# ynalcakan/RGBX_Semantic_Segmentation

Hardware: AMD Instinct MI355X
Metric: train images/sec CMX-B2 480x640 bs=2/GPU at 1/2/4/8 MI355X; % MFMA roofline (higher is better)
Workload: dtype bf16

## Files before the change

### rgbx_semantic_segmentation_amd/_lib.py

```python
from __future__ import annotations

import ctypes
import os
import re

import torch

_HERE = os.path.dirname(os.path.abspath(__file__))
_VARIANT = os.environ.get("CMX_LIB_VARIANT", "")
LIB_PATH = os.path.join(_HERE, f"libcmx_hip_{_VARIANT}.so" if _VARIANT else "libcmx_hip.so")
HEADER_PATHS = [os.path.join(_HERE, "..", "include", "cmx_hip.h"), os.path.join(_HERE, "cmx_hip.h")]
OHEM_HEADER_PATHS = [os.path.join(_HERE, "..", "include", "cmx_ohem.h"), os.path.join(_HERE, "cmx_ohem.h")]
EASPP_HEADER_PATHS = [os.path.join(_HERE, "..", "include", "cmx_easpp.h"), os.path.join(_HERE, "cmx_easpp.h")]
FCN_HEADER_PATHS = [os.path.join(_HERE, "..", "include", "cmx_fcn.h"), os.path.join(_HERE, "cmx_fcn.h")]
DEEPLAB_HEADER_PATHS = [os.path.join(_HERE, "..", "include", "cmx_deeplab.h"), os.path.join(_HERE, "cmx_deeplab.h")]


class CMXError(RuntimeError):
    pass


CMX_OK, CMX_ERR_SHAPE, CMX_ERR_DTYPE, CMX_ERR_LAUNCH, CMX_ERR_ARG = 0, -1, -2, -3, -4


def _ctype(decl: str):
    decl = decl.strip()
    if "*" in decl:
        if decl.startswith("const char") and decl.count("*") == 1 and not decl.split("*")[1].strip():
            return ctypes.c_char_p
        return ctypes.c_void_p
    base = decl.rsplit(" ", 1)[0] if " " in decl else decl
    base = base.replace("const", "").strip()
    return {"int": ctypes.c_int32, "int64_t": ctypes.c_int64, "uint64_t": ctypes.c_uint64, "float": ctypes.c_float,
            "size_t": ctypes.c_size_t, "double": ctypes.c_double, "hipStream_t": ctypes.c_void_p, "void": None}[base]


POINTER, STREAM, SCALAR = "pointer", "stream", "scalar"


def _kind(decl: str) -> str:
    if "*" in decl:
        return SCALAR if decl.strip().startswith("const char") else POINTER
    return STREAM if "hipStream_t" in decl.split() else SCALAR


class Signature(tuple):
    kinds: tuple = ()


def _header(path: str | None) -> str:
    return open(path or next(p for p in HEADER_PATHS if os.path.exists(p))).read()


def parse_header(path: str | None = None):
    text = re.sub(r"/\*.*?\*/", "", _header(path), flags=re.S)
    out = {}
    for m in re.finditer(r"^\s*([A-Za-z_][\w\s\*]*?)\b(cmx_\w+)\s*\(([^)]*)\)\s*;", text, re.M):
        ret, name, args = m.group(1), m.group(2), m.group(3).strip()
        rt = ctypes.c_char_p if ret.strip() == "const char*" else _ctype(ret.strip() + " r")
        decls = [] if args in ("", "void") else args.split(",")
        out[name] = Signature((rt, [_ctype(a) for a in decls]))
        out[name].kinds = tuple(_kind(a) for a in decls)
    return out


def header_abi_version(path: str | None = None) -> int:
    m = re.search(r"^#define\s+CMX_ABI_VERSION\s+(\d+)", _header(path), re.M)
    if m is None:
        raise CMXError(f"{path or 'cmx_hip.h'} defines no CMX_ABI_VERSION")
    return int(m.group(1))


def _load():
    if not os.path.exists(LIB_PATH):
        raise CMXError(f"libcmx_hip.so not found at {LIB_PATH}; run __graft_entry__.build() "
                       "(or `make -C rgbx_semantic_segmentation_amd/csrc`).  There is no CPU fallback.")
    lib = ctypes.CDLL(LIB_PATH)
    lib.cmx_abi_version.restype = ctypes.c_int32
    lib.cmx_abi_version.argtypes = []
    want, have = header_abi_version(), int(lib.cmx_abi_version())
    if have != want:
        raise CMXError(f"{LIB_PATH} was built for C-ABI revision {have}, the header declares {want}: "
                       "rebuild it (`make -C rgbx_semantic_segmentation_amd/csrc`)")
    sigs = parse_header()
    ohem = parse_header(next(p for p in OHEM_HEADER_PATHS if os.path.exists(p)))
    easpp = parse_header(next(p for p in EASPP_HEADER_PATHS if os.path.exists(p)))
    fcn = parse_header(next(p for p in FCN_HEADER_PATHS if os.path.exists(p)))
    deeplab = parse_header(next(p for p in DEEPLAB_HEADER_PATHS if os.path.exists(p)))
    for table in (sigs, ohem, easpp, fcn, deeplab):
        for name, (rt, argt) in table.items():
            fn = getattr(lib, name)
            fn.argtypes = argt
            fn.restype = rt
            assert STREAM not in table[name].kinds[:-1], f"{name}: hipStream_t must be the last parameter"
    return lib, sigs, ohem, easpp, fcn, deeplab


LIB, SIGNATURES, OHEM_SIGNATURES, EASPP_SIGNATURES, FCN_SIGNATURES, DEEPLAB_SIGNATURES = _load()


def last_error() -> str:
    return LIB.cmx_last_error().decode()


def stream() -> int:
    return torch.cuda.current_stream().cuda_stream


def ptr(t) -> int:
    return 0 if t is None else t.data_ptr()


def _pointer_arg(a):
    return a.data_ptr() if isinstance(a, torch.Tensor) else a


def _scalar_arg(a):
    if isinstance(a, torch.Tensor):
        raise TypeError("a tensor was passed where the header declares a scalar")
    return int(a) if a is True or a is False else a


_BOUND = {name: (getattr(LIB, name), tuple(_pointer_arg if k == POINTER else _scalar_arg for k in sig.kinds),
                 sig.kinds[-1:] == (STREAM,))
          for name, sig in {**SIGNATURES, **OHEM_SIGNATURES, **EASPP_SIGNATURES, **FCN_SIGNATURES,
                            **DEEPLAB_SIGNATURES}.items()}


def marshal(name: str, args: tuple) -> tuple:
    _, convs, takes_stream = _BOUND[name]
    if len(args) != len(convs):
        if not (takes_stream and len(args) == len(convs) - 1):
            raise TypeError(f"{name} takes {len(convs)} arguments, {len(args)} given")
        args = (*args, stream())
    return tuple([c(a) for c, a in zip(convs, args)])


observer = None


def try_call(name: str, *args) -> int:
    fn = _BOUND[name][0]
    args = marshal(name, args)
    st = int(fn(*args))
    if st == 0 and observer is not None:
        observer(name, fn, args)
    return st


def call(name: str, *args) -> None:
    refusable(name, (), *args)


REFUSED = object()


def refusable(name: str, refusals: tuple, *args):
    st = try_call(name, *args)
    if st in refusals:
        return REFUSED
    if st != 0:
        raise CMXError(f"{name} failed ({st}): {last_error()}")


def query(name: str, *args) -> int:
    return int(_BOUND[name][0](*marshal(name, args)))


DTYPE_CODES = {torch.float32: 0, torch.bfloat16: 1, torch.float16: 2}


def dtype_code(t: torch.Tensor) -> int:
    if t.dtype not in DTYPE_CODES:
        raise CMXError(f"unsupported dtype {t.dtype}")
    return DTYPE_CODES[t.dtype]
```

### rgbx_semantic_segmentation_amd/csrc/dwconv.hip

```cpp
#include "cmx_common.h"

namespace {
constexpr int RXF = 4;
constexpr int RXB = 2;
constexpr int RY = 8;
constexpr int DW_BWD_THREADS = 65536;

typedef cmx_f2 Px[2];

template <typename T>
__device__ __forceinline__ void ld4(const T* p, Px& v) {
  if constexpr (sizeof(T) == 4) {
    const float4 a = *reinterpret_cast<const float4*>(p);
    v[0] = (cmx_f2){a.x, a.y};
    v[1] = (cmx_f2){a.z, a.w};
  } else {
    const uint2 a = *reinterpret_cast<const uint2*>(p);
    v[0] = unpack2<T>(a.x);
    v[1] = unpack2<T>(a.y);
  }
}

template <typename T>
__device__ __forceinline__ void st4(T* p, const Px& v) {
  if constexpr (sizeof(T) == 4) {
    *reinterpret_cast<float4*>(p) = make_float4(v[0].x, v[0].y, v[1].x, v[1].y);
  } else {
    *reinterpret_cast<uint2*>(p) = make_uint2(pack2<T>(v[0].x, v[0].y), pack2<T>(v[1].x, v[1].y));
  }
}

template <typename T>
__device__ __forceinline__ cmx_f2 stored(cmx_f2 v) {
  if constexpr (sizeof(T) == 4) {
    return v;
  } else {
    return unpack2<T>(pack2<T>(v.x, v.y));
  }
}

__device__ __forceinline__ void load_w36(const float* wg, cmx_f2 (&w2)[2][9]) {
  const float4* p = reinterpret_cast<const float4*>(wg);
  float w[36];
#pragma unroll
  for (int i = 0; i < 9; ++i) {
    const float4 a = p[i];
    w[4 * i] = a.x; w[4 * i + 1] = a.y; w[4 * i + 2] = a.z; w[4 * i + 3] = a.w;
  }
#pragma unroll
  for (int k = 0; k < 9; ++k) {
    w2[0][k] = (cmx_f2){w[k], w[9 + k]};
    w2[1][k] = (cmx_f2){w[18 + k], w[27 + k]};
  }
}

__device__ __forceinline__ void load_bias(const float* b, Px& bias) {
  if (b) {
    const float4 bb = *reinterpret_cast<const float4*>(b);
    bias[0] = (cmx_f2){bb.x, bb.y};
    bias[1] = (cmx_f2){bb.z, bb.w};
  } else {
    bias[0] = bias[1] = pk_splat(0.f);
  }
}

template <typename T, int R>
__device__ __forceinline__ void load_row(const T* ib, int y, int x0, int H, int W, int C, Px (&r)[R + 2]) {
  const bool yok = y >= 0 && y < H;
#pragma unroll
  for (int j = 0; j < R + 2; ++j) {
    const int x = x0 - 1 + j;
    if (yok && x >= 0 && x < W) {
      ld4<T>(ib + (y * W + x) * C, r[j]);
    } else {
      r[j][0] = pk_splat(0.f);
      r[j][1] = pk_splat(0.f);
    }
  }
}

struct Strip {
  int img, x0, y0;
};

template <int R>
__device__ __forceinline__ Strip strip_of(int s, int NXS, int NYS) {
  Strip st;
  st.x0 = (s % NXS) * R;
  const int r = s / NXS;
  st.y0 = (r % NYS) * RY;
  st.img = r / NYS;
  return st;
}

template <typename T, bool FLIP, int ACT>
__global__ __launch_bounds__(256) void dw_fwd_kernel(const T* __restrict__ h, const float* __restrict__ w,
                                                     const float* __restrict__ b, T* __restrict__ out, int ipg, int H,
                                                     int W, int C, int NXS, int NYS) {
  const int CQ = C >> 2;
  const int t = blockIdx.x * blockDim.x + threadIdx.x;
  if (t >= CQ * NXS * NYS * ipg) return;
  const int g = blockIdx.y;
  const int c0 = (t % CQ) * 4;
  const Strip st = strip_of<RXF>(t / CQ, NXS, NYS);
  cmx_f2 wr[2][9];
  load_w36(w + ((long)g * C + c0) * 9, wr);
  Px bias;
  load_bias(b ? b + g * C + c0 : nullptr, bias);
  const long off = ((long)g * ipg + st.img) * H * W * C + c0;
  const T* ib = h + off;
  T* ob = out + off;
  Px rin[3][RXF + 2];
  load_row<T, RXF>(ib, st.y0 - 1, st.x0, H, W, C, rin[0]);
  load_row<T, RXF>(ib, st.y0, st.x0, H, W, C, rin[1]);
#pragma unroll
  for (int rr = 0; rr < RY; ++rr) {
    const int y = st.y0 + rr;
    load_row<T, RXF>(ib, y + 1, st.x0, H, W, C, rin[(rr + 2) % 3]);
#pragma unroll
    for (int xi = 0; xi < RXF; ++xi) {
      Px acc = {bias[0], bias[1]};
#pragma unroll
      for (int i = 0; i < 3; ++i)
#pragma unroll
        for (int j = 0; j < 3; ++j) {
          const int tap = FLIP ? 8 - (i * 3 + j) : i * 3 + j;
#pragma unroll
          for (int u = 0; u < 2; ++u) acc[u] = pk_fma(wr[u][tap], rin[(rr + i) % 3][xi + j][u], acc[u]);
        }
      acc[0] = act2_fwd<ACT>(acc[0]);
      acc[1] = act2_fwd<ACT>(acc[1]);
      if (y < H && st.x0 + xi < W) st4<T>(ob + (y * W + st.x0 + xi) * C, acc);
    }
  }
}

template <typename T, int ACT>
__global__ __launch_bounds__(256) void dw_bwd_dz_kernel(const T* __restrict__ da, const T* __restrict__ h,
                                                        const float* __restrict__ w, const float* __restrict__ b,
                                                        T* __restrict__ dz, float* __restrict__ ws, int ipg, int H,
                                                        int W, int C, int NXS, int NYS, int P) {
  const int CQ = C >> 2;
  const int t = blockIdx.x * blockDim.x + threadIdx.x;
  if (t >= CQ * P) return;
  const int g = blockIdx.y;
  const int q = t % CQ, slot = t / CQ;
  const int c0 = q * 4;
  cmx_f2 wr[2][9], aw[2][9];
  Px bias, ab;
  load_w36(w + ((long)g * C + c0) * 9, wr);
  load_bias(b ? b + g * C + c0 : nullptr, bias);
#pragma unroll
  for (int u = 0; u < 2; ++u) {
    ab[u] = pk_splat(0.f);
#pragma unroll
    for (int k = 0; k < 9; ++k) aw[u][k] = pk_splat(0.f);
  }
  const int nstrips = NXS * NYS * ipg;
  for (int s = slot; s < nstrips; s += P) {
    const Strip st = strip_of<RXB>(s, NXS, NYS);
    const long off = ((long)g * ipg + st.img) * H * W * C + c0;
    const T* ib = h + off;
    const T* dab = da + off;
    T* dzb = dz + off;
    Px rin[3][RXB + 2];
    load_row<T, RXB>(ib, st.y0 - 1, st.x0, H, W, C, rin[0]);
    load_row<T, RXB>(ib, st.y0, st.x0, H, W, C, rin[1]);
#pragma unroll
    for (int rr = 0; rr < RY; ++rr) {
      const int y = st.y0 + rr;
      load_row<T, RXB>(ib, y + 1, st.x0, H, W, C, rin[(rr + 2) % 3]);
#pragma unroll
      for (int xi = 0; xi < RXB; ++xi) {
        const bool in = y < H && st.x0 + xi < W;
        Px d = {pk_splat(0.f), pk_splat(0.f)};
        if (in) {
          Px z = {bias[0], bias[1]};
#pragma unroll
          for (int k = 0; k < 9; ++k)
#pragma unroll
            for (int u = 0; u < 2; ++u) z[u] = pk_fma(wr[u][k], rin[(rr + k / 3) % 3][xi + k % 3][u], z[u]);
          const int pofs = (y * W + st.x0 + xi) * C;
          ld4<T>(dab + pofs, d);
#pragma unroll
          for (int u = 0; u < 2; ++u) d[u] = d[u] * act2_grad<ACT>(z[u]);
          st4<T>(dzb + pofs, d);
#pragma unroll
          for (int u = 0; u < 2; ++u) d[u] = stored<T>(d[u]);
        }
#pragma unroll
        for (int u = 0; u < 2; ++u) {
          ab[u] += d[u];
#pragma unroll
          for (int k = 0; k < 9; ++k) aw[u][k] = pk_fma(d[u], rin[(rr + k / 3) % 3][xi + k % 3][u], aw[u][k]);
        }
      }
    }
  }
  float* o = ws + ((long)g * P + slot) * C * 10 + (long)c0 * 10;
#pragma unroll
  for (int u = 0; u < 2; ++u) {
#pragma unroll
    for (int k = 0; k < 9; ++k) {
      o[(2 * u) * 10 + k] = aw[u][k].x;
      o[(2 * u + 1) * 10 + k] = aw[u][k].y;
    }
    o[(2 * u) * 10 + 9] = ab[u].x;
    o[(2 * u + 1) * 10 + 9] = ab[u].y;
  }
}

__global__ void dw_scatter_kernel(const float* __restrict__ tmp, float* __restrict__ dw, float* __restrict__ db, int G,
                                  int C, int accumulate) {
  const long total = (long)G * C * 10;
  for (int i = blockIdx.x * blockDim.x + threadIdx.x; i < (int)total; i += gridDim.x * blockDim.x) {
    const int k = i % 10;
    const int gc = i / 10;
    const float s = tmp[i];
    float* o = k < 9 ? &dw[gc * 9 + k] : (db ? &db[gc] : nullptr);
    if (o) *o = accumulate ? *o + s : s;
  }
}

constexpr int TY2 = 8, TX2 = 16;
constexpr int EY = TY2 + 2, EX = TX2 + 2;
constexpr int HY = TY2 + 4, HX = TX2 + 4;
constexpr int TYB = 16, TXB = 16, EYB = TYB + 2, EXB = TXB + 2;

template <typename T> struct V8;
template <> struct V8<bf16> { uint4 a; };
template <> struct V8<f16> { uint4 a; };
template <> struct V8<float> { float4 a, b; };

template <typename T>
__device__ __forceinline__ V8<T> v8_load(const T* p) {
  V8<T> v;
  if constexpr (sizeof(T) == 2) v.a = *reinterpret_cast<const uint4*>(p);
  else { v.a = reinterpret_cast<const float4*>(p)[0]; v.b = reinterpret_cast<const float4*>(p)[1]; }
  return v;
}
template <typename T>
__device__ __forceinline__ void v8_store(T* p, const V8<T>& v) {
  if constexpr (sizeof(T) == 2) *reinterpret_cast<uint4*>(p) = v.a;
  else { reinterpret_cast<float4*>(p)[0] = v.a; reinterpret_cast<float4*>(p)[1] = v.b; }
}
template <typename T>
__device__ __forceinline__ V8<T> v8_zero() {
  V8<T> v;
  if constexpr (sizeof(T) == 2) v.a = make_uint4(0, 0, 0, 0);
  else { v.a = make_float4(0.f, 0.f, 0.f, 0.f); v.b = v.a; }
  return v;
}
template <typename T>
__device__ __forceinline__ void v8_unpack(const V8<T>& v, cmx_f2 (&o)[4]) {
  if constexpr (sizeof(T) == 2) {
    const uint32_t w[4] = {v.a.x, v.a.y, v.a.z, v.a.w};
#pragma unroll
    for (int i = 0; i < 4; ++i) o[i] = unpack2<T>(w[i]);
  } else {
    o[0] = (cmx_f2){v.a.x, v.a.y}; o[1] = (cmx_f2){v.a.z, v.a.w};
    o[2] = (cmx_f2){v.b.x, v.b.y}; o[3] = (cmx_f2){v.b.z, v.b.w};
  }
}
template <typename T>
__device__ __forceinline__ V8<T> v8_pack(const cmx_f2 (&o)[4]) {
  V8<T> v;
  if constexpr (sizeof(T) == 2) {
    v.a = make_uint4(pack2<T>(o[0].x, o[0].y), pack2<T>(o[1].x, o[1].y), pack2<T>(o[2].x, o[2].y),
                     pack2<T>(o[3].x, o[3].y));
  } else {
    v.a = make_float4(o[0].x, o[0].y, o[1].x, o[1].y);
    v.b = make_float4(o[2].x, o[2].y, o[3].x, o[3].y);
  }
  return v;
}

__device__ __forceinline__ void load_w72(const float* wg, cmx_f2 (&w2)[4][9]) {
  cmx_f2 (&a)[2][9] = *reinterpret_cast<cmx_f2 (*)[2][9]>(&w2[0]);
  cmx_f2 (&b)[2][9] = *reinterpret_cast<cmx_f2 (*)[2][9]>(&w2[2]);
  load_w36(wg, a);
  load_w36(wg + 36, b);
}

struct Tile2 {
  int g, img, ty0, tx0, cb0, sp;
};
template <int TY_ = TY2, int TX_ = TX2>
__device__ __forceinline__ Tile2 tile2_of(int CB, int ipg, int tiles_x, int tiles_y, int ncb) {
  Tile2 t;
  int b = blockIdx.x;
  const int cb = b % ncb; b /= ncb;
  t.sp = b;
  const int tx = b % tiles_x; b /= tiles_x;
  const int ty = b % tiles_y; b /= tiles_y;
  t.img = b;
  t.g = blockIdx.y;
  t.ty0 = ty * TY_; t.tx0 = tx * TX_; t.cb0 = cb * CB;
  return t;
}

template <typename T, int CB, int RY_, int RX_>
__device__ __forceinline__ void stage_region(const T* __restrict__ base, T* img, int y0, int x0, int H, int W, int C) {
  constexpr int NCG = CB / 8, NPX = RY_ * RX_;
  constexpr int ITER = (NCG * NPX + 255) / 256;
  V8<T> v[ITER];
#pragma unroll
  for (int k = 0; k < ITER; ++k) {
    const int it = threadIdx.x + k * 256;
    const int cg = it % NCG, px = it / NCG;
    const int y = y0 + px / RX_, x = x0 + px % RX_;
    v[k] = v8_zero<T>();
    if (it < NCG * NPX && y >= 0 && y < H && x >= 0 && x < W) v[k] = v8_load<T>(base + ((long)y * W + x) * C + cg * 8);
  }
#pragma unroll
  for (int k = 0; k < ITER; ++k) {
    const int it = threadIdx.x + k * 256;
    if (it < NCG * NPX) v8_store<T>(img + ((it % NCG) * NPX + it / NCG) * 8, v[k]);
  }
}

template <typename T> struct V4;
template <> struct V4<bf16> { uint2 a; };
template <> struct V4<f16> { uint2 a; };
template <> struct V4<float> { float4 a; };
template <typename T>
__device__ __forceinline__ V4<T> v4_load(const T* p) {
  V4<T> v;
  if constexpr (sizeof(T) == 2) v.a = *reinterpret_cast<const uint2*>(p);
  else v.a = *reinterpret_cast<const float4*>(p);
  return v;
}
template <typename T>
__device__ __forceinline__ void v4_unpack(const V4<T>& v, cmx_f2 (&o)[2]) {
  if constexpr (sizeof(T) == 2) {
    o[0] = unpack2<T>(v.a.x);
    o[1] = unpack2<T>(v.a.y);
  } else {
    o[0] = (cmx_f2){v.a.x, v.a.y}; o[1] = (cmx_f2){v.a.z, v.a.w};
  }
}
template <typename T>
__device__ __forceinline__ void v4_store(T* p, const cmx_f2 (&o)[2]) {
  if constexpr (sizeof(T) == 2) *reinterpret_cast<uint2*>(p) = make_uint2(pack2<T>(o[0].x, o[0].y), pack2<T>(o[1].x, o[1].y));
  else *reinterpret_cast<float4*>(p) = make_float4(o[0].x, o[0].y, o[1].x, o[1].y);
}
template <typename T, int CB, int RY_, int RX_>
__device__ __forceinline__ void stage_region_pm(const T* __restrict__ base, T* img, int y0, int x0, int H, int W, int C) {
  constexpr int NCG = CB / 8, NPX = RY_ * RX_;
  constexpr int ITER = (NCG * NPX + 255) / 256;
  V8<T> v[ITER];
#pragma unroll
  for (int k = 0; k < ITER; ++k) {
    const int it = threadIdx.x + k * 256;
    const int cg = it % NCG, px = it / NCG;
    const int y = y0 + px / RX_, x = x0 + px % RX_;
    v[k] = v8_zero<T>();
    if (it < NCG * NPX && y >= 0 && y < H && x >= 0 && x < W) v[k] = v8_load<T>(base + ((long)y * W + x) * C + cg * 8);
  }
#pragma unroll
  for (int k = 0; k < ITER; ++k) {
    const int it = threadIdx.x + k * 256;
    if (it < NCG * NPX) v8_store<T>(img + it * 8, v[k]);
  }
}

template <typename T, int CB, int ACT, bool FLIP>
__global__ __launch_bounds__(256) void dw2_fwd_kernel(const T* __restrict__ h, const float* __restrict__ w,
                                                      const float* __restrict__ b, T* __restrict__ out, int ipg, int H,
                                                      int W, int C, int tiles_x, int tiles_y, int ncb,
                                                      T* __restrict__ gprime) {
  constexpr int NCQ = CB / 4, PPI = 256 / NCQ;
  __shared__ __attribute__((aligned(16))) T hs[EY * EX * CB];
  const Tile2 t = tile2_of(CB, ipg, tiles_x, tiles_y, ncb);
  const long ibase = ((long)t.g * ipg + t.img) * H * W * C + t.cb0;
  stage_region_pm<T, CB, EY, EX>(h + ibase, hs, t.ty0 - 1, t.tx0 - 1, H, W, C);
  const int cq = threadIdx.x % NCQ, pl = threadIdx.x / NCQ;
  const int c0 = t.cb0 + cq * 4;
  __syncthreads();
  cmx_f2 wr[2][9], bias[2];
  load_w36(w + ((long)t.g * C + c0) * 9, wr);
  if (b) {
    const float4 b0 = *reinterpret_cast<const float4*>(b + (long)t.g * C + c0);
    bias[0] = (cmx_f2){b0.x, b0.y}; bias[1] = (cmx_f2){b0.z, b0.w};
  } else {
    bias[0] = bias[1] = pk_splat(0.f);
  }
  const T* hc = hs + cq * 4;
  if constexpr (PPI == TX2) {
    const int x = t.tx0 + pl;
    const int nr = H - t.ty0;
    if (x >= W) return;
    const T* hp = hc + pl * CB;
    cmx_f2 win[3][3][2];
#pragma unroll
    for (int j = 0; j < 3; ++j) {
      v4_unpack<T>(v4_load<T>(hp + j * CB), win[0][j]);
      v4_unpack<T>(v4_load<T>(hp + (EX + j) * CB), win[1][j]);
    }
    long o = ibase + ((long)t.ty0 * W + x) * C + cq * 4;
    const long ostep = (long)W * C;
#pragma unroll
    for (int r = 0; r < TY2; ++r) {
      if (r < nr) {
#pragma unroll
        for (int j = 0; j < 3; ++j) {
          v4_unpack<T>(v4_load<T>(hp + ((r + 2) * EX + j) * CB), win[(r + 2) % 3][j]);
        }
        cmx_f2 acc[2] = {bias[0], bias[1]};
#pragma unroll
        for (int i = 0; i < 3; ++i)
#pragma unroll
          for (int j = 0; j < 3; ++j) {
            const int tap = FLIP ? 8 - (i * 3 + j) : i * 3 + j;
#pragma unroll
            for (int u = 0; u < 2; ++u) acc[u] = pk_fma(wr[u][tap], win[(r + i) % 3][j][u], acc[u]);
          }
        if (gprime) {
          cmx_f2 gd[2];
#pragma unroll
          for (int u = 0; u < 2; ++u) gd[u] = act2_grad<ACT>(acc[u]);
          v4_store<T>(gprime + o, gd);
        }
#pragma unroll
        for (int u = 0; u < 2; ++u) acc[u] = act2_fwd<ACT>(acc[u]);
        v4_store<T>(out + o, acc);
        o += ostep;
      }
    }
  } else {
    for (int it = pl; it < TY2 * TX2; it += PPI) {
      const int r = it / TX2, c = it % TX2;
      const int y = t.ty0 + r, x = t.tx0 + c;
      if (y >= H || x >= W) continue;
      cmx_f2 acc[2] = {bias[0], bias[1]};
#pragma unroll
      for (int i = 0; i < 3; ++i)
#pragma unroll
        for (int j = 0; j < 3; ++j) {
          cmx_f2 v[2];
          v4_unpack<T>(v4_load<T>(hc + ((r + i) * EX + c + j) * CB), v);
          const int tap = FLIP ? 8 - (i * 3 + j) : i * 3 + j;
#pragma unroll
          for (int u = 0; u < 2; ++u) acc[u] = pk_fma(wr[u][tap], v[u], acc[u]);
        }
      const long o = ibase + ((long)y * W + x) * C + cq * 4;
      if (gprime) {
        cmx_f2 gd[2];
#pragma unroll
        for (int u = 0; u < 2; ++u) gd[u] = act2_grad<ACT>(acc[u]);
        v4_store<T>(gprime + o, gd);
      }
#pragma unroll
      for (int u = 0; u < 2; ++u) acc[u] = act2_fwd<ACT>(acc[u]);
      v4_store<T>(out + o, acc);
    }
  }
}

template <int N>
__device__ __forceinline__ void rs_step(const float (&v)[N], float (&o)[N / 2], int off, bool up) {
#pragma unroll
  for (int k = 0; k < N / 2; ++k) {
    const float send = up ? v[k] : v[k + N / 2];
    const float keep = up ? v[k + N / 2] : v[k];
    o[k] = keep + xor_lane(send, off);
  }
}

template <typename T, int CB>
__device__ __forceinline__ void stage_dz(const T* __restrict__ da, const T* __restrict__ gp, T* dzs, int ty0, int tx0,
                                         int H, int W, int C) {
  constexpr int NCG = CB / 8, NE = EYB * EXB;
  constexpr int ITE = (NCG * NE + 255) / 256;
  V8<T> a[ITE], g[ITE];
#pragma unroll
  for (int k = 0; k < ITE; ++k) {
    const int it = threadIdx.x + k * 256;
    const int cg = it % NCG, px = it / NCG;
    const int y = ty0 - 1 + px / EXB, x = tx0 - 1 + px % EXB;
    a[k] = v8_zero<T>();
    g[k] = v8_zero<T>();
    if (it < NCG * NE && y >= 0 && y < H && x >= 0 && x < W) {
      const long o = ((long)y * W + x) * C + cg * 8;
      a[k] = v8_load<T>(da + o);
      g[k] = v8_load<T>(gp + o);
    }
  }
#pragma unroll
  for (int k = 0; k < ITE; ++k) {
    const int it = threadIdx.x + k * 256;
    if (it < NCG * NE) {
      cmx_f2 d[4], gd[4];
      v8_unpack<T>(a[k], d);
      v8_unpack<T>(g[k], gd);
#pragma unroll
      for (int u = 0; u < 4; ++u) d[u] = d[u] * gd[u];
      v8_store<T>(dzs + it * 8, v8_pack<T>(d));
    }
  }
}

template <typename T, int CB>
__global__ __launch_bounds__(256, 3) void dw2_bwdg_kernel(const T* __restrict__ da, const T* __restrict__ h,
                                                       const T* __restrict__ gprime, const float* __restrict__ w,
                                                       T* __restrict__ dh, float* __restrict__ part, int ipg, int H,
                                                       int W, int C, int tiles_x, int tiles_y, int ncb, int nsp) {
  constexpr int NCQ = CB / 4, PPI = 256 / NCQ;
  constexpr int NE = EYB * EXB, NIN = TYB * TXB;
  constexpr int LPQ = 64 / NCQ;
  constexpr int NV = LPQ == 4 ? 10 : 5;
  constexpr int NIT = NIN / PPI;
  __shared__ __attribute__((aligned(16))) T dzs[NE * CB];
  static_assert(sizeof(dzs) >= 4 * 64 * NV * sizeof(float), "cross-wave reduce buffer");
  static_assert(NIN % PPI == 0, "pixel rounds");
  const Tile2 t = tile2_of<TYB, TXB>(CB, ipg, tiles_x, tiles_y, ncb);
  const long ibase = ((long)t.g * ipg + t.img) * H * W * C + t.cb0;
  stage_dz<T, CB>(da + ibase, gprime + ibase, dzs, t.ty0, t.tx0, H, W, C);
  const int cq = threadIdx.x % NCQ, pl = threadIdx.x / NCQ;
  const int c0 = t.cb0 + cq * 4;
  V4<T> hreg[NIT];
#pragma unroll
  for (int k = 0; k < NIT; ++k) {
    const int it = pl + k * PPI;
    const int y = t.ty0 + it / TXB, x = t.tx0 + it % TXB;
    hreg[k].a = {};
    if (y < H && x < W) hreg[k] = v4_load<T>(h + ibase + ((long)y * W + x) * C + cq * 4);
  }
  __syncthreads();
  cmx_f2 wr[2][9];
  load_w36(w + ((long)t.g * C + c0) * 9, wr);
  const T* dzc = dzs + cq * 4;
  cmx_f2 acc[2][10];
#pragma unroll
  for (int u = 0; u < 2; ++u)
#pragma unroll
    for (int k = 0; k < 10; ++k) acc[u][k] = pk_splat(0.f);
  if constexpr (PPI == TXB) {
    const int x = t.tx0 + pl;
    const int nr = H - t.ty0;
    if (x < W) {
      const T* dzp = dzc + pl * CB;
      cmx_f2 win[3][3][2];
#pragma unroll
      for (int j = 0; j < 3; ++j) {
        v4_unpack<T>(v4_load<T>(dzp + j * CB), win[0][j]);
        v4_unpack<T>(v4_load<T>(dzp + (EXB + j) * CB), win[1][j]);
      }
      long o = ibase + ((long)t.ty0 * W + x) * C + cq * 4;
      const long ostep = (long)W * C;
#pragma unroll
      for (int k = 0; k < NIT; ++k) {
        if (k < nr) {
#pragma unroll
          for (int j = 0; j < 3; ++j) v4_unpack<T>(v4_load<T>(dzp + ((k + 2) * EXB + j) * CB), win[(k + 2) % 3][j]);
          cmx_f2 hv[2];
          v4_unpack<T>(hreg[k], hv);
          cmx_f2 g[2] = {pk_splat(0.f), pk_splat(0.f)};
#pragma unroll
          for (int i = 0; i < 3; ++i)
#pragma unroll
            for (int j = 0; j < 3; ++j) {
              const cmx_f2 (&dv)[2] = win[(k + 2 - i) % 3][2 - j];
#pragma unroll
              for (int u = 0; u < 2; ++u) {
                g[u] = pk_fma(wr[u][i * 3 + j], dv[u], g[u]);
                acc[u][i * 3 + j] = pk_fma(hv[u], dv[u], acc[u][i * 3 + j]);
              }
              if (i == 1 && j == 1) {
#pragma unroll
                for (int u = 0; u < 2; ++u) acc[u][9] += dv[u];
              }
            }
          if (dh) v4_store<T>(dh + o, g);
          o += ostep;
        }
      }
    }
  } else {
#pragma unroll
    for (int k = 0; k < NIT; ++k) {
      const int it = pl + k * PPI;
      const int r = it / TXB, c = it % TXB;
      const int y = t.ty0 + r, x = t.tx0 + c;
      if (y >= H || x >= W) continue;
      cmx_f2 hv[2];
      v4_unpack<T>(hreg[k], hv);
      cmx_f2 g[2] = {pk_splat(0.f), pk_splat(0.f)};
#pragma unroll
      for (int i = 0; i < 3; ++i)
#pragma unroll
        for (int j = 0; j < 3; ++j) {
          cmx_f2 dv[2];
          v4_unpack<T>(v4_load<T>(dzc + ((r + 2 - i) * EXB + c + 2 - j) * CB), dv);
#pragma unroll
          for (int u = 0; u < 2; ++u) {
            g[u] = pk_fma(wr[u][i * 3 + j], dv[u], g[u]);
            acc[u][i * 3 + j] = pk_fma(hv[u], dv[u], acc[u][i * 3 + j]);
          }
          if (i == 1 && j == 1) {
#pragma unroll
            for (int u = 0; u < 2; ++u) acc[u][9] += dv[u];
          }
        }
      if (dh) v4_store<T>(dh + ibase + ((long)y * W + x) * C + cq * 4, g);
    }
  }
  const int lane = threadIdx.x & 63, wv = threadIdx.x >> 6;
  float flat[40], r20[20], r10[10];
#pragma unroll
  for (int u = 0; u < 2; ++u)
#pragma unroll
    for (int k = 0; k < 10; ++k) {
      flat[(2 * u) * 10 + k] = acc[u][k].x;
      flat[(2 * u + 1) * 10 + k] = acc[u][k].y;
    }
  int seg = 0;
  rs_step<40>(flat, r20, NCQ, (lane & NCQ) != 0); seg = seg * 2 + ((lane & NCQ) != 0);
  rs_step<20>(r20, r10, 2 * NCQ, (lane & (2 * NCQ)) != 0); seg = seg * 2 + ((lane & (2 * NCQ)) != 0);
  float rv[NV];
  if constexpr (NV == 5) {
    rs_step<10>(r10, rv, 4 * NCQ, (lane & (4 * NCQ)) != 0); seg = seg * 2 + ((lane & (4 * NCQ)) != 0);
  } else {
#pragma unroll
    for (int k = 0; k < 10; ++k) rv[k] = r10[k];
  }
  __syncthreads();
  float* red = reinterpret_cast<float*>(dzs);
#pragma unroll
  for (int k = 0; k < NV; ++k) red[(wv * 64 + lane) * NV + k] = rv[k];
  __syncthreads();
  float* o = part + ((long)t.g * nsp + t.sp) * C * 10 + (long)t.cb0 * 10;
  for (int e = threadIdx.x; e < 64 * NV; e += 256) {
    const float v = red[e] + red[64 * NV + e] + red[128 * NV + e] + red[192 * NV + e];
    const int l = e / NV, k = e % NV;
    const int q = l % NCQ, sg = (l / NCQ);
    int sgi = 0;
#pragma unroll
    for (int bit = 0; bit < (NV == 5 ? 3 : 2); ++bit) sgi = sgi * 2 + ((sg >> bit) & 1);
    o[q * 40 + sgi * NV + k] = v;
  }
}


template <typename T, int CB, int ACT>
__global__ __launch_bounds__(256, 2) void dw2_bwd_kernel(const T* __restrict__ da, const T* __restrict__ h,
                                                      const float* __restrict__ w, const float* __restrict__ b,
                                                      T* __restrict__ dh, float* __restrict__ part, int ipg, int H,
                                                      int W, int C, int tiles_x, int tiles_y, int ncb, int nsp) {
  constexpr int NCG = CB / 8, TPC = 256 / NCG;
  __shared__ __attribute__((aligned(16))) T hs[NCG * HY * HX * 8];
  __shared__ __attribute__((aligned(16))) T das[NCG * EY * EX * 8];
  __shared__ __attribute__((aligned(16))) T dzs[NCG * EY * EX * 8];
  const Tile2 t = tile2_of(CB, ipg, tiles_x, tiles_y, ncb);
  const long ibase = ((long)t.g * ipg + t.img) * H * W * C + t.cb0;
  stage_region<T, CB, HY, HX>(h + ibase, hs, t.ty0 - 2, t.tx0 - 2, H, W, C);
  stage_region<T, CB, EY, EX>(da + ibase, das, t.ty0 - 1, t.tx0 - 1, H, W, C);
  const int cg = threadIdx.x / TPC, pl = threadIdx.x % TPC;
  const int c0 = t.cb0 + cg * 8;
  cmx_f2 wr[4][9], bias[4];
  load_w72(w + ((long)t.g * C + c0) * 9, wr);
  if (b) {
    const float4 b0 = *reinterpret_cast<const float4*>(b + (long)t.g * C + c0);
    const float4 b1 = *reinterpret_cast<const float4*>(b + (long)t.g * C + c0 + 4);
    bias[0] = (cmx_f2){b0.x, b0.y}; bias[1] = (cmx_f2){b0.z, b0.w};
    bias[2] = (cmx_f2){b1.x, b1.y}; bias[3] = (cmx_f2){b1.z, b1.w};
  } else {
#pragma unroll
    for (int u = 0; u < 4; ++u) bias[u] = pk_splat(0.f);
  }
  __syncthreads();
  const T* hc = hs + cg * HY * HX * 8;
  const T* dac = das + cg * EY * EX * 8;
  T* dzc = dzs + cg * EY * EX * 8;
  for (int it = pl; it < EY * EX; it += TPC) {
    const int r = it / EX, c = it % EX;
    const int y = t.ty0 - 1 + r, x = t.tx0 - 1 + c;
    V8<T> dzv = v8_zero<T>();
    if (y >= 0 && y < H && x >= 0 && x < W) {
      cmx_f2 z[4] = {bias[0], bias[1], bias[2], bias[3]};
#pragma unroll
      for (int i = 0; i < 3; ++i)
#pragma unroll
        for (int j = 0; j < 3; ++j) {
          cmx_f2 v[4];
          v8_unpack<T>(v8_load<T>(hc + ((r + i) * HX + c + j) * 8), v);
#pragma unroll
          for (int u = 0; u < 4; ++u) z[u] = pk_fma(wr[u][i * 3 + j], v[u], z[u]);
        }
      cmx_f2 d[4];
      v8_unpack<T>(v8_load<T>(dac + it * 8), d);
#pragma unroll
      for (int u = 0; u < 4; ++u) d[u] = d[u] * act2_grad<ACT>(z[u]);
      dzv = v8_pack<T>(d);
    }
    v8_store<T>(dzc + it * 8, dzv);
  }
  __syncthreads();
  if (dh) {
    for (int it = pl; it < TY2 * TX2; it += TPC) {
      const int r = it / TX2, c = it % TX2;
      const int y = t.ty0 + r, x = t.tx0 + c;
      if (y >= H || x >= W) continue;
      cmx_f2 g[4] = {pk_splat(0.f), pk_splat(0.f), pk_splat(0.f), pk_splat(0.f)};
#pragma unroll
      for (int i = 0; i < 3; ++i)
#pragma unroll
        for (int j = 0; j < 3; ++j) {
          cmx_f2 dv[4];
          v8_unpack<T>(v8_load<T>(dzc + ((r + 2 - i) * EX + c + 2 - j) * 8), dv);
#pragma unroll
          for (int u = 0; u < 4; ++u) g[u] = pk_fma(wr[u][i * 3 + j], dv[u], g[u]);
        }
      v8_store<T>(dh + ibase + ((long)y * W + x) * C + cg * 8, v8_pack<T>(g));
    }
  }
  cmx_f2 acc[4][10];
#pragma unroll
  for (int u = 0; u < 4; ++u)
#pragma unroll
    for (int k = 0; k < 10; ++k) acc[u][k] = pk_splat(0.f);
  for (int it = pl; it < TY2 * TX2; it += TPC) {
    const int r = it / TX2, c = it % TX2;
    if (t.ty0 + r >= H || t.tx0 + c >= W) continue;
    cmx_f2 dz0[4];
    v8_unpack<T>(v8_load<T>(dzc + ((r + 1) * EX + c + 1) * 8), dz0);
#pragma unroll
    for (int i = 0; i < 3; ++i)
#pragma unroll
      for (int j = 0; j < 3; ++j) {
        cmx_f2 hv[4];
        v8_unpack<T>(v8_load<T>(hc + ((r + 1 + i) * HX + c + 1 + j) * 8), hv);
#pragma unroll
        for (int u = 0; u < 4; ++u) acc[u][i * 3 + j] = pk_fma(dz0[u], hv[u], acc[u][i * 3 + j]);
      }
#pragma unroll
    for (int u = 0; u < 4; ++u) acc[u][9] += dz0[u];
  }
  const int lane = threadIdx.x & 63;
  float flat[80], r40[40], r20[20], r10[10], r5[5];
#pragma unroll
  for (int u = 0; u < 4; ++u)
#pragma unroll
    for (int k = 0; k < 10; ++k) {
      flat[(2 * u) * 10 + k] = acc[u][k].x;
      flat[(2 * u + 1) * 10 + k] = acc[u][k].y;
    }
  int seg = 0, s_off = TPC >> 1;
  rs_step<80>(flat, r40, s_off, (lane & s_off) != 0); seg = seg * 2 + ((lane & s_off) != 0); s_off >>= 1;
  rs_step<40>(r40, r20, s_off, (lane & s_off) != 0); seg = seg * 2 + ((lane & s_off) != 0); s_off >>= 1;
  rs_step<20>(r20, r10, s_off, (lane & s_off) != 0); seg = seg * 2 + ((lane & s_off) != 0); s_off >>= 1;
  rs_step<10>(r10, r5, s_off, (lane & s_off) != 0); seg = seg * 2 + ((lane & s_off) != 0); s_off >>= 1;
  for (; s_off > 0; s_off >>= 1) {
#pragma unroll
    for (int k = 0; k < 5; ++k) r5[k] += xor_lane(r5[k], s_off);
  }
  if ((lane & (TPC / 16 - 1)) == 0) {
    float* o = part + ((long)t.g * nsp + t.sp) * C * 10 + (long)c0 * 10 + seg * 5;
#pragma unroll
    for (int k = 0; k < 5; ++k) o[k] = r5[k];
  }
}

int bwd_slots(int CQ, int nstrips) {
  int pmax = DW_BWD_THREADS / CQ;
  if (pmax < 1) pmax = 1;
  if (pmax >= nstrips) return nstrips;
  const int per = (nstrips + pmax - 1) / pmax;
  return (nstrips + per - 1) / per;
}
}

static int tile_cb(int C, int dtype) { return (C % 64 == 0 && (dtype == 1 || dtype == 2)) ? 64 : C % 32 == 0 ? 32 : 0; }

extern "C" {

int cmx_dwconv3x3_fwd(const void* h, const float* w, const float* b, void* out, int NI, int imgs_per_group, int H,
                      int W, int C, int act, int dtype, hipStream_t s) {
  return cmx_dwconv3x3_fwd_save(h, w, b, out, nullptr, NI, imgs_per_group, H, W, C, act, dtype, s);
}

int cmx_dwconv3x3_fwd_save(const void* h, const float* w, const float* b, void* out, void* gprime, int NI,
                           int imgs_per_group, int H, int W, int C, int act, int dtype, hipStream_t s) {
  CMX_REQUIRE(C % 4 == 0 && NI % imgs_per_group == 0, CMX_ERR_SHAPE, "dwconv_fwd: C=%d", C);
  CMX_REQUIRE(!gprime || tile_cb(C, dtype), CMX_ERR_SHAPE, "dwconv_fwd_save: C=%d has no LDS-tiled path", C);
  CMX_REQUIRE((long)NI * H * W * C < (1L << 31), CMX_ERR_SHAPE, "dwconv_fwd: tensor too large for 32-bit indexing");
  const int G = NI / imgs_per_group;
  const int CB = tile_cb(C, dtype);
  if (CB) {
    const int tx = cdiv(W, TX2), ty = cdiv(H, TY2), ncb = C / CB;
    const dim3 grid((unsigned)imgs_per_group * ty * tx * ncb, G);
    CMX_DISPATCH(dtype, T, {
      CMX_ACT_DISPATCH(act, A, {
        if (CB == 32) {
          hipLaunchKernelGGL((dw2_fwd_kernel<T, 32, A, false>), grid, dim3(256), 0, s, (const T*)h, w, b, (T*)out,
                             imgs_per_group, H, W, C, tx, ty, ncb, (T*)gprime);
        } else if constexpr (sizeof(T) == 2) {
          hipLaunchKernelGGL((dw2_fwd_kernel<T, 64, A, false>), grid, dim3(256), 0, s, (const T*)h, w, b, (T*)out,
                             imgs_per_group, H, W, C, tx, ty, ncb, (T*)gprime);
        }
      });
    });
    return cmx_check_launch("dwconv_fwd");
  }
  const int NXS = cdiv(W, RXF), NYS = cdiv(H, RY);
  const long threads = (long)(C / 4) * NXS * NYS * imgs_per_group;
  CMX_DISPATCH(dtype, T, {
    CMX_ACT_DISPATCH(act, A, {
      hipLaunchKernelGGL((dw_fwd_kernel<T, false, A>), dim3(cdiv(threads, 256), G), dim3(256), 0, s, (const T*)h, w,
                         b, (T*)out, imgs_per_group, H, W, C, NXS, NYS);
    });
  });
  return cmx_check_launch("dwconv_fwd");
}

int cmx_dwconv3x3_bwd_saved(const void* da, const void* h, const void* gprime, const float* w, void* dh, float* dw,
                            float* db, float* workspace, int NI, int imgs_per_group, int H, int W, int C, int accumulate,
                            int dtype, hipStream_t s) {
  const int CB = tile_cb(C, dtype);
  CMX_REQUIRE(CB && NI % imgs_per_group == 0 && gprime, CMX_ERR_SHAPE, "dwconv_bwd_saved: C=%d", C);
  CMX_REQUIRE((long)NI * H * W * C < (1L << 31), CMX_ERR_SHAPE, "dwconv_bwd_saved: tensor too large");
  const int G = NI / imgs_per_group;
  const int tx = cdiv(W, TXB), ty = cdiv(H, TYB), ncb = C / CB;
  const int P = imgs_per_group * ty * tx;
  const dim3 grid((unsigned)P * ncb, G);
  CMX_DISPATCH(dtype, T, {
    if (CB == 32) {
      hipLaunchKernelGGL((dw2_bwdg_kernel<T, 32>), grid, dim3(256), 0, s, (const T*)da, (const T*)h,
                         (const T*)gprime, w, (T*)dh, workspace, imgs_per_group, H, W, C, tx, ty, ncb, P);
    } else if constexpr (sizeof(T) == 2) {
      hipLaunchKernelGGL((dw2_bwdg_kernel<T, 64>), grid, dim3(256), 0, s, (const T*)da, (const T*)h,
                         (const T*)gprime, w, (T*)dh, workspace, imgs_per_group, H, W, C, tx, ty, ncb, P);
    }
  });
  if (!dw && !db) return cmx_check_launch("dwconv_bwd_saved");
  float* tmp = workspace + (size_t)G * P * C * 10;
  int st = cmx_reduce_partials(workspace, tmp, G, P, C * 10, 0, 1.f, s);
  if (st) return st;
  const long tot = (long)G * C * 10;
  hipLaunchKernelGGL(dw_scatter_kernel, dim3(cdiv(tot, 256) < 4096 ? cdiv(tot, 256) : 4096), dim3(256), 0, s, tmp, dw,
                     db, G, C, accumulate);
  return cmx_check_launch("dwconv_bwd_saved");
}

int cmx_dwconv3x3_bwd_saved_tiles(int imgs_per_group, int H, int W) {
  return imgs_per_group * cdiv(H, TYB) * cdiv(W, TXB);
}

size_t cmx_dwconv3x3_bwd_workspace(int NI, int imgs_per_group, int H, int W, int C) {
  const int G = NI / imgs_per_group;
  int P;
  if (tile_cb(C, 0)) {
    const int p8 = imgs_per_group * cdiv(H, TY2) * cdiv(W, TX2);
    const int p16 = cmx_dwconv3x3_bwd_saved_tiles(imgs_per_group, H, W);
    P = p8 > p16 ? p8 : p16;
  } else {
    P = bwd_slots(C / 4, cdiv(W, RXB) * cdiv(H, RY) * imgs_per_group);
  }
  return ((size_t)G * P * C * 10 + (size_t)G * C * 10) * sizeof(float);
}

int cmx_dwconv3x3_bwd(const void* da, const void* h, const float* w, const float* b, void* dz, void* dh, float* dw,
                      float* db, float* workspace, int NI, int imgs_per_group, int H, int W, int C, int act,
                      int accumulate, int dtype, hipStream_t s) {
  CMX_REQUIRE(C % 4 == 0 && NI % imgs_per_group == 0, CMX_ERR_SHAPE, "dwconv_bwd: C=%d", C);
  CMX_REQUIRE((long)NI * H * W * C < (1L << 31), CMX_ERR_SHAPE, "dwconv_bwd: tensor too large for 32-bit indexing");
  const int G = NI / imgs_per_group;
  const int CB = tile_cb(C, dtype);
  int P;
  if (CB) {
    const int tx = cdiv(W, TX2), ty = cdiv(H, TY2), ncb = C / CB;
    P = imgs_per_group * ty * tx;
    const dim3 grid((unsigned)P * ncb, G);
    CMX_DISPATCH(dtype, T, {
      CMX_ACT_DISPATCH(act, A, {
        if (CB == 32) {
          hipLaunchKernelGGL((dw2_bwd_kernel<T, 32, A>), grid, dim3(256), 0, s, (const T*)da, (const T*)h, w, b,
                             (T*)dh, workspace, imgs_per_group, H, W, C, tx, ty, ncb, P);
        } else if constexpr (sizeof(T) == 2) {
          hipLaunchKernelGGL((dw2_bwd_kernel<T, 64, A>), grid, dim3(256), 0, s, (const T*)da, (const T*)h, w, b,
                             (T*)dh, workspace, imgs_per_group, H, W, C, tx, ty, ncb, P);
        }
      });
    });
  } else {
    CMX_REQUIRE(dz, CMX_ERR_ARG, "dwconv_bwd: C=%d takes the strip path, which needs a dz buffer", C);
    const int CQ = C / 4;
    const int NXB = cdiv(W, RXB), NXS = cdiv(W, RXF), NYS = cdiv(H, RY);
    P = bwd_slots(CQ, NXB * NYS * imgs_per_group);
    CMX_DISPATCH(dtype, T, {
      CMX_ACT_DISPATCH(act, A, {
        hipLaunchKernelGGL((dw_bwd_dz_kernel<T, A>), dim3(cdiv((long)CQ * P, 256), G), dim3(256), 0, s, (const T*)da,
                           (const T*)h, w, b, (T*)dz, workspace, imgs_per_group, H, W, C, NXB, NYS, P);
      });
      if (dh) {
        const long threads = (long)CQ * NXS * NYS * imgs_per_group;
        hipLaunchKernelGGL((dw_fwd_kernel<T, true, 0>), dim3(cdiv(threads, 256), G), dim3(256), 0, s, (const T*)dz, w,
                           (const float*)nullptr, (T*)dh, imgs_per_group, H, W, C, NXS, NYS);
      }
    });
  }
  if (!dw && !db) return cmx_check_launch("dwconv_bwd");
  float* tmp = workspace + (size_t)G * P * C * 10;
  int st = cmx_reduce_partials(workspace, tmp, G, P, C * 10, 0, 1.f, s);
  if (st) return st;
  const long tot = (long)G * C * 10;
  hipLaunchKernelGGL(dw_scatter_kernel, dim3(cdiv(tot, 256) < 4096 ? cdiv(tot, 256) : 4096), dim3(256), 0, s, tmp, dw,
                     db, G, C, accumulate);
  return cmx_check_launch("dwconv_bwd");
}

}
```

### rgbx_semantic_segmentation_amd/floor.py

```python
from __future__ import annotations

import collections

from .models.encoders.dual_segformer import MIT_SPECS, NUM_HEADS, SR_RATIOS

PEAK_TFLOPS = 2516.6
PEAK_TBS = 8.0
A = 2
F32 = 4


def _grid(H, W, k, s, p):
    return (H + 2 * p - k) // s + 1, (W + 2 * p - k) // s + 1


def step_work(backbone="mit_b2", H=480, W=640, B=2, K=40, E=512, n_params=None):
    fam = collections.defaultdict(lambda: [0.0, 0.0])

    def add(f, flops=0.0, byts=0.0):
        fam[f][0] += flops
        fam[f][1] += byts

    def gemm(M, N, Kd, G=1, res=False, wgrad=True, dgrad=True, bias_grad=True):
        add("gemm", 2 * G * M * N * Kd, G * A * (M * Kd + N * Kd + M * N + (M * N if res else 0)))
        if dgrad:
            add("gemm", 2 * G * M * N * Kd, G * A * (M * N + N * Kd + M * Kd))
        if wgrad:
            add("wgrad", 2 * G * M * N * Kd, G * (A * (M * N + M * Kd) + F32 * N * (Kd + (1 if bias_grad else 0))))

    def ln(rows, C, G=1, two=False, tap=False):
        add("layernorm", 0, G * A * rows * C * 2 + G * F32 * 2 * rows)
        add("layernorm", 0, G * A * rows * C * (3 + (1 if two else 0) + (1 if tap else 0)) + G * F32 * 2 * rows)

    def dw(M_pix, C, G=1):
        add("dwconv", 2 * 9 * G * M_pix * C * 3, G * A * M_pix * C * 3)
        add("dwconv", 0, G * A * M_pix * C * 4)

    def bn(M, C, res=False):
        add("batchnorm", 0, A * M * C * (1 + 2 + (1 if res else 0)))
        add("batchnorm", 0, A * M * C * (2 + 3 + (2 if res else 0) + (1 if res else 0)))

    dims, depths = MIT_SPECS[backbone]["embed_dims"], MIT_SPECS[backbone]["depths"]
    G = 2
    h, w, cin = H, W, 3
    grids = []
    for s in range(4):
        k, st = (7, 4) if s == 0 else (3, 2)
        h, w = _grid(h, w, k, st, k // 2)
        N, C = h * w, dims[s]
        M = B * N
        grids.append((h, w, C))
        if s == 0:
            Kp = (cin * k * k + 7) // 8 * 8
            img = F32 * B * cin * H * W
            add("pe1", 2 * G * M * C * cin * k * k, G * (img + A * C * Kp + A * M * C))
            add("pe1", 2 * G * M * C * cin * k * k, G * (img + A * M * C + F32 * C * (Kp + 1)))
        else:
            gemm(M, C, cin * k * k, G)
            add("im2col", 0, G * A * M * cin * k * k * 2)
        ln(M, C, G)
        R = SR_RATIOS[s]
        hk, wk = _grid(h, w, R, R, 0) if R > 1 else (h, w)
        Nk = hk * wk
        Mk = B * Nk
        for _ in range(depths[s]):
            ln(M, C, G, two=R > 1, tap=True)
            gemm(M, C, C, G)
            if R > 1:
                gemm(Mk, C, R * R * C, G)
                ln(Mk, C, G)
            gemm(Mk, 2 * C, C, G)
            d = C // NUM_HEADS[s]
            fwd_f = 4 * G * B * N * Nk * C
            add("sra", fwd_f, G * A * (M * C + Mk * 2 * C + M * C) + G * F32 * B * NUM_HEADS[s] * N)
            add("sra", 2.5 * fwd_f, G * A * (3 * M * C + Mk * 2 * C + M * C + Mk * 2 * C) + G * F32 * B * NUM_HEADS[s] * N * 2)
            gemm(M, C, C, G, res=True)
            ln(M, C, G, tap=True)
            gemm(M, 4 * C, C, G)
            dw(M, 4 * C, G)
            gemm(M, C, 4 * C, G, res=True)
        ln(M, C, G, tap=True)
        add("frm", 0, G * A * M * C)
        add("frm", 2 * 2 * B * (16 * C * C + 8 * C * C), F32 * 3 * (16 * C * C + 8 * C * C))
        gemm(M, C, 2 * C, 1)
        add("frm", 0, A * M * C * (G + 1 + G))
        add("frm", 0, A * M * C * (G + G + 1 + G + 1) + A * M * C * G * 2)
        d = C // NUM_HEADS[s]
        gemm(M, 2 * C, C, G)
        gemm(M, 2 * C, C, G, bias_grad=False)
        add("ffm", 2 * G * B * NUM_HEADS[s] * N * d * d * 2 * 3,
            G * A * (M * 2 * C + M * C * 2) * 3)
        gemm(M, C, 2 * C, G, res=True)
        gemm(M, C, 2 * C, 1, bias_grad=False)
        gemm(M, C, 2 * C, 1)
        dw(M, C, 1)
        gemm(M, C, C, 1)
        bn(M, C)
        bn(M, C, res=True)
        if s == 3 and backbone.endswith("_w_ef_aspp"):
            for n_out in (256, 64, 64, 64):
                gemm(M, n_out, C, 1, bias_grad=False)
                bn(M, n_out)
            for _ in range(3 * 3):
                mac2, wsz = 2 * M * 9 * 64 * 64, 9 * 64 * 64
                add("easpp", 3 * mac2, A * (2 * M * 64 + wsz) * 2 + A * 2 * M * 64 + F32 * wsz)
                bn(M, 64)
            for _ in range(3):
                gemm(M, 256, 64, 1, bias_grad=False)
                bn(M, 256)
            add("easpp", 3 * 2 * B * 256 * C, A * M * C * 2 + F32 * 3 * 256 * C)
            add("easpp", 0, A * M * (4 * 256 + 1280) * 2)
            gemm(M, C, 1280, 1, bias_grad=False)
            bn(M, C)
            add("easpp", 0, F32 * M * C * 3)
        cin = C
    h1, w1, _ = grids[0]
    N1 = B * h1 * w1
    for (hh, ww, C) in grids:
        gemm(B * hh * ww, E, C, 1)
    for (hh, ww, C) in grids[1:]:
        gemm(B * hh * ww, E, E, 1, bias_grad=False)
        add("bilinear", 0, A * (B * hh * ww * E + N1 * E) * 2)
    gemm(N1, E, E, 1)
    bn(N1, E)
    gemm(N1, K, E, 1)
    add("ce", 0, A * N1 * K * 3 + 8 * B * H * W * 2)
    if n_params:
        add("adamw", 0, n_params * 30)
    return fam


def floor_table(**kw):
    rows, tot = [], 0.0
    for f, (fl, by) in sorted(step_work(**kw).items(), key=lambda kv: -max(kv[1][0] / PEAK_TFLOPS / 1e6,
                                                                            kv[1][1] / PEAK_TBS / 1e6)):
        tf, tb = fl / (PEAK_TFLOPS * 1e6), by / (PEAK_TBS * 1e6)
        rows.append((f, fl, by, max(tf, tb), "mfma" if tf > tb else "hbm"))
        tot += max(tf, tb)
    return rows, tot


if __name__ == "__main__":
    rows, tot = floor_table(n_params=66.58e6)
    for f, fl, by, us, bd in rows:
        print(f"{f:10s} {fl / 1e9:9.1f} GFLOP {by / 1e9:8.3f} GB  floor {us:8.1f} us ({bd})")
    print(f"step floor {tot:.0f} us")
```

### rgbx_semantic_segmentation_amd/functions.py

```python
from __future__ import annotations

import os

import torch
from torch.autograd import Function

from . import deferred
from . import kernels as K


def _c(t):
    return t if t.is_contiguous() else t.contiguous()


def _dgrad(dz, W_slice, out):
    K.gemm(dz, W_slice.transpose(1, 2), out)
    return out


def _wgrad_into(dz, x, Wg_slice, bg=None):
    if deferred.wgrad(dz, x, Wg_slice, bg):
        return
    K.gemm(dz.transpose(1, 2), x.transpose(1, 2), Wg_slice, out_mode=1, dbias=bg, splitk=0)


def _fwd_gemm(x, W, b, y, act="none", res=None, rscale=None, rps=1, x2=None):
    K.gemm(x, W, y, bias=b, residual=res, rscale=rscale, rows_per_sample=rps, act=act, A2=x2)
    return y


class GLinear(Function):

    @staticmethod
    def forward(ctx, W, Wg, b, bg, anchor, act, res, rscale, rps, x1, x2, tap=None, ln=None, dgrad_tap=None):
        G, N, Ktot = W.shape
        M = x1.shape[1]
        assert x1.shape[-1] + (x2.shape[-1] if x2 is not None else 0) == Ktot, (x1.shape, W.shape)
        y = torch.empty(G, M, N, dtype=x1.dtype, device=x1.device)
        pre = None
        if ln is not None:
            gamma, beta, eps, sink = ln
            pre = K.gemm_ln(x1, W, y, gamma, beta, eps, bias=b, residual=res, rscale=rscale, rows_per_sample=rps,
                            act=act, A2=x2)
            sink.pre = pre
        if pre is None:
            _fwd_gemm(x1, W, b, y, act=act, res=res, rscale=rscale, rps=rps, x2=x2)
        ctx.save_for_backward(W, x1, x2, y if act == "relu" else None)
        ctx.meta = (Wg, bg, act, res is not None, rscale, rps, tap, dgrad_tap)
        return y

    @staticmethod
    def backward(ctx, dy):
        W, x1, x2, y = ctx.saved_tensors
        Wg, bg, act, has_res, rscale, rps, tap, dgrad_tap = ctx.meta
        dy = _c(dy)
        G, M, N = dy.shape
        dres = dy if has_res else None
        dz = dy
        if rscale is not None:
            dz = tap.take(dy) if tap is not None else None
            if dz is None:
                dz = K.scale_samples(dy, rscale, rps * N)
        if act == "relu":
            dz = K.act_bwd(dz, y, "relu")
        k1 = x1.shape[-1]
        dx1 = dx2 = None
        if dgrad_tap is not None and ctx.needs_input_grad[9] and dz.is_contiguous():
            dgrad_tap.put((dz, W[:, :, :k1]))
        elif ctx.needs_input_grad[9]:
            dx1 = _dgrad(dz, W[:, :, :k1], torch.empty_like(x1))
        if x2 is not None and ctx.needs_input_grad[10]:
            dx2 = _dgrad(dz, W[:, :, k1:], torch.empty_like(x2))
        _wgrad_into(dz, x1, Wg[:, :, :k1], bg)
        if x2 is not None:
            _wgrad_into(dz, x2, Wg[:, :, k1:])
        return (None, None, None, None, None, None, dres, None, None, dx1, dx2, None, None, None)


class LNTail:
    __slots__ = ("mod", "pre")

    def __init__(self, mod):
        self.mod, self.pre = mod, None


def glinear(store, wp, bp, x1, x2=None, act="none", res=None, rscale=None, rps=1, tap=None, ln_tail=None,
            dgrad_tap=None):
    W = store.w(wp)
    Wg = store.g(wp)
    G = W.shape[0]
    W = W.view(G, W.shape[1], -1)
    Wg = Wg.view(G, Wg.shape[1], -1)
    b = bg = None
    if bp is not None:
        b = store.w(bp, compute=False).view(G, -1)
        bg = store.g(bp).view(G, -1)
    ln = None
    N = W.shape[1]
    if ln_tail is not None and LN_ROW and N <= 128 and N % 8 == 0:
        m = ln_tail.mod
        ln = (store.w(m.weight, compute=False).view(G, -1), store.w(m.bias, compute=False).view(G, -1), m.eps, ln_tail)
    return GLinear.apply(W, Wg, b, bg, wp, act, res, rscale, rps, x1, x2, tap, ln, dgrad_tap)


LN_ROW = os.environ.get("CMX_LN_ROW", "1") != "0"

MULTI_GEMM = os.environ.get("CMX_MULTI_GEMM", "1") != "0"


def _gemm_group(jobs):
    rest = jobs
    if MULTI_GEMM and len(jobs) > 1:
        plans = [K.gemm(**j, plan=True) for j in jobs]
        ok = [p for p in plans if p is not None]
        if len(ok) > 1:
            for i in range(0, len(ok), 4):
                if len(ok[i:i + 4]) > 1:
                    K.gemm_multi(ok[i:i + 4])
                else:
                    K.gemm(**jobs[plans.index(ok[i])])
            rest = [j for j, p in zip(jobs, plans) if p is None]
    for j in rest:
        K.gemm(**j)


class GLinearMulti(Function):

    @staticmethod
    def forward(ctx, spec, *ts):
        n = len(spec)
        xs = ts[n:]
        ys, jobs = [], []
        for (W, Wg, b, bg), x in zip(spec, xs):
            y = torch.empty(W.shape[0], x.shape[1], W.shape[1], dtype=x.dtype, device=x.device)
            jobs.append(dict(A=x, B=W, C=y, bias=b))
            ys.append(y)
        _gemm_group(jobs)
        ctx.spec = spec
        ctx.save_for_backward(*xs)
        return tuple(ys)

    @staticmethod
    def backward(ctx, *dys):
        xs = ctx.saved_tensors
        spec = ctx.spec
        n = len(spec)
        dxs, jobs = [None] * n, []
        for i, ((W, Wg, b, bg), x, dy) in enumerate(zip(spec, xs, dys)):
            if dy is None:
                continue
            dy = _c(dy)
            if ctx.needs_input_grad[1 + n + i]:
                dxs[i] = torch.empty_like(x)
                jobs.append(dict(A=dy, B=W.transpose(1, 2), C=dxs[i]))
            _wgrad_into(dy, x, Wg, bg)
        _gemm_group(jobs)
        return (None,) * (1 + n) + tuple(dxs)


def glinear_multi(store, specs):
    spec, anchors, xs = [], [], []
    for wp, bp, x in specs:
        W = store.w(wp)
        G = W.shape[0]
        W = W.view(G, W.shape[1], -1)
        Wg = store.g(wp).view(G, W.shape[1], -1)
        b = bg = None
        if bp is not None:
            b = store.w(bp, compute=False).view(G, -1)
            bg = store.g(bp).view(G, -1)
        spec.append((W, Wg, b, bg))
        anchors.append(wp)
        xs.append(x)
    return GLinearMulti.apply(tuple(spec), *anchors, *xs)


class GradTap:
    __slots__ = ("t",)

    def __init__(self):
        self.t = None

    def put(self, t):
        self.t = t

    def take(self, like):
        t, self.t = self.t, None
        return t if (t is not None and t.shape == like.shape) else None


class LayerNormResF(Function):

    @staticmethod
    def forward(ctx, x, gamma, beta, gg, bg, eps, G, scale, rps, tap, anchor, pre=None, dtap=None):
        if pre is not None:
            y, mean, rstd = pre
        else:
            y, mean, rstd = K.layernorm_fwd(x, gamma, beta, eps, G=G)
        ctx.save_for_backward(x, gamma, mean, rstd)
        ctx.meta = (gg, bg, G, scale, rps, tap, dtap)
        ctx.set_materialize_grads(False)
        return y, y.view_as(y), x

    @staticmethod
    def backward(ctx, dy, dy2, dres):
        x, gamma, mean, rstd = ctx.saved_tensors
        gg, bg, G, scale, rps, tap, dtap = ctx.meta
        C = x.shape[-1]
        R = x.numel() // C // G
        handed = dtap.take() if dtap is not None else None
        if handed is not None:
            other = dy if dy is not None else dy2
            other = _c(other) if other is not None else None
            dres_c = _c(dres) if dres is not None else None
            dxs = torch.empty_like(x) if (tap is not None and scale is not None) else None
            sc = scale if dxs is not None else None
            if len(handed) == 3:
                dyc, Wc, pg = handed
                Gc, NIg, H, Wd_, Cc = pg[:5]
                xv = x.view(Gc * NIg, H, Wd_, Cc)
                out = K.conv_patch_dgrad_ln_bwd(dyc, Wc, pg, xv, gamma, mean, rstd,
                                                dres=dres_c.view_as(xv) if dres_c is not None else None,
                                                dy2=other.view_as(xv) if other is not None else None, sscale=sc,
                                                rows_per_sample=rps, dxs=dxs.view_as(xv) if dxs is not None else None)
                if out is not None:
                    out = (out[0].view_as(x), out[1])
                else:
                    dy = torch.empty(Gc * NIg, H, Wd_, Cc, dtype=dyc.dtype, device=dyc.device)
                    K.conv_patch_dgrad(dyc, Wc, dy, pg)
                    dy, dy2 = dy.view_as(x), other
            else:
                dz, Wd = handed
                out = K.gemm_ln_bwd(dz, Wd, x, gamma, mean, rstd, dres=dres_c, dy2=other, sscale=sc,
                                    rows_per_sample=rps, dxs=dxs)
                if out is None:
                    dy = _dgrad(dz, Wd, torch.empty_like(x))
                    dy2 = other
            if out is not None:
                dx, part = out
                nb = part.shape[1]
                deferred.reduce(part, gg, bg, G, nb, nb * 2 * C, 2 * C, 1, 2 * C, C, gg.stride(0), 0, bg.stride(0), 0)
                if dxs is not None:
                    tap.put(dxs)
                return dx, None, None, None, None, None, None, None, None, None, None, None, None
        elif dy is None:
            dy, dy2 = dy2, None
        dy = _c(dy) if dy is not None else torch.zeros_like(x)
        dy2 = _c(dy2) if dy2 is not None else None
        dres = _c(dres) if dres is not None else None
        dxs = torch.empty_like(x) if (tap is not None and scale is not None) else None
        defer = deferred.ENABLED
        dx, part = K.layernorm_bwd_res(dy, x, gamma, mean, rstd, G, None if defer else gg, None if defer else bg,
                                       dy2=dy2, dres=dres, sscale=scale, rows_per_sample=rps, dxs=dxs)
        if defer:
            nb = part.shape[1]
            deferred.reduce(part, gg, bg, G, nb, nb * 2 * C, 2 * C, 1, 2 * C, C, gg.stride(0), 0, bg.stride(0), 0)
        if dxs is not None:
            tap.put(dxs)
        return dx, None, None, None, None, None, None, None, None, None, None, None, None


LN_BWD_FUSE = os.environ.get("CMX_LN_BWD_FUSE", "1") != "0"


def ln_bwd_fusable(x, patch=None) -> bool:
    C = x.shape[-1]
    ok = (LN_BWD_FUSE and deferred.ENABLED and x.dtype in (torch.bfloat16, torch.float16) and C <= 128
          and C % 8 == 0 and x.is_contiguous())
    if ok and patch is not None:
        H, W, R = patch
        ok = C in (64, 128) and H % R == 0 and W % R == 0
    return ok


def layernorm_res(store, mod, x, G, scale=None, rps=1, tap=None, tail=None, dtap=None):
    gamma = store.w(mod.weight, compute=False).view(G, -1)
    beta = store.w(mod.bias, compute=False).view(G, -1)
    gg = store.g(mod.weight).view(G, -1)
    bg = store.g(mod.bias).view(G, -1)
    pre = None
    if tail is not None:
        assert tail.mod is mod
        pre, tail.pre = tail.pre, None
    return LayerNormResF.apply(x, gamma, beta, gg, bg, mod.eps, G, scale, rps, tap, mod.weight, pre, dtap)


class LayerNormF(Function):
    @staticmethod
    def forward(ctx, x, gamma, beta, gg, bg, eps, G, anchor):
        y, mean, rstd = K.layernorm_fwd(x, gamma, beta, eps, G=G)
        ctx.save_for_backward(x, gamma, mean, rstd)
        ctx.gg, ctx.bg, ctx.G = gg, bg, G
        return y

    @staticmethod
    def backward(ctx, dy):
        x, gamma, mean, rstd = ctx.saved_tensors
        if deferred.ENABLED:
            dx = _layernorm_bwd_deferred(_c(dy), x, gamma, mean, rstd, ctx.G, ctx.gg, ctx.bg)
        else:
            dx = K.layernorm_bwd(_c(dy), x, gamma, mean, rstd, ctx.G, ctx.gg, ctx.bg)
        return dx, None, None, None, None, None, None, None


def _layernorm_bwd_deferred(dy, x, gamma, mean, rstd, G, gg, bg):
    C = x.shape[-1]
    dx, part = K.layernorm_bwd(dy, x, gamma, mean, rstd, G, None, None)
    nb = part.shape[1]
    deferred.reduce(part, gg, bg, G, nb, nb * 2 * C, 2 * C, 1, 2 * C, C, gg.stride(0), 0, bg.stride(0), 0)
    return dx


def layernorm(store, mod, x, G):
    gamma = store.w(mod.weight, compute=False).view(G, -1)
    beta = store.w(mod.bias, compute=False).view(G, -1)
    gg = store.g(mod.weight).view(G, -1)
    bg = store.g(mod.bias).view(G, -1)
    return LayerNormF.apply(x, gamma, beta, gg, bg, mod.eps, G, mod.weight)


class SplitF(Function):

    @staticmethod
    def forward(ctx, t, k, dim):
        ctx.k, ctx.dim, ctx.n = k, dim, t.shape[dim]
        ctx.set_materialize_grads(False)
        return t.narrow(dim, 0, k), t.narrow(dim, k, t.shape[dim] - k)

    @staticmethod
    def backward(ctx, g1, g2):
        if g1 is None and g2 is None:
            return None, None, None
        ref = g1 if g1 is not None else g2
        shp = list(ref.shape)
        if g1 is None:
            shp[ctx.dim] = ctx.k
            g1 = torch.zeros(shp, dtype=ref.dtype, device=ref.device)
        if g2 is None:
            shp[ctx.dim] = ctx.n - ctx.k
            g2 = torch.zeros(shp, dtype=ref.dtype, device=ref.device)
        return torch.cat([g1, g2], ctx.dim), None, None


def split(t, k, dim=-1):
    return SplitF.apply(t, k, dim % t.dim())


class ResidualF(Function):

    @staticmethod
    def forward(ctx, x, y, scale, nps):
        ctx.scale, ctx.nps = scale, nps
        return K.residual_add(x, y, scale, n_per_sample=nps)

    @staticmethod
    def backward(ctx, dout):
        dout = _c(dout)
        dy = dout if ctx.scale is None else K.scale_samples(dout, ctx.scale, ctx.nps)
        return dout, dy, None, None


class ReluF(Function):
    @staticmethod
    def forward(ctx, x):
        y = K.act_fwd(x, "relu")
        ctx.save_for_backward(y)
        return y

    @staticmethod
    def backward(ctx, dy):
        (y,) = ctx.saved_tensors
        return K.act_bwd(_c(dy), y, "relu")


class SRAttentionF(Function):

    @staticmethod
    def forward(ctx, q, kv, Bt, N, Nk, heads, D):
        C = heads * D
        o, lse = K.sra_attn_fwd(q, kv, kv[..., C:], Bt, N, Nk, heads, D, D ** -0.5, C, 2 * C)
        o = o.view(q.shape)
        ctx.save_for_backward(q, kv, o, lse)
        ctx.dims = (Bt, N, Nk, heads, D)
        return o

    @staticmethod
    def backward(ctx, do):
        q, kv, o, lse = ctx.saved_tensors
        Bt, N, Nk, heads, D = ctx.dims
        C = heads * D
        dq, dkv = K.sra_attn_bwd(q, kv, kv[..., C:], o, _c(do), lse, Bt, N, Nk, heads, D, D ** -0.5, C, 2 * C)
        return dq.view(q.shape), dkv.view(kv.shape), None, None, None, None, None


class ActF(Function):

    @staticmethod
    def forward(ctx, z, act):
        ctx.act = act
        ctx.save_for_backward(z)
        return K.act_fwd(z, act)

    @staticmethod
    def backward(ctx, dy):
        (z,) = ctx.saved_tensors
        return K.act_bwd(_c(dy), z, ctx.act), None


class CrossFlashAttnF(Function):

    @staticmethod
    def forward(ctx, q, kv, B, N, heads, D):
        G, M, C = q.shape
        assert G == 2 and M == B * N and kv.shape == (2, M, 2 * C) and q.is_contiguous() and kv.is_contiguous()
        dt = K.dtype_code(q)
        o = torch.empty_like(q)
        lse = torch.empty(2, B, heads, N, dtype=torch.float32, device=q.device)
        for g in range(2):
            src = kv[1 - g]
            K.call("cmx_sra_attn_fwd", q[g], src, src[:, C:], o[g], lse[g], B, N, N, heads, D, C, 2 * C, C, D ** -0.5,
                   dt)
        ctx.save_for_backward(q, kv, o, lse)
        ctx.dims = (B, N, heads, D)
        return o

    @staticmethod
    def backward(ctx, do):
        q, kv, o, lse = ctx.saved_tensors
        B, N, heads, D = ctx.dims
        C = heads * D
        do = _c(do)
        dt = K.dtype_code(q)
        dq = torch.empty_like(q)
        dkv = torch.empty_like(kv)
        ws = K._ws(K.query("cmx_sra_attn_bwd_workspace", B, N, N, heads, D), q.device)
        for g in range(2):
            src, dsrc = kv[1 - g], dkv[1 - g]
            K.call("cmx_sra_attn_bwd", q[g], src, src[:, C:], o[g], do[g], lse[g], dq[g], dsrc, dsrc[:, C:], ws, B, N,
                   N, heads, D, C, 2 * C, C, C, C, 2 * C, D ** -0.5, dt)
        return dq, dkv, None, None, None, None


def _rowln(x, g, b, eps):
    R, C = x.shape
    y = torch.empty_like(x)
    mean = torch.empty(R, dtype=torch.float32, device=x.device)
    rstd = torch.empty_like(mean)
    K.call("cmx_rowln_fwd", x, g, b, y, mean, rstd, R, C, float(eps))
    return y, mean, rstd


def _rowln_bwd(dy, x, g, mean, rstd, gg, gb):
    R, C = x.shape
    dx = torch.empty_like(x)
    K.call("cmx_rowln_bwd", dy, x, g, mean, rstd, dx, gg, gb, R, C)
    return dx


class IFRMF(Function):

    @staticmethod
    def forward(ctx, x, sw, prm, anchor):
        (W1, b1, g1, e1, W3, b3, g4, e4, Wg, bgt, lc, ls, eps1, eps4) = prm["w"]
        G, B, N, C = x.shape
        dt = K.dtype_code(x)
        pooled, argmax = K.frm_pool_fwd(x, pool_tickets(anchor, x, B, C))
        h1 = K.small_linear_fwd(pooled, W1, b1, 4 * C)
        n1, m1, r1 = _rowln(h1, g1, e1, eps1)
        a1 = K.act_fwd(n1, "gelu")
        h2 = K.small_linear_fwd(a1, W3, b3, 2 * C)
        y, m2, r2 = _rowln(h2, g4, e4, eps4)
        gt = K.small_linear_fwd(y, Wg, bgt, 2 * C, "sigmoid")
        cw = torch.empty(B, 2 * C, dtype=torch.float32, device=x.device)
        K.call("cmx_mul2", y, gt, cw, B * 2 * C)
        out = torch.empty_like(x)
        K.call("cmx_ifrm_combine_fwd", x, cw, sw, lc, ls, out, B, N, C, dt)
        ctx.save_for_backward(x, sw, pooled, argmax, h1, m1, r1, n1, a1, h2, m2, r2, y, gt, cw)
        ctx.prm = prm
        return out

    @staticmethod
    def backward(ctx, dout):
        x, sw, pooled, argmax, h1, m1, r1, n1, a1, h2, m2, r2, y, gt, cw = ctx.saved_tensors
        (W1, b1, g1, e1, W3, b3, g4, e4, Wg, bgt, lc, ls, eps1, eps4) = ctx.prm["w"]
        (gW1, gb1, gg1, ge1, gW3, gb3, gg4, ge4, gWg, gbg, glc, gls) = ctx.prm["g"]
        G, B, N, C = x.shape
        dt = K.dtype_code(x)
        f32 = dict(dtype=torch.float32, device=x.device)
        dout = _c(dout)
        dx = torch.empty_like(x)
        dsw = torch.empty_like(sw)
        nb = K.query("cmx_ifrm_combine_nblk", B, N)
        part = torch.empty(nb, 2 * C, **f32)
        lpart = torch.empty(2, nb, **f32)
        K.call("cmx_ifrm_combine_bwd", dout, x, cw, sw, lc, ls, dx, dsw, part, lpart, B, N, C, dt)
        K.partials_sum(lpart[0], glc, 1, nb, 1)
        K.partials_sum(lpart[1], gls, 1, nb, 1)
        dcw = K.partials_sum(part, torch.empty(B, 2 * C, **f32), B, nb // B, 2 * C)
        dy = torch.empty_like(y)
        dgt = torch.empty_like(gt)
        K.call("cmx_mul2_bwd", dcw, y, gt, dy, dgt, B * 2 * C)
        dyp = K.small_linear_bwd(dgt, 1, 0, 2 * C, gt, y, Wg, gWg, gbg, 2 * C, "sigmoid")
        K.partials_sum(dyp, dy, 1, dyp.shape[0], B * 2 * C, accumulate=True)
        dh2 = _rowln_bwd(dy, h2, g4, m2, r2, gg4, ge4)
        dap = K.small_linear_bwd(dh2, 1, 0, 2 * C, h2, a1, W3, gW3, gb3, 2 * C)
        da1 = K.partials_sum(dap, torch.empty(B, 4 * C, **f32), 1, dap.shape[0], B * 4 * C)
        dn1 = K.act_bwd(da1, n1, "gelu")
        dh1 = _rowln_bwd(dn1, h1, g1, m1, r1, gg1, ge1)
        dpp = K.small_linear_bwd(dh1, 1, 0, 4 * C, h1, pooled, W1, gW1, gb1, 4 * C)
        K.frm_pool_bwd(dpp, argmax, dx)
        return dx, dsw, None, None


class DWConvF(Function):

    @staticmethod
    def forward(ctx, h, w, b, wg, bg, NI, ipg, H, W, act, anchor):
        C = h.shape[-1]
        out = torch.empty_like(h)
        tiled = C % (64 if h.dtype in (torch.bfloat16, torch.float16) else 32) == 0
        gprime = torch.empty_like(h) if tiled else None
        K.call("cmx_dwconv3x3_fwd_save", h, w, b, out, gprime, NI, ipg, H, W, C, K.ACT[act], K.dtype_code(h))
        ctx.save_for_backward(h, w, b, gprime)
        ctx.meta = (wg, bg, NI, ipg, H, W, act)
        return out

    @staticmethod
    def backward(ctx, da):
        h, w, b, gprime = ctx.saved_tensors
        wg, bg, NI, ipg, H, W, act = ctx.meta
        C = h.shape[-1]
        da = _c(da)
        G, dt = NI // ipg, K.dtype_code(h)
        dh = torch.empty_like(h) if ctx.needs_input_grad[0] else None
        nbytes = K.query("cmx_dwconv3x3_bwd_workspace", NI, ipg, H, W, C)
        ws = K._ws(nbytes, h.device)
        defer = deferred.ENABLED
        dw, db = (None, None) if defer else (wg, bg)
        if gprime is not None:
            K.call("cmx_dwconv3x3_bwd_saved", da, h, gprime, w, dh, dw, db, ws, NI, ipg, H, W, C, 0, dt)
        else:
            dz = torch.empty_like(h) if C % 32 else None
            K.call("cmx_dwconv3x3_bwd", da, h, w, b, dz, dh, dw, db, ws, NI, ipg, H, W, C, K.ACT[act], 0, dt)
        if defer:
            P = (K.query("cmx_dwconv3x3_bwd_saved_tiles", ipg, H, W) if gprime is not None
                 else nbytes // (40 * G * C) - 1)
            deferred.reduce(ws, wg, bg, G, P, P * C * 10, C * 10, C, 10, 9, wg.stride(0), 9, bg.stride(0), 1)
        return dh, None, None, None, None, None, None, None, None, None, None


def dwconv(store, conv, h, NI, ipg, H, W, act):
    G = NI // ipg
    w = store.w(conv.weight, compute=False).view(G, -1, 9)
    b = store.w(conv.bias, compute=False).view(G, -1)
    wg = store.g(conv.weight).view(G, -1, 9)
    bg = store.g(conv.bias).view(G, -1)
    return DWConvF.apply(h, w, b, wg, bg, NI, ipg, H, W, act, conv.weight)


class DgradTap:
    __slots__ = ("t",)

    def __init__(self):
        self.t = None

    def put(self, t):
        self.t = t

    def take(self):
        t, self.t = self.t, None
        return t


IMPLICIT_CONV = os.environ.get("CMX_IMPLICIT_CONV", "1") != "0"
PE1_DIRECT = os.environ.get("CMX_PE1_DIRECT", "1") != "0"


class ConvF(Function):

    @staticmethod
    def forward(ctx, x, W, Wg, b, bg, geom, anchor, x2=None, dtap=None):
        G, NI, H, Wd, C, KH, KW, st, pad, Ho, Wo, nchw = geom
        ctx.x2 = x2
        ctx.dtap = dtap
        ctx.pe1 = None
        Kp = W.shape[-1]
        if IMPLICIT_CONV and not nchw and x.dtype in (torch.bfloat16, torch.float16) and C % 64 == 0 \
                and x.is_contiguous():
            N = W.shape[1]
            NIg = NI // G
            y = torch.empty(G, NIg * Ho * Wo, N, dtype=x.dtype, device=x.device)
            M = NIg * Ho * Wo
            dt = K.dtype_code(x)
            sk = K.query("cmx_gemm_splitk", G, M, N, Kp, 0, dt)
            ws = K._ws(K.query("cmx_gemm_workspace", G, M, N, sk), x.device) if sk > 1 else None
            K.call("cmx_conv_implicit_fwd", x, W, y, b, ws, G, NIg, H, Wd, C, KH, KW, st, pad, Ho, Wo, N,
                   NIg * H * Wd * C, W.stride(0), y.stride(0), b.stride(0) if b is not None else 0, sk, dt)
            ctx.save_for_backward(x, W)
            ctx.meta = (Wg, bg, geom)
            ctx.xshape = x.shape
            ctx.implicit = True
            return y
        ctx.implicit = False
        if nchw and PE1_DIRECT and W.dtype in (torch.bfloat16, torch.float16) and deferred.ENABLED \
                and b is not None and (C, KH, KW, st, pad) == (3, 7, 7, 4, 3) and W.shape[1] <= 64 \
                and W.shape[1] % 8 == 0 and x.dtype == torch.float32 and x.is_contiguous() \
                and (x2 is None or x2.is_contiguous()):
            Bg = NI // G
            img1 = (x2 if x2 is not None else x[Bg:]) if G == 2 else None
            y = K.pe1_conv_fwd(x, img1, W, b, (G, Bg, C, H, Wd, KH, KW, st, pad, Ho, Wo))
            ctx.pe1 = (x, img1)
            ctx.save_for_backward(None, W)
            ctx.meta = (Wg, bg, geom)
            return y
        cols = torch.empty(G, NI // G * Ho * Wo, Kp, dtype=W.dtype, device=W.device)
        if nchw:
            if x2 is not None:
                K.call("cmx_im2col_nchw2_f32", x, x2, NI - x2.shape[0], cols, NI, C, H, Wd, KH, KW, st, pad, Ho, Wo, Kp,
                       K.dtype_code(cols))
            else:
                K.call("cmx_im2col_nchw_f32", x, cols, NI, C, H, Wd, KH, KW, st, pad, Ho, Wo, Kp, K.dtype_code(cols))
        else:
            K.im2col_nhwc(x, cols, NI, H, Wd, C, KH, KW, st, pad, Ho, Wo)
        y = _fwd_gemm(cols, W, b, torch.empty(G, cols.shape[1], W.shape[1], dtype=cols.dtype, device=cols.device))
        ctx.save_for_backward(cols, W)
        ctx.meta = (Wg, bg, geom)
        ctx.xshape = x.shape
        return y

    @staticmethod
    def backward(ctx, dy):
        cols, W = ctx.saved_tensors
        Wg, bg, geom = ctx.meta
        G, NI, H, Wd, C, KH, KW, st, pad, Ho, Wo, nchw = geom
        dy = _c(dy)
        if ctx.pe1 is not None:
            _pe1_wgrad(dy, ctx.pe1, Wg, bg, (G, NI // G, C, H, Wd, KH, KW, st, pad, Ho, Wo), W.shape[1], W.shape[-1])
            return None, None, None, None, None, None, None, None, None
        if ctx.implicit:
            x = cols
            if not deferred.conv_wgrad(dy, x, Wg, bg, (G, NI // G, H, Wd, C, KH, KW, st, pad, Ho, Wo)):
                cols = torch.empty(G, NI // G * Ho * Wo, W.shape[-1], dtype=x.dtype, device=x.device)
                _wgrad_into(dy, K.im2col_nhwc(x, cols, NI, H, Wd, C, KH, KW, st, pad, Ho, Wo), Wg, bg)
        else:
            _wgrad_into(dy, cols, Wg, bg)
        dx = None
        if ctx.needs_input_grad[0] and ctx.dtap is not None and KH == KW == st and pad == 0 and H == Ho * st \
                and Wd == Wo * st:
            ctx.dtap.put((dy, W, (G, NI // G, H, Wd, C, st, Ho, Wo)))
        elif ctx.needs_input_grad[0] and not nchw and KH == KW == st and pad == 0 and H // st == Ho and Wd // st == Wo:
            exact = H % st == 0 and Wd % st == 0
            dx = (torch.empty if exact else torch.zeros)(NI, H, Wd, C, dtype=dy.dtype, device=dy.device)
            dx = K.conv_patch_dgrad(dy, W, dx, (G, NI // G, H, Wd, C, st, Ho, Wo)).view(ctx.xshape)
        elif ctx.needs_input_grad[0] and not nchw:
            dcols = _dgrad(dy, W, torch.empty(G, NI // G * Ho * Wo, W.shape[-1], dtype=dy.dtype, device=dy.device))
            dx = torch.empty(NI, H, Wd, C, dtype=dy.dtype, device=dy.device)
            K.call("cmx_col2im_nhwc", dcols, dx, NI, H, Wd, C, KH, KW, st, pad, Ho, Wo, W.shape[-1], K.dtype_code(dx))
            dx = dx.view(ctx.xshape)
        return dx, None, None, None, None, None, None, None, None


def _pe1_wgrad(dy, imgs, Wg, bg, geom, N, Kp):
    ws = K.pe1_conv_wgrad(dy, *imgs, geom, N, Kp)
    G, nblk = ws.shape[:2]
    deferred.reduce(ws, Wg, bg, G, nblk, nblk * N * (Kp + 1), N * (Kp + 1), N, Kp + 1, Kp, Wg.stride(0),
                    Wg.stride(1), bg.stride(0), 1)


class PatchEmbed1F(Function):

    @staticmethod
    def forward(ctx, x, x2, W, Wg, b, bg, gamma, beta, gg, gb, eps, geom, anchor):
        G, NI, H, Wd, C, KH, KW, st, pad, Ho, Wo = geom
        Bg = NI // G
        img1 = (x2 if x2 is not None else x[Bg:]) if G == 2 else None
        y, out, mean, rstd = K.pe1_conv_fwd(x, img1, W, b, (G, Bg, C, H, Wd, KH, KW, st, pad, Ho, Wo),
                                            ln=(gamma, beta, eps))
        ctx.save_for_backward(y, gamma, mean, rstd)
        ctx.imgs = (x, img1)
        ctx.meta = (W.shape, Wg, bg, gg, gb, geom)
        return out

    @staticmethod
    def backward(ctx, dout):
        y, gamma, mean, rstd = ctx.saved_tensors
        wshape, Wg, bg, gg, gb, geom = ctx.meta
        G, NI, H, Wd, C, KH, KW, st, pad, Ho, Wo = geom
        dy = _layernorm_bwd_deferred(_c(dout), y, gamma, mean, rstd, G, gg, gb)
        _pe1_wgrad(dy, ctx.imgs, Wg, bg, (G, NI // G, C, H, Wd, KH, KW, st, pad, Ho, Wo), wshape[1], wshape[-1])
        return (None,) * 13


def patch_embed1(store, pe, x, G, NI, H, W, x2=None):
    mod = pe.proj
    KH, KW = mod.kernel_size
    C = x.shape[1]
    st, pad = pe.stride, pe.pad
    Ho, Wo = (H + 2 * pad - KH) // st + 1, (W + 2 * pad - KW) // st + 1
    Wt = store.w(mod.weight)
    N = Wt.shape[1]
    if (PE1_DIRECT and deferred.ENABLED and Wt.dtype in (torch.bfloat16, torch.float16) and mod.bias is not None
            and (C, KH, KW, st, pad) == (3, 7, 7, 4, 3) and N in (32, 64) and x.dtype == torch.float32
            and x.is_contiguous() and (x2 is None or x2.is_contiguous())):
        Wt = Wt.view(G, N, -1)
        Wg = store.g(mod.weight).view(G, N, -1)
        b = store.w(mod.bias, compute=False).view(G, -1)
        bg = store.g(mod.bias).view(G, -1)
        nm = pe.norm
        gamma = store.w(nm.weight, compute=False).view(G, -1)
        beta = store.w(nm.bias, compute=False).view(G, -1)
        gg = store.g(nm.weight).view(G, -1)
        gb = store.g(nm.bias).view(G, -1)
        geom = (G, NI, H, W, C, KH, KW, st, pad, Ho, Wo)
        out = PatchEmbed1F.apply(x, x2, Wt, Wg, b, bg, gamma, beta, gg, gb, nm.eps, geom, mod.weight)
        return out, Ho, Wo
    y, Ho, Wo = conv(store, mod, x, G, NI, H, W, C, st, pad, nchw=True, x2=x2)
    return layernorm(store, pe.norm, y, G), Ho, Wo


def conv(store, mod, x, G, NI, H, W, C, stride, pad, nchw=False, x2=None, dtap=None):
    KH, KW = mod.kernel_size
    Ho = (H + 2 * pad - KH) // stride + 1
    Wo = (W + 2 * pad - KW) // stride + 1
    Wt = store.w(mod.weight)
    Wgt = store.g(mod.weight)
    Wt = Wt.view(G, Wt.shape[1], -1)
    Wgt = Wgt.view(G, Wgt.shape[1], -1)
    b = store.w(mod.bias, compute=False).view(G, -1) if mod.bias is not None else None
    bg = store.g(mod.bias).view(G, -1) if mod.bias is not None else None
    geom = (G, NI, H, W, C, KH, KW, stride, pad, Ho, Wo, nchw)
    return ConvF.apply(x, Wt, Wgt, b, bg, geom, mod.weight, x2, dtap), Ho, Wo


def _heads(t, GB, N, heads, D, off=0):
    G, M, W = t.shape
    rs = t.stride(1)
    assert t.stride(2) == 1 and t.stride(0) == M * rs and M == (GB // G) * N, (t.shape, t.stride(), GB, N)
    return t.as_strided((GB, heads, N, D), (N * rs, D, rs, 1), t.storage_offset() + off)


def _cross_attn_fwd(u, kv, B, N, heads, D):
    G, M, C = u.shape
    GB = G * B
    kh, vh = _heads(kv, GB, N, heads, D), _heads(kv, GB, N, heads, D, C)
    KV = torch.empty(GB, heads, D, D, dtype=torch.float32, device=u.device)
    K.gemm_h2(kh.transpose(2, 3), vh.transpose(2, 3), KV, out_mode=1)
    P = torch.empty(GB, heads, D, D, dtype=torch.float32, device=u.device)
    ctxT = torch.empty(GB, heads, D, D, dtype=u.dtype, device=u.device)
    K.call("cmx_ffm_ctx_fwd", KV, P, ctxT, G, B, heads, D, D ** -0.5, K.dtype_code(u))
    out = torch.empty(G, M, C, dtype=u.dtype, device=u.device)
    K.gemm_h2(_heads(u, GB, N, heads, D), ctxT, _heads(out, GB, N, heads, D))
    return out, P, ctxT


def _cross_attn_bwd(dout, u, kv, P, ctxT, B, N, heads, D, du):
    G, M, C = u.shape
    GB = G * B
    dout = _c(dout)
    doh = _heads(dout, GB, N, heads, D)
    K.gemm_h2(doh, ctxT.transpose(2, 3), _heads(du, GB, N, heads, D))
    dctx = torch.empty(GB, heads, D, D, dtype=torch.float32, device=u.device)
    K.gemm_h2(_heads(u, GB, N, heads, D).transpose(2, 3), doh.transpose(2, 3), dctx, out_mode=1)
    dA = torch.empty(GB, heads, D, D, dtype=u.dtype, device=u.device)
    K.call("cmx_ffm_ctx_bwd", P, dctx, dA, G, B, heads, D, D ** -0.5, K.dtype_code(u))
    dkv = torch.empty(G, M, 2 * C, dtype=kv.dtype, device=kv.device)
    kh, vh = _heads(kv, GB, N, heads, D), _heads(kv, GB, N, heads, D, C)
    K.gemm_h2(vh, dA, _heads(dkv, GB, N, heads, D))
    K.gemm_h2(kh, dA.transpose(2, 3), _heads(dkv, GB, N, heads, D, C))
    return dkv


class CrossAttentionF(Function):

    @staticmethod
    def forward(ctx, u, kv, B, N, heads, D):
        out, P, ctxT = _cross_attn_fwd(u, kv, B, N, heads, D)
        ctx.save_for_backward(u, kv, P, ctxT)
        ctx.meta = (B, N, heads, D)
        return out

    @staticmethod
    def backward(ctx, dout):
        u, kv, P, ctxT = ctx.saved_tensors
        B, N, heads, D = ctx.meta
        du = torch.empty_like(u)
        dkv = _cross_attn_bwd(dout, u, kv, P, ctxT, B, N, heads, D, du)
        return du, dkv, None, None, None, None


def _stacked_w(store, p):
    W = store.w(p)
    return W.view(W.shape[0], W.shape[1], -1)


def _stacked_g(store, p):
    Wg = store.g(p)
    return Wg.view(Wg.shape[0], Wg.shape[1], -1)


class CrossPathF(Function):

    @staticmethod
    def forward(ctx, x, Wcp, Wgcp, bcp, bgcp, Wkv, Wgkv, Wend, Wgend, bend, bgend, B, N, heads, anchor):
        G, M, C = x.shape
        D = C // heads
        a = torch.empty(G, M, 2 * C, dtype=x.dtype, device=x.device)
        _fwd_gemm(x, Wcp, bcp, a, act="relu")
        y, u = a[..., :C], a[..., C:]
        kv = torch.empty(G, M, 2 * C, dtype=x.dtype, device=x.device)
        _fwd_gemm(u, Wkv, None, kv)
        v, P, ctxT = _cross_attn_fwd(u, kv, B, N, heads, D)
        e = torch.empty(G, M, C, dtype=x.dtype, device=x.device)
        _fwd_gemm(y, Wend, bend, e, res=x, x2=v)
        ctx.save_for_backward(x, a, kv, v, P, ctxT, Wcp, Wkv, Wend)
        ctx.meta = (Wgcp, bgcp, Wgkv, Wgend, bgend, B, N, heads, D)
        return e

    @staticmethod
    def backward(ctx, de):
        x, a, kv, v, P, ctxT, Wcp, Wkv, Wend = ctx.saved_tensors
        Wgcp, bgcp, Wgkv, Wgend, bgend, B, N, heads, D = ctx.meta
        G, M, C = x.shape
        de = _c(de)
        y, u = a[..., :C], a[..., C:]
        da = torch.empty(G, M, 2 * C, dtype=x.dtype, device=x.device)
        dy, du = da[..., :C], da[..., C:]
        dv = torch.empty_like(v)
        _gemm_group([dict(A=de, B=Wend[:, :, :C].transpose(1, 2), C=dy, mask=y),
                     dict(A=de, B=Wend[:, :, C:].transpose(1, 2), C=dv)])
        _wgrad_into(de, y, Wgend[:, :, :C], bgend)
        _wgrad_into(de, v, Wgend[:, :, C:])
        dkv = _cross_attn_bwd(dv, u, kv, P, ctxT, B, N, heads, D, du)
        K.gemm(dkv, Wkv.transpose(1, 2), du, residual=du, mask=u)
        _wgrad_into(dkv, u, Wgkv)
        dz = da
        dx = torch.empty_like(x)
        K.gemm(dz, Wcp.transpose(1, 2), dx, residual=de)
        _wgrad_into(dz, x, Wgcp, bgcp)
        return (dx,) + (None,) * 14


def cross_path(store, cp, x, B, N, heads):
    w = lambda p: _stacked_w(store, p)
    g = lambda p: _stacked_g(store, p)
    G = x.shape[0]
    pj, kvm, ep = cp.channel_proj1, cp.cross_attn.kv1, cp.end_proj1
    return CrossPathF.apply(x, w(pj.weight), g(pj.weight), store.w(pj.bias, compute=False).view(G, -1),
                            store.g(pj.bias).view(G, -1), w(kvm.weight), g(kvm.weight), w(ep.weight), g(ep.weight),
                            store.w(ep.bias, compute=False).view(G, -1), store.g(ep.bias).view(G, -1), B, N, heads,
                            pj.weight)


class PairEmbedF(Function):

    @staticmethod
    def forward(ctx, o, Wres, Wgres, Wce, Wgce, bce, bgce, anchor):
        _, M, C = o.shape
        res = torch.empty(1, M, C, dtype=o.dtype, device=o.device)
        t = torch.empty(1, M, Wce.shape[1], dtype=o.dtype, device=o.device)
        _gemm_group([dict(A=o[0:1], B=Wres, C=res, A2=o[1:2]),
                     dict(A=o[0:1], B=Wce, C=t, bias=bce, A2=o[1:2])])
        ctx.save_for_backward(o, Wres, Wce)
        ctx.meta = (Wgres, Wgce, bgce)
        return res, t

    @staticmethod
    def backward(ctx, dres, dt):
        o, Wres, Wce = ctx.saved_tensors
        Wgres, Wgce, bgce = ctx.meta
        _, M, C = o.shape
        dres, dt = _c(dres), _c(dt)
        do = torch.empty_like(o)

        def halves(W):
            return W[0].view(W.shape[1], 2, C).permute(1, 0, 2)
        K.gemm(dres.expand(2, M, dres.shape[2]), halves(Wres).transpose(1, 2), do)
        K.gemm(dt.expand(2, M, dt.shape[2]), halves(Wce).transpose(1, 2), do, residual=do)
        _wgrad_into(dres, o[0:1], Wgres[:, :, :C])
        _wgrad_into(dres, o[1:2], Wgres[:, :, C:])
        _wgrad_into(dt, o[0:1], Wgce[:, :, :C], bgce)
        _wgrad_into(dt, o[1:2], Wgce[:, :, C:])
        return (do,) + (None,) * 7


def pair_embed(store, ce, o):
    w = lambda p: _stacked_w(store, p)
    g = lambda p: _stacked_g(store, p)
    c0 = ce.channel_embed[0]
    return PairEmbedF.apply(o, w(ce.residual.weight), g(ce.residual.weight), w(c0.weight), g(c0.weight),
                            store.w(c0.bias, compute=False).view(1, -1), store.g(c0.bias).view(1, -1),
                            ce.residual.weight)


_POOL_TK: dict = {}


def pool_tickets(owner, x, B, C):
    return K.tickets(_POOL_TK, "cmx_frm_pool_tickets", owner, x, B, C)


FRM_PROBE = None


class FRMF(Function):

    @staticmethod
    def forward(ctx, x, prm, anchor):
        (W1, b1, W2, b2, W0, b0, w2s, b2s) = prm["w"]
        G, B, N, C = x.shape
        dt = K.dtype_code(x)
        pooled, argmax = K.frm_pool_fwd(x, pool_tickets(anchor, x, B, C))
        y1 = K.small_linear_fwd(pooled, W1, b1, 4 * C, "relu")
        cw = K.small_linear_fwd(y1, W2, b2, 2 * C, "sigmoid")
        if FRM_PROBE is not None:
            FRM_PROBE[id(anchor)] = y1.detach().clone()
        h = torch.empty(1, B * N, C, dtype=x.dtype, device=x.device)
        K.gemm(x[0].view(1, B * N, C), W0[None], h, bias=b0[None], A2=x[1].view(1, B * N, C))
        h = h[0]
        sw = torch.empty(B * N, 2, dtype=torch.float32, device=x.device)
        out = torch.empty_like(x)
        K.call("cmx_frm_combine_fwd", x, cw, h, w2s, b2s, sw, out, B, N, C, dt)
        ctx.save_for_backward(x, pooled, argmax, y1, cw, h, sw)
        ctx.prm = prm
        ctx.set_materialize_grads(False)
        return out, out.view_as(out)

    @staticmethod
    def backward(ctx, dout, dout2):
        x, pooled, argmax, y1, cw, h, sw = ctx.saved_tensors
        (W1, b1, W2, b2, W0, b0, w2s, b2s) = ctx.prm["w"]
        (gW1, gb1, gW2, gb2, gW0, gb0, gw2s, gb2s) = ctx.prm["g"]
        G, B, N, C = x.shape
        dt = K.dtype_code(x)
        if dout is None:
            dout, dout2 = dout2, None
        if dout is None:
            return None, None, None
        dout = _c(dout)
        dout2 = _c(dout2) if dout2 is not None else None
        dx = torch.empty_like(x)
        dh = torch.empty_like(h)
        nb = K.query("cmx_frm_combine_bwd_nblk", N, C, dt)
        ws = K._ws(K.query("cmx_frm_combine_bwd_workspace", B, N, C, dt), x.device)
        K.call("cmx_frm_combine_bwd", dout, dout2, x, cw, sw, h, w2s, dx, dh, ws, B, N, C, dt)
        psp = ws[B * nb * 2 * C:B * nb * 2 * C + B * nb * (2 * C + 2)]
        if deferred.ENABLED:
            deferred.reduce(psp, gw2s, gb2s, 1, B * nb, 0, 2 * C + 2, 1, 2 * C + 2, 2 * C, 0, 0, 0, 0)
        else:
            tmp = torch.empty(2 * C + 2, dtype=torch.float32, device=x.device)
            K.partials_sum(psp, tmp, 1, B * nb, 2 * C + 2)
            gw2s.view(-1).copy_(tmp[:2 * C])
            gb2s.view(-1).copy_(tmp[2 * C:])
        Wd = W0.view(C, 2, C).permute(1, 0, 2)
        dx2 = dx.view(2, B * N, C)
        K.gemm(dh[None].expand(2, B * N, C), Wd.transpose(1, 2), dx2, residual=dx2)
        _wgrad_into(dh[None], x[0].view(1, B * N, C), gW0[None, :, :C], gb0.view(1, C))
        _wgrad_into(dh[None], x[1].view(1, B * N, C), gW0[None, :, C:])
        ns = K.query("cmx_small_linear_nslice")
        if B * -(-2 * C // ns) * nb <= 8192:
            dcw, nsl, ss, sm = ws, nb, 2 * C, nb * 2 * C
        else:
            dcw, nsl, ss, sm = torch.empty(B, 2 * C, dtype=torch.float32, device=x.device), 1, 0, 2 * C
            K.partials_sum(ws, dcw, B, nb, 2 * C)
        dy1p = K.small_linear_bwd(dcw, nsl, ss, sm, cw, y1, W2, gW2, gb2, 2 * C, "sigmoid")
        dpp = K.small_linear_bwd(dy1p, ns, B * 4 * C, 4 * C, y1, pooled, W1, gW1, gb1, 4 * C, "relu")
        K.frm_pool_bwd(dpp, argmax, dx)
        return dx, None, None


def frm(store, mod, x):
    cwm, swm = mod.channel_weights.mlp, mod.spatial_weights.mlp
    C = x.shape[-1]
    f32 = lambda p: store.w(p, stacked=False, compute=False)
    cmp = lambda p: store.w(p, stacked=False)
    g = lambda p: store.g(p, stacked=False)
    prm = {
        "w": (f32(cwm[0].weight), f32(cwm[0].bias), f32(cwm[2].weight), f32(cwm[2].bias),
              cmp(swm[0].weight).view(C, 2 * C), f32(swm[0].bias), f32(swm[2].weight).view(2, C), f32(swm[2].bias)),
        "g": (g(cwm[0].weight), g(cwm[0].bias), g(cwm[2].weight), g(cwm[2].bias),
              g(swm[0].weight).view(C, 2 * C), g(swm[0].bias), g(swm[2].weight).view(2, C), g(swm[2].bias)),
    }
    return FRMF.apply(x, prm, cwm[0].weight)


def sync_bn_sums(sums: torch.Tensor, count: float, group) -> float:
    if group is None:
        return count
    import torch.distributed as dist
    dist.all_reduce(sums, group=group)
    return count * dist.get_world_size(group)


BN_SMALL_M = int(os.environ.get("CMX_BN_SMALL_M", "600"))


class BatchNormF(Function):
    @staticmethod
    def forward(ctx, x, res, prm, training, act, dscale, rps, group, anchor):
        gamma, beta, gg, bg, rm, rv, eps, momentum = prm
        M, C = x.shape
        dt = K.dtype_code(x)
        mean = torch.empty(C, dtype=torch.float32, device=x.device)
        invstd = torch.empty(C, dtype=torch.float32, device=x.device)
        count = float(M)
        ctx.small = training and group is None and M <= BN_SMALL_M and C % 16 == 0
        y = torch.empty_like(x)
        if ctx.small:
            sums = torch.empty(2, C, dtype=torch.float64, device=x.device)
            K.call("cmx_bn_small_fwd", x, res, gamma, beta, dscale, y, sums, mean, invstd, rm, rv, M, C, rps,
                   K.ACT[act], eps, momentum, dt)
        elif training:
            sums, ws = K.bn_scratch(M, C, x.device)
            if group is None:
                K.call("cmx_bn_stats_finalize", x, sums, ws, M, C, eps, momentum, rm, rv, mean, invstd, dt)
            else:
                K.call("cmx_bn_stats", x, sums, ws, M, C, dt)
                count = sync_bn_sums(sums, count, group)
                K.call("cmx_bn_finalize", sums, count, eps, momentum, rm, rv, mean, invstd, C, 1)
        else:
            K.call("cmx_bn_finalize", None, 1.0, eps, momentum, rm, rv, mean, invstd, C, 0)
        if not ctx.small:
            K.call("cmx_bn_apply", x, mean, invstd, gamma, beta, res, dscale, y, M, C, rps, K.ACT[act], dt)
        ctx.save_for_backward(x, res if res is not None else x, mean, invstd)
        ctx.meta = (prm, training, act, dscale, rps, group, count, res is not None)
        return y

    @staticmethod
    def backward(ctx, dy):
        x, res, mean, invstd = ctx.saved_tensors
        prm, training, act, dscale, rps, group, count, has_res = ctx.meta
        gamma, beta, gg, bg, rm, rv, eps, momentum = prm
        res = res if has_res else None
        M, C = x.shape
        dt = K.dtype_code(x)
        dy = _c(dy)
        dx = torch.empty_like(x)
        dres = torch.empty_like(x) if has_res else None
        if ctx.small:
            K.call("cmx_bn_small_bwd", dy, x, mean, invstd, gamma, beta, res, dscale, gg, bg, dx, dres, M, C, rps,
                   K.ACT[act], 0, dt)
            return dx, dres, None, None, None, None, None, None, None
        sums, ws = K.bn_scratch(M, C, x.device)
        K.call("cmx_bn_bwd_reduce", dy, x, mean, invstd, gamma, beta, res, dscale, sums, gg, bg, ws, M, C, rps,
               K.ACT[act], 0, dt)
        if training:
            sync_bn_sums(sums, count, group)
        K.call("cmx_bn_bwd_apply", dy, x, mean, invstd, gamma, beta, res, dscale, sums, count, dx, dres, M, C, rps,
               K.ACT[act], training, dt)
        return dx, dres, None, None, None, None, None, None, None


def batchnorm(store, bn, x, training, res=None, act="none", dscale=None, rps=1, group=None):
    prm = (store.w(bn.weight, stacked=False, compute=False), store.w(bn.bias, stacked=False, compute=False),
           store.g(bn.weight, stacked=False), store.g(bn.bias, stacked=False), bn.running_mean, bn.running_var,
           float(bn.eps), float(bn.momentum))
    if training and not getattr(bn, "_nbt_shared", False):
        bn.num_batches_tracked.add_(1)
    return BatchNormF.apply(x, res, prm, training, act, dscale, rps, group, bn.weight)


_SE_TK: dict = {}


def se_tickets(owner, x, B, C):
    return K.tickets(_SE_TK, "cmx_se_pool_tickets", owner, x, B, C, least=1)


class SEGateF(Function):

    @staticmethod
    def forward(ctx, y, prm, dscale, anchor):
        (W1, b1, W2, b2) = prm["w"]
        B, N, C = y.shape
        H = W1.shape[0]
        dt = K.dtype_code(y)
        pooled = torch.empty(B, C, dtype=torch.float32, device=y.device)
        ws = K._ws(K.query("cmx_se_pool_workspace", B, N, C), y.device)
        K.call("cmx_se_pool_fwd", y, pooled, ws, se_tickets(anchor, y, B, C), B, N, C, dt)
        z1 = K.small_linear_fwd(pooled, W1, b1, H)
        h1 = K.act_fwd(z1, "gelu")
        a = K.small_linear_fwd(h1, W2, b2, C, "sigmoid")
        out = torch.empty_like(y)
        K.call("cmx_se_scale_fwd", y, a, dscale, out, B, N, C, dt)
        ctx.save_for_backward(y, a, z1, pooled)
        ctx.meta = (prm, dscale)
        return out

    @staticmethod
    def backward(ctx, dout):
        y, a, z1, pooled = ctx.saved_tensors
        prm, dscale = ctx.meta
        (W1, b1, W2, b2) = prm["w"]
        (gW1, gb1, gW2, gb2) = prm["g"]
        B, N, C = y.shape
        H = W1.shape[0]
        dt = K.dtype_code(y)
        f32 = dict(dtype=torch.float32, device=y.device)
        dout = _c(dout)
        nda = K.query("cmx_se_bwd_nslice", B, N, C)
        dap = torch.empty(nda, B, C, **f32)
        K.call("cmx_se_bwd_reduce", dout, y, dscale, dap, B, N, C, dt)
        h1 = K.act_fwd(z1, "gelu")
        dh1p = K.small_linear_bwd(dap, nda, B * C, C, a, h1, W2, gW2, gb2, C, "sigmoid")
        dh1 = K.partials_sum(dh1p, torch.empty(B, H, **f32), 1, dh1p.shape[0], B * H)
        dz1 = K.act_bwd(dh1, z1, "gelu")
        dpp = K.small_linear_bwd(dz1, 1, 0, H, z1, pooled, W1, gW1, gb1, H)
        dy = torch.empty_like(y)
        K.call("cmx_se_bwd_apply", dout, a, dscale, dpp, dpp.shape[0], B * C, dy, B, N, C, dt)
        return dy, None, None, None


def se_gate(store, att, y, dscale=None):
    f32 = lambda p: store.w(p, stacked=False, compute=False)
    g = lambda p: store.g(p, stacked=False)
    c1, c2 = att[1], att[3]
    prm = {"w": (f32(c1.weight), f32(c1.bias), f32(c2.weight), f32(c2.bias)),
           "g": (g(c1.weight), g(c1.bias), g(c2.weight), g(c2.bias))}
    return SEGateF.apply(y, prm, dscale, c1.weight)


class DilatedConv3F(Function):

    @staticmethod
    def forward(ctx, geom, Ws, Wgs, a0, a1, a2, x0, x1, x2):
        B, h, w, rates = geom
        xs = (x0, x1, x2)
        ys = tuple(torch.empty_like(x) for x in xs)
        K.easpp_conv("cmx_easpp_conv_fwd", xs, Ws, ys, B, h, w, rates)
        ctx.save_for_backward(*xs)
        ctx.meta = (geom, Ws, Wgs)
        return ys

    @staticmethod
    def backward(ctx, *dys):
        xs = ctx.saved_tensors
        (B, h, w, rates), Ws, Wgs = ctx.meta
        dys = tuple(_c(d) for d in dys)
        dxs = tuple(torch.empty_like(x) for x in xs)
        K.easpp_conv("cmx_easpp_conv_dgrad", dys, Ws, dxs, B, h, w, rates)
        K.easpp_conv_wgrad(dys, xs, Wgs, B, h, w, rates)
        return (None,) * 6 + dxs


def dilated_conv3(store, convs, xs, B, h, w):
    Ws = tuple(store.w(c.weight, stacked=False) for c in convs)
    Wgs = tuple(store.g(c.weight, stacked=False) for c in convs)
    geom = (B, h, w, tuple(int(c.dilation[0]) for c in convs))
    return DilatedConv3F.apply(geom, Ws, Wgs, *(c.weight for c in convs), *xs)


class PooledConvF(Function):

    @staticmethod
    def forward(ctx, x, W, Wg, B, N, anchor):
        x = _c(x)
        C = x.shape[-1]
        pooled = torch.empty(B, C, dtype=torch.float32, device=x.device)
        ws = K._ws(K.query("cmx_se_pool_workspace", B, N, C), x.device)
        K.call("cmx_se_pool_fwd", x, pooled, ws, se_tickets(anchor, x, B, C), B, N, C, K.dtype_code(x))
        z = K.small_linear_fwd(pooled, W, None, W.shape[0])
        ctx.save_for_backward(pooled, z, W)
        ctx.meta = (Wg, B, N, x.dtype)
        return z

    @staticmethod
    def backward(ctx, dz):
        pooled, z, W = ctx.saved_tensors
        Wg, B, N, dtype = ctx.meta
        C, Cout = pooled.shape[1], W.shape[0]
        dpp = K.small_linear_bwd(_c(dz), 1, 0, Cout, z, pooled, W, Wg, None, Cout)
        dx = torch.empty(B * N, C, dtype=dtype, device=dz.device)
        K.call("cmx_easpp_pool_bwd", dpp, dpp.shape[0], B * C, dx, B, N, C, K.dtype_code(dx))
        return dx, None, None, None, None, None


def pooled_conv(store, conv, x, B, N):
    return PooledConvF.apply(x, store.w(conv.weight, stacked=False, compute=False),
                             store.g(conv.weight, stacked=False), B, N, conv.weight)


class EasppConcatF(Function):

    @staticmethod
    def forward(ctx, y0, y1, y2, y3, pool, B, N):
        y0, y1, y2, y3, pool = (_c(t) for t in (y0, y1, y2, y3, pool))
        Cm = y0.shape[-1]
        cat = torch.empty(B * N, 5 * Cm, dtype=y0.dtype, device=y0.device)
        K.call("cmx_easpp_concat_fwd", y0, y1, y2, y3, pool, cat, B, N, Cm, K.dtype_code(y0))
        ctx.meta = (B, N, Cm)
        return cat

    @staticmethod
    def backward(ctx, dcat):
        B, N, Cm = ctx.meta
        dcat = _c(dcat)
        ds = tuple(torch.empty(B * N, Cm, dtype=dcat.dtype, device=dcat.device) for _ in range(4))
        dpool = torch.empty(B, Cm, dtype=torch.float32, device=dcat.device)
        K.call("cmx_easpp_concat_bwd", dcat, *ds, dpool, B, N, Cm, K.dtype_code(dcat))
        return (*ds, dpool, None, None)


def easpp_dropout_scale(state, n, p, device):
    scale = torch.empty(n, dtype=torch.float32, device=device)
    K.call("cmx_easpp_dropout_mask", scale, n, float(p), state[0], state[1])
    return scale


class AsppConv3F(Function):

    @staticmethod
    def forward(ctx, geom, Ws, Wgs, a0, a1, a2, x):
        B, h, w, rates = geom
        if x.stride(-1) != 1:
            x = x.contiguous()
        ctx.save_for_backward(x)
        ctx.meta = (geom, Ws, Wgs)
        return K.aspp_conv_fwd(x, Ws, B, h, w, rates)

    @staticmethod
    def backward(ctx, *dys):
        x, = ctx.saved_tensors
        (B, h, w, rates), Ws, Wgs = ctx.meta
        dys = tuple(_c(d) for d in dys)
        dx = K.aspp_conv_dgrad(dys, Ws, B, h, w, rates) if ctx.needs_input_grad[6] else None
        K.aspp_conv_wgrad(dys, x, Wgs, B, h, w, rates)
        return (None,) * 6 + (dx,)


def aspp_conv3(store, convs, x, B, h, w):
    Ws = tuple(store.w(c.weight, stacked=False) for c in convs)
    Wgs = tuple(store.g(c.weight, stacked=False) for c in convs)
    geom = (B, h, w, tuple(int(c.dilation[0]) for c in convs))
    return AsppConv3F.apply(geom, Ws, Wgs, *(c.weight for c in convs), x)


class UpcatAcF(Function):

    @staticmethod
    def forward(ctx, lo, skip, dims):
        B, h, w, H, W = dims
        lo, skip = _c(lo), _c(skip)
        ctx.meta = (dims, lo.shape[-1], skip.shape[-1])
        return K.upcat_ac_fwd(lo, skip, B, h, w, H, W)

    @staticmethod
    def backward(ctx, dcat):
        (B, h, w, H, W), C, Cs = ctx.meta
        dlo, dskip = K.upcat_ac_bwd(_c(dcat), B, h, w, H, W, C, Cs)
        return dlo, dskip, None


def _adjoint_to(dZ, B, H1, W1, h, w, E):
    tmp = torch.empty(B * H1, w, E, dtype=torch.float32, device=dZ.device)
    K.bilinear_adjoint_1d(dZ, tmp, B * H1, W1, w, E, W1 * E, E)
    g = torch.empty(B, h * w, E, dtype=dZ.dtype, device=dZ.device)
    return K.bilinear_adjoint_1d(tmp, g, B, H1, h, w * E, H1 * w * E, w * E)


class DecoderFuseF(Function):

    SLOTS = (0, 1, 2, 3)

    @staticmethod
    def forward(ctx, e4, e3, e2, e1, Wf, Wfg, bf, bfg, sizes, anchor):
        return _decoder_fuse_fwd(ctx, DecoderFuseF.SLOTS, e4, e3, e2, e1, Wf, Wfg, bf, bfg, sizes)

    @staticmethod
    def backward(ctx, dZ):
        return _decoder_fuse_bwd(ctx, dZ)


class DecoderFuseC1F(DecoderFuseF):
    SLOTS = (3, 2, 1, 0)

    @staticmethod
    def forward(ctx, e4, e3, e2, e1, Wf, Wfg, bf, bfg, sizes, anchor):
        return _decoder_fuse_fwd(ctx, DecoderFuseC1F.SLOTS, e4, e3, e2, e1, Wf, Wfg, bf, bfg, sizes)


def _decoder_fuse_fwd(ctx, slots, e4, e3, e2, e1, Wf, Wfg, bf, bfg, sizes):
    B, N1, E = e1.shape
    (H1, W1), hw = sizes[0], sizes[1:]
    W = Wf[0]
    zs, jobs = [], []
    for j, (e, (h, w)) in enumerate(zip((e4, e3, e2), (hw[2], hw[1], hw[0]))):
        slot = slots[j]
        z = torch.empty(1, B * h * w, E, dtype=e.dtype, device=e.device)
        jobs.append(dict(A=e.reshape(1, B * h * w, E), B=W[None, :, slot * E:(slot + 1) * E], C=z))
        zs.append(z)
    _gemm_group(jobs)
    Z = K.decoder_fuse_fwd(_c(e1), W[:, slots[3] * E:(slots[3] + 1) * E], bf, zs, H1, W1, hw)
    ctx.save_for_backward(e4, e3, e2, e1, Wf)
    ctx.meta = (Wfg, bfg, sizes, slots)
    return Z


def _decoder_fuse_bwd(ctx, dZ):
    e4, e3, e2, e1, Wf = ctx.saved_tensors
    Wfg, bfg, sizes, slots = ctx.meta
    B, N1, E = e1.shape
    (H1, W1), hw = sizes[0], sizes[1:]
    dZ = _c(dZ).view(1, B * N1, E)
    grads, jobs = [], []
    for j, (e, (h, w)) in enumerate(zip((e4, e3, e2), (hw[2], hw[1], hw[0]))):
        dz = _adjoint_to(dZ, B, H1, W1, h, w, E).view(1, B * h * w, E)
        sl = slice(slots[j] * E, (slots[j] + 1) * E)
        g = torch.empty_like(dz)
        jobs.append(dict(A=dz, B=Wf[:, :, sl].transpose(1, 2), C=g))
        grads.append(g.view(e.shape))
        _wgrad_into(dz, e.reshape(1, B * h * w, E), Wfg[:, :, sl])
    e1f = e1.reshape(1, B * N1, E)
    de1 = torch.empty_like(e1f)
    s1 = slice(slots[3] * E, (slots[3] + 1) * E)
    jobs.append(dict(A=dZ, B=Wf[:, :, s1].transpose(1, 2), C=de1))
    _wgrad_into(dZ, e1f, Wfg[:, :, s1], bfg)
    _gemm_group(jobs)
    return grads[0], grads[1], grads[2], de1.view(e1.shape), None, None, None, None, None, None


DECODER_FOLD = os.environ.get("CMX_DECODER_FOLD", "1") != "0"
DECODER_UP3 = os.environ.get("CMX_DECODER_UP3", "0") == "1"
DECODER_ADJ3 = os.environ.get("CMX_DECODER_ADJ3", "1") != "0"


def _up3_ok(E, ws):
    return DECODER_UP3 and E % 64 == 0 and sum(ws) <= 160


def _adj3_ok(E, W1, ws, dtype):
    cs, esz = (64, 4) if dtype == torch.float32 else (128, 2)
    if not DECODER_ADJ3 or E % cs:
        return False
    taps = sum(w * ((2 * W1 + w - 1) // w + 3) for w in ws)
    return (2 * taps + 3) // 4 * 16 + W1 * cs * esz <= 65536


class DecoderFoldF(Function):

    SLOTS = (0, 1, 2, 3)

    @staticmethod
    def forward(ctx, x4, x3, x2, x1, Wf, Wc, bf, bc, grads, sizes, anchor):
        return _decoder_fold_fwd(ctx, DecoderFoldF.SLOTS, x4, x3, x2, x1, Wf, Wc, bf, bc, grads, sizes)

    @staticmethod
    def backward(ctx, dZ):
        return _decoder_fold_bwd(ctx, dZ)


class DecoderFoldC1F(DecoderFoldF):
    SLOTS = (3, 2, 1, 0)

    @staticmethod
    def forward(ctx, x4, x3, x2, x1, Wf, Wc, bf, bc, grads, sizes, anchor):
        return _decoder_fold_fwd(ctx, DecoderFoldC1F.SLOTS, x4, x3, x2, x1, Wf, Wc, bf, bc, grads, sizes)


def _decoder_fold_fwd(ctx, slots, x4, x3, x2, x1, Wf, Wc, bf, bc, grads, sizes):
    B, N1, C1 = x1.shape
    E = Wf.shape[0]
    (H1, W1), hw = sizes[0], sizes[1:]
    xs = (x4, x3, x2, x1)
    Cs = [w.shape[1] for w in Wc]
    Ms = [torch.empty(1, E, C, dtype=Wf.dtype, device=Wf.device) for C in Cs]
    _gemm_group([dict(A=Wf[None, :, s * E:(s + 1) * E], B=Wc[s][None].transpose(1, 2), C=Ms[s], splitk=1)
                 for s in range(4)])
    b = torch.empty(E, dtype=torch.float32, device=Wf.device)
    K.call("cmx_decoder_fold_bias", Wf, Wf.stride(0), bf, *bc, b, E, K.dtype_code(Wf))
    zs, jobs = [], []
    for j, (h, w) in enumerate((hw[2], hw[1], hw[0])):
        s = slots[j]
        z = torch.empty(1, B * h * w, E, dtype=x1.dtype, device=x1.device)
        jobs.append(dict(A=_c(xs[j]).reshape(1, B * h * w, Cs[s]), B=Ms[s], C=z))
        zs.append(z)
    _gemm_group(jobs)
    if _up3_ok(E, [w for (_, w) in hw]):
        Z = torch.empty(B * N1, E, dtype=x1.dtype, device=x1.device)
        U = torch.empty(1, B * N1, E, dtype=x1.dtype, device=x1.device)
        K.call("cmx_bilinear_up3_add", zs[0], zs[1], zs[2], B, *hw[2], *hw[1], *hw[0], b, U, H1, W1, E,
               K.dtype_code(x1))
        K.gemm(_c(x1).view(1, B * N1, C1), Ms[slots[3]], Z.view(1, B * N1, E), residual=U)
    else:
        Z = K.decoder_fuse_fwd(_c(x1), Ms[slots[3]][0], b, zs, H1, W1, hw)
    ctx.save_for_backward(*xs, Wf, *Wc, *Ms)
    ctx.meta = (bc, grads, sizes, _adj3_ok(E, W1, [w for (_, w) in hw], x1.dtype), slots)
    return Z


def _decoder_fold_bwd(ctx, dZ):
    t = ctx.saved_tensors
    xs, Wf, Wc, Ms = t[:4], t[4], t[5:9], t[9:13]
    bc, grads, sizes, adj3, slots = ctx.meta
    B, N1, C1 = xs[3].shape
    E = Wf.shape[0]
    (H1, W1), hw = sizes[0], sizes[1:]
    Cs = [w.shape[1] for w in Wc]
    dZ = _c(dZ).view(1, B * N1, E)
    offs = [0]
    for C in Cs:
        offs.append(offs[-1] + E * C)
    dM = torch.empty(offs[-1], dtype=torch.float32, device=dZ.device)
    gb = torch.empty(1, E, dtype=torch.float32, device=dZ.device)
    if adj3:
        dYs = [torch.empty(1, B * h * w, E, dtype=dZ.dtype, device=dZ.device) for (h, w) in (hw[2], hw[1], hw[0])]
        ts = [torch.empty(B * H1 * w * E, dtype=torch.float32, device=dZ.device) for (h, w) in (hw[2], hw[1], hw[0])]
        K.call("cmx_bilinear_adjoint3", dZ, *ts, *dYs, B, H1, W1, *hw[2], *hw[1], *hw[0], E, K.dtype_code(dZ))
    dxs, jobs = [], []
    for j in range(4):
        s = slots[j]
        if j == 3:
            dY = dZ
        elif adj3:
            dY = dYs[j]
        else:
            dY = _adjoint_to(dZ, B, H1, W1, *hw[2 - j], E).view(1, -1, E)
        x = xs[j].reshape(1, -1, Cs[s])
        dx = torch.empty_like(x)
        jobs.append(dict(A=dY, B=Ms[s].transpose(1, 2), C=dx))
        dxs.append(dx.view(xs[j].shape))
        _wgrad_into(dY, x, dM[offs[s]:offs[s + 1]].view(1, E, Cs[s]), gb if j == 3 else None)
    _gemm_group(jobs)
    deferred.after(lambda: _decoder_fold_chain(dM, gb, offs, Wf, Wc, bc, grads, Cs, E))
    return (*dxs, None, None, None, None, None, None, None)


def _decoder_fold_chain(dM, gb, offs, Wf, Wc, bc, grads, Cs, E):
    Wfg, bfg, Wcg, bcg = grads
    h16 = Wf.dtype != torch.float32
    dMh = torch.empty(dM.shape, dtype=Wf.dtype, device=dM.device) if h16 else None
    WfT = torch.empty(4 * E, E, dtype=Wf.dtype, device=Wf.device)
    K.call("cmx_decoder_fold_bwd_prep", dM, dMh, dM.numel(), gb, Wf, Wf.stride(0), WfT, Wfg, Wfg.stride(-2), *bc, *bcg,
           bfg, E, K.dtype_code(Wf))
    src = dMh if h16 else dM
    D = [src[offs[s]:offs[s + 1]].view(1, E, Cs[s]) for s in range(4)]
    _gemm_group([dict(A=D[s], B=Wc[s][None], C=Wfg[:, :, s * E:(s + 1) * E], out_mode=2, splitk=1) for s in range(4)])
    _gemm_group([dict(A=WfT[None, s * E:(s + 1) * E], B=D[s].transpose(1, 2), C=Wcg[s], out_mode=1, splitk=1)
                 for s in range(4)])


def _scale_adjoint(ctx, adj, dloss, out):
    dl = torch.empty(ctx.lshape, dtype=ctx.ldtype, device=adj.device)
    K.call("cmx_upsample_ce_bwd_scale", adj, dloss, out, dl, dl.numel(), K.dtype_code(dl))
    return dl


class UpsampleCEF(Function):

    @staticmethod
    def forward(ctx, logits, label, dims, ignore):
        B, h, w, H, W, Kc = dims
        fused = H == 4 * h and W == 4 * w and Kc <= 40
        logits = _c(logits)
        grad = None if fused else torch.empty(B, H, W, Kc, dtype=logits.dtype, device=logits.device)
        out = torch.empty(3, dtype=torch.float32, device=logits.device)
        ws = K._ws(K.query("cmx_upsample_ce_workspace", B, H, W), logits.device)
        if fused and ctx.needs_input_grad[0]:
            adj = torch.empty(B, h * w, Kc, dtype=torch.float32, device=logits.device)
            K.call("cmx_upsample_ce_fwd_adj", logits, label, adj, out, ws, B, h, w, H, W, Kc, ignore,
                   K.dtype_code(logits))
            ctx.save_for_backward(adj, out, label)
            ctx.fused, ctx.ldtype, ctx.lshape = "adj", logits.dtype, logits.shape
            return out[0]
        K.call("cmx_upsample_ce_fwd", logits, label, grad, out, ws, B, h, w, H, W, Kc, ignore, K.dtype_code(logits))
        ctx.save_for_backward(logits if fused else grad, out, label)
        ctx.fused = fused
        ctx.dims = dims
        ctx.ldtype = logits.dtype
        ctx.lshape = logits.shape
        return out[0]

    @staticmethod
    def backward(ctx, dloss):
        grad, out, label = ctx.saved_tensors
        dloss = _c(dloss.reshape(1).to(torch.float32))
        if ctx.fused == "adj":
            return _scale_adjoint(ctx, grad, dloss, out), None, None, None
        B, h, w, H, W, Kc = ctx.dims
        tmp = torch.empty(B * H, w, Kc, dtype=torch.float32, device=grad.device)
        K.bilinear_adjoint_1d(grad, tmp, B * H, W, w, Kc, W * Kc, Kc)
        dl = torch.empty(B, h * w, Kc, dtype=ctx.ldtype, device=grad.device)
        K.bilinear_adjoint_1d(tmp, dl, B, H, h, w * Kc, H * w * Kc, w * Kc, a1=dloss, a2=out[1:])
        return dl.view(ctx.lshape), None, None, None


LOSS_WCE, LOSS_FOCAL2D, LOSS_FOCAL = 0, 1, 2


class UpsampleLossF(Function):

    @staticmethod
    def forward(ctx, logits, label, dims, ignore, spec, weight):
        B, h, w, H, W, Kc = dims
        kind, gamma, alpha, ce_scale, focal_scale = spec
        logits = _c(logits)
        if weight is not None and (weight.device != logits.device or weight.dtype != torch.float32
                                   or weight.numel() != Kc or not weight.is_contiguous()):
            raise ValueError(f"class weight: {Kc} contiguous fp32 values on {logits.device} expected")
        out = torch.empty(3, dtype=torch.float32, device=logits.device)
        adj = torch.empty(B, h * w, Kc, dtype=torch.float32, device=logits.device)
        ws = K._ws(K.query("cmx_upsample_loss_workspace", B, h, w), logits.device)
        if K.refusable("cmx_upsample_loss_fwd_adj", (K.CMX_ERR_SHAPE,), logits, label, weight, adj, out, ws, B, h, w, H,
                       W, Kc, ignore, int(kind), float(gamma), float(alpha), float(ce_scale), float(focal_scale),
                       K.dtype_code(logits)) is K.REFUSED:
            raise NotImplementedError(f"fused upsample + loss: {K.last_error()}; only CrossEntropyLoss has a "
                                      "materialised path for other shapes")
        ctx.save_for_backward(adj, out)
        ctx.ldtype, ctx.lshape = logits.dtype, logits.shape
        return out[0]

    @staticmethod
    def backward(ctx, dloss):
        adj, out = ctx.saved_tensors
        dloss = _c(dloss.reshape(1).to(torch.float32))
        return _scale_adjoint(ctx, adj, dloss, out), None, None, None, None, None


class UpsampleDiceF(Function):

    @staticmethod
    def forward(ctx, logits, label, dims, ignore, spec):
        B, h, w, H, W, Kc = dims
        ce_scale, dice_scale, smooth = spec
        logits = _c(logits)
        f32 = dict(dtype=torch.float32, device=logits.device)
        out = torch.empty(3, **f32)
        stats = torch.empty(B, Kc, 3, **f32)
        adj = torch.empty(B, h * w, Kc, **f32) if ctx.needs_input_grad[0] else None
        ws = K._ws(K.query("cmx_upsample_dice_workspace", B, h, w, Kc), logits.device)
        if K.refusable("cmx_upsample_dice_fwd_adj", (K.CMX_ERR_SHAPE,), logits, label, adj, out, stats, ws, B, h, w, H,
                       W, Kc, ignore, float(ce_scale), float(dice_scale), float(smooth),
                       K.dtype_code(logits)) is K.REFUSED:
            raise NotImplementedError(f"fused upsample + Dice loss: {K.last_error()}; only CrossEntropyLoss has "
                                      "a materialised path for other shapes")
        ctx.save_for_backward(adj, out)
        ctx.ldtype, ctx.lshape = logits.dtype, logits.shape
        return out[0]

    @staticmethod
    def backward(ctx, dloss):
        adj, out = ctx.saved_tensors
        dloss = _c(dloss.reshape(1).to(torch.float32))
        return _scale_adjoint(ctx, adj, dloss, out), None, None, None, None


class UpsampleOhemF(Function):

    last = None

    @staticmethod
    def forward(ctx, logits, label, dims, ignore, spec):
        B, h, w, H, W, Kc = dims
        thresh, min_kept = spec
        logits = _c(logits)
        f32 = dict(dtype=torch.float32, device=logits.device)
        out = torch.empty(4, **f32)
        py = torch.empty(B, H, W, **f32)
        counts = torch.empty(3, dtype=torch.int64, device=logits.device)
        adj = torch.empty(B, h * w, Kc, **f32)
        ws = K._ws(K.query("cmx_upsample_ohem_workspace", B, h, w), logits.device)
        if K.refusable("cmx_upsample_ohem_fwd_adj", (K.CMX_ERR_SHAPE,), logits, label, adj, out, py, counts, ws, B, h, w,
                       H, W, Kc, ignore, float(thresh), int(min_kept), K.dtype_code(logits)) is K.REFUSED:
            raise NotImplementedError(f"fused upsample + OHEM loss: {K.last_error()}; only CrossEntropyLoss has "
                                      "a materialised path for other shapes")
        UpsampleOhemF.last = (out, counts)
        ctx.save_for_backward(adj, out)
        ctx.ldtype, ctx.lshape = logits.dtype, logits.shape
        return out[0]

    @staticmethod
    def backward(ctx, dloss):
        adj, out = ctx.saved_tensors
        dloss = _c(dloss.reshape(1).to(torch.float32))
        return _scale_adjoint(ctx, adj, dloss, out), None, None, None, None


LOSS_CE = -1
LOSS_SCALES = (8, 16, 32)


class UpsampleScaledLossF(Function):

    @staticmethod
    def forward(ctx, logits, label, dims, ignore, spec, weight):
        B, h, w, H, W, Kc = dims
        S = H // h if h > 0 else 0
        if S not in LOSS_SCALES or H != S * h or W != S * w:
            raise NotImplementedError(f"fused upsample + loss at the scale of an FCN head: {h}x{w} -> {H}x{W} is not "
                                      f"an exact scale in {LOSS_SCALES}")
        kind, gamma, alpha, ce_scale, focal_scale = (LOSS_CE, 0.0, 0.0, 1.0, 0.0) if spec is None else spec
        logits = _c(logits)
        if weight is not None and (weight.device != logits.device or weight.dtype != torch.float32
                                   or weight.numel() != Kc or not weight.is_contiguous()):
            raise ValueError(f"class weight: {Kc} contiguous fp32 values on {logits.device} expected")
        out = torch.empty(3, dtype=torch.float32, device=logits.device)
        adj = torch.empty(B, h * w, Kc, dtype=torch.float32, device=logits.device)
        ws = K._ws(K.query("cmx_upsample_loss_scaled_workspace", B, h, w, S), logits.device)
        if K.refusable("cmx_upsample_loss_scaled_fwd_adj", (K.CMX_ERR_SHAPE,), logits, label, weight, adj, out, ws, B,
                       h, w, S, Kc, ignore, int(kind), float(gamma), float(alpha), float(ce_scale), float(focal_scale),
                       K.dtype_code(logits)) is K.REFUSED:
            raise NotImplementedError(f"fused upsample + loss at the scale of an FCN head: {K.last_error()}")
        if not ctx.needs_input_grad[0]:
            return out[0]
        ctx.save_for_backward(adj, out)
        ctx.ldtype, ctx.lshape = logits.dtype, logits.shape
        return out[0]

    @staticmethod
    def backward(ctx, dloss):
        adj, out = ctx.saved_tensors
        dloss = _c(dloss.reshape(1).to(torch.float32))
        return _scale_adjoint(ctx, adj, dloss, out), None, None, None, None, None


def upsample_logits_nchw(logits, B, h, w, H, W, Kc):
    out = torch.empty(B, Kc, H, W, dtype=torch.float32, device=logits.device)
    K.call("cmx_bilinear_fwd_nchw_f32", _c(logits), out, B, h, w, H, W, Kc, K.dtype_code(logits))
    return out
```

### rgbx_semantic_segmentation_amd/models/encoders/dual_segformer.py

```python
from __future__ import annotations

import math
from typing import List, Optional

import torch
import torch.nn as nn

from ... import functions as F
from ... import streams
from ..net_utils import (FeatureRectifyModule, FeatureFusionModule, ImprovedFeatureRectifyModule,
                         ImprovedFeatureFusionModule, init_segformer)

MIT_SPECS = {
    "mit_b0": dict(embed_dims=[32, 64, 160, 256], depths=[2, 2, 2, 2]),
    "mit_b1": dict(embed_dims=[64, 128, 320, 512], depths=[2, 2, 2, 2]),
    "mit_b2": dict(embed_dims=[64, 128, 320, 512], depths=[3, 4, 6, 3]),
    "mit_b3": dict(embed_dims=[64, 128, 320, 512], depths=[3, 4, 18, 3]),
    "mit_b4": dict(embed_dims=[64, 128, 320, 512], depths=[3, 8, 27, 3]),
    "mit_b5": dict(embed_dims=[64, 128, 320, 512], depths=[3, 6, 40, 3]),
}
NUM_HEADS = [1, 2, 5, 8]
SR_RATIOS = [8, 4, 2, 1]
MLP_RATIO = 4


def drop_path_probs(depths: List[int], rate: float):
    dpr = [x.item() for x in torch.linspace(0, rate, sum(depths))]
    out, cur = [], 0
    for s, d in enumerate(depths):
        if s == 1:
            out.append(([dpr[cur]] * d, [dpr[cur + 1]] * d))
        else:
            p = [dpr[cur + i] for i in range(d)]
            out.append((p, list(p)))
        cur += d
    return out


class DWConv(nn.Module):
    def __init__(self, dim):
        super().__init__()
        self.dwconv = nn.Conv2d(dim, dim, 3, 1, 1, bias=True, groups=dim)


class Mlp(nn.Module):
    def __init__(self, dim, hidden):
        super().__init__()
        self.fc1 = nn.Linear(dim, hidden)
        self.dwconv = DWConv(hidden)
        self.fc2 = nn.Linear(hidden, dim)


class Attention(nn.Module):
    def __init__(self, dim, num_heads, sr_ratio):
        super().__init__()
        self.num_heads = num_heads
        self.q = nn.Linear(dim, dim, bias=True)
        self.kv = nn.Linear(dim, 2 * dim, bias=True)
        self.proj = nn.Linear(dim, dim)
        self.sr_ratio = sr_ratio
        if sr_ratio > 1:
            self.sr = nn.Conv2d(dim, dim, sr_ratio, sr_ratio)
            self.norm = nn.LayerNorm(dim)


class Block(nn.Module):
    def __init__(self, dim, num_heads, sr_ratio, drop_path):
        super().__init__()
        self.norm1 = nn.LayerNorm(dim, eps=1e-6)
        self.attn = Attention(dim, num_heads, sr_ratio)
        self.drop_path_prob = drop_path
        self.norm2 = nn.LayerNorm(dim, eps=1e-6)
        self.mlp = Mlp(dim, dim * MLP_RATIO)


class OverlapPatchEmbed(nn.Module):
    def __init__(self, patch_size, stride, in_chans, embed_dim):
        super().__init__()
        self.proj = nn.Conv2d(in_chans, embed_dim, patch_size, stride, patch_size // 2)
        self.norm = nn.LayerNorm(embed_dim)
        self.stride = stride
        self.pad = patch_size // 2


def _conv_bn_relu(cin, cout, k=1, rate=1):
    return nn.Sequential(nn.Conv2d(cin, cout, k, padding=rate if k > 1 else 0, dilation=rate if k > 1 else 1,
                                   bias=False), nn.BatchNorm2d(cout), nn.ReLU(True))


class ASPPConv(nn.Module):
    def __init__(self, channels, rate):
        super().__init__()
        self.block = _conv_bn_relu(channels, channels, 3, rate)


class AsppPooling(nn.Module):
    def __init__(self, cin, cout):
        super().__init__()
        self.gap = nn.Sequential(nn.AdaptiveAvgPool2d(1), *_conv_bn_relu(cin, cout))


class eASPP(nn.Module):
    reduce_dim, middle_dim = 64, 256

    def __init__(self, channels, atrous_rates=(12, 24, 36)):
        super().__init__()
        r, m = self.reduce_dim, self.middle_dim
        self.input_conv = _conv_bn_relu(channels, m)
        for i, rate in enumerate(atrous_rates):
            setattr(self, f"branch{i + 1}", nn.ModuleList(
                [_conv_bn_relu(channels, r)] + [ASPPConv(r, rate) for _ in range(3)] + [_conv_bn_relu(r, m)]))
        self.img_pooling = AsppPooling(channels, m)
        self.project = nn.Sequential(*_conv_bn_relu(5 * m, channels), nn.Dropout(0.5))

    def dropout_scale(self, n, device, mask=None):
        p = self.project[3].p
        if p <= 0:
            return None
        if mask is not None:
            return (mask.to(device=device, dtype=torch.float32).reshape(-1) / (1 - p)).contiguous()
        device = torch.device(device)
        st = self.__dict__.get("_mask_state")
        if st is None or st[1].device.type != device.type or device.index not in (None, st[1].device.index):
            if device.type == "cuda" and torch.cuda.is_current_stream_capturing():
                raise RuntimeError("eASPP: the dropout mask's device step counter must exist before a graph capture: "
                                   "run one eager training step first")
            seed = int(torch.randint(0, 2 ** 62, (1,)).item())
            st = self.__dict__["_mask_state"] = (seed, torch.zeros(2, dtype=torch.int64, device=device))
        return F.easpp_dropout_scale(st, n, p, device)

    def run(self, store, x, B, h, w, training, mask=None):
        M, N = B * h * w, h * w
        if training and B == 1:
            raise ValueError("eASPP: training needs more than 1 image per batch: the pooled branch's BatchNorm sees "
                             "one value per channel (as torch.nn.BatchNorm2d refuses)")
        br = (self.branch1, self.branch2, self.branch3)

        def unit(seq, t, **kw):
            return F.batchnorm(store, seq[1], t, training, act="relu", **kw)

        xg = x.view(1, M, -1)
        ys = F.glinear_multi(store, [(u[0].weight, None, xg) for u in (self.input_conv, *(b[0] for b in br))])
        x_in = unit(self.input_conv, ys[0].view(M, -1))
        t = [unit(b[0], y.view(M, -1)) for b, y in zip(br, ys[1:])]
        for d in (1, 2, 3):
            t = F.dilated_conv3(store, [b[d].block[0] for b in br], t, B, h, w)
            t = [unit(b[d].block, y) for b, y in zip(br, t)]
        ys = F.glinear_multi(store, [(b[4][0].weight, None, y.view(1, M, -1)) for b, y in zip(br, t)])
        outs = [unit(b[4], y.view(M, -1)) for b, y in zip(br, ys)]
        gap = self.img_pooling.gap
        pool = F.batchnorm(store, gap[2], F.pooled_conv(store, gap[1], x, B, N), training, act="relu")
        cat = F.EasppConcatF.apply(x_in, *outs, pool, B, N)
        y = F.glinear(store, self.project[0].weight, None, cat.view(1, M, -1)).view(M, -1)
        scale = self.dropout_scale(y.numel(), y.device, mask) if training else None
        return unit(self.project, y, dscale=scale, rps=1)


class RGBXTransformer(nn.Module):
    def __init__(self, embed_dims, depths, drop_path_rate=0.1, frm="FRM", ffm="FFM", aspp=False):
        super().__init__()
        self.embed_dims, self.depths = list(embed_dims), list(depths)
        self.dp = drop_path_probs(depths, drop_path_rate)
        cins = [3] + list(embed_dims[:3])
        for pre in ("", "extra_"):
            for s in range(4):
                k, st = (7, 4) if s == 0 else (3, 2)
                setattr(self, f"{pre}patch_embed{s + 1}", OverlapPatchEmbed(k, st, cins[s], embed_dims[s]))
        for s in range(4):
            for pre, probs in (("", self.dp[s][0]), ("extra_", self.dp[s][1])):
                setattr(self, f"{pre}block{s + 1}", nn.ModuleList(
                    [Block(embed_dims[s], NUM_HEADS[s], SR_RATIOS[s], probs[i]) for i in range(depths[s])]))
                setattr(self, f"{pre}norm{s + 1}", nn.LayerNorm(embed_dims[s], eps=1e-6))
        rect = FeatureRectifyModule if frm == "FRM" else ImprovedFeatureRectifyModule
        fuse = FeatureFusionModule if ffm == "FFM" else ImprovedFeatureFusionModule
        self.FRMs = nn.ModuleList([rect(d) for d in embed_dims])
        self.FFMs = nn.ModuleList([fuse(d, NUM_HEADS[s]) for s, d in enumerate(embed_dims)])
        if aspp:
            self.single_aspp = eASPP(embed_dims[3], atrous_rates=(12, 24, 36))
        self.apply(init_segformer)

    def drop_path_keep_probs(self):
        rows = []
        for s in range(4):
            for i in range(self.depths[s]):
                rows.append((1.0 - self.dp[s][0][i], 1.0 - self.dp[s][1][i]))
        return rows

    def run_block(self, store, blk: Block, x, B, H, W, s_attn, s_mlp, prev=(None, None), tail=None,
                  next_norm=None):
        G, M, C = x.shape
        N = H * W
        a = blk.attn
        stap = F.DgradTap() if (a.sr_ratio > 1 and F.ln_bwd_fusable(x, (H, W, a.sr_ratio))) else None
        h, h2, xr = F.layernorm_res(store, blk.norm1, x, G, scale=prev[0], rps=N, tap=prev[1], tail=tail, dtap=stap)

        if a.sr_ratio > 1:
            xs, Hk, Wk = F.conv(store, a.sr, h2, G, G * B, H, W, C, a.sr_ratio, 0, dtap=stap)
            xs, Nk = F.layernorm(store, a.norm, xs, G), Hk * Wk
        else:
            xs, Nk = h2, N
        q, kv = F.glinear_multi(store, [(a.q.weight, a.q.bias, h), (a.kv.weight, a.kv.bias, xs)])
        o = F.SRAttentionF.apply(q, kv, G * B, N, Nk, a.num_heads, C // a.num_heads)
        tap_a = F.GradTap() if s_attn is not None else None
        t2 = F.LNTail(blk.norm2)
        x = F.glinear(store, a.proj.weight, a.proj.bias, o, res=xr, rscale=s_attn, rps=N, tap=tap_a, ln_tail=t2)
        ltap = F.DgradTap() if F.ln_bwd_fusable(x) else None
        h, _, xr = F.layernorm_res(store, blk.norm2, x, G, scale=s_attn, rps=N, tap=tap_a, tail=t2, dtap=ltap)
        f = F.glinear(store, blk.mlp.fc1.weight, blk.mlp.fc1.bias, h, dgrad_tap=ltap)
        f = F.dwconv(store, blk.mlp.dwconv.dwconv, f, G * B, B, H, W, "gelu")
        tap_m = F.GradTap() if s_mlp is not None else None
        tn = F.LNTail(next_norm) if next_norm is not None else None
        x = F.glinear(store, blk.mlp.fc2.weight, blk.mlp.fc2.bias, f, res=xr, rscale=s_mlp, rps=N, tap=tap_m,
                      ln_tail=tn)
        return x, (s_mlp, tap_m), tn

    def run(self, store, images, B, H, W, training, dp_scales: Optional[torch.Tensor], bn_group=None, aspp_mask=None):
        neck = getattr(self, "single_aspp", None)

        def fuse(s, r, Hc, Wc):
            o = self.FFMs[s].run(store, r, B, Hc, Wc, training)
            if s == 3 and neck is not None:
                o = neck.run(store, o, B, Hc, Wc, training, mask=aspp_mask)
            return o

        G = 2
        x2 = None
        if isinstance(images, (tuple, list)):
            x, x2 = images
        else:
            x = images
        outs, grids = [], []
        bi = 0
        Hc, Wc, Cin = H, W, 3
        sync = getattr(self, "grad_sync", None)
        main = torch.cuda.current_stream() if x.is_cuda else None
        side = streams.ffm_stream(main.device) if (main is not None and streams.FFM_SIDE) else None
        for s in range(4):
            pe = getattr(self, f"patch_embed{s + 1}")
            if sync is not None and s > 0 and x.requires_grad:
                x.register_hook(sync.segment_hook(3 - s))
            if s == 0:
                x, Ho, Wo = F.patch_embed1(store, pe, x, G, G * B, Hc, Wc, x2=x2)
            else:
                x, Ho, Wo = F.conv(store, pe.proj, x, G, G * B, Hc, Wc, Cin, pe.stride, pe.pad)
                x = F.layernorm(store, pe.norm, x, G)
            Hc, Wc, Cin = Ho, Wo, self.embed_dims[s]
            prev = (None, None)
            blocks = getattr(self, f"block{s + 1}")
            snorm = getattr(self, f"norm{s + 1}")
            tail = None
            for i, blk in enumerate(blocks):
                sa = sm = None
                if dp_scales is not None:
                    sa, sm = dp_scales[bi, 0], dp_scales[bi, 1]
                nxt = blocks[i + 1].norm1 if i + 1 < len(blocks) else snorm
                x, prev, tail = self.run_block(store, blk, x, B, Hc, Wc, sa, sm, prev, tail=tail, next_norm=nxt)
                bi += 1
            x, _, _ = F.layernorm_res(store, snorm, x, G, scale=prev[0], rps=Hc * Wc, tap=prev[1], tail=tail)
            C = self.embed_dims[s]
            fr = self.FRMs[s]
            if isinstance(fr, ImprovedFeatureRectifyModule):
                r = rn = fr.rectify(store, x.view(G, B, Hc * Wc, C), training)
            else:
                r, rn = F.frm(store, fr, x.view(G, B, Hc * Wc, C))
            if side is not None:
                side.wait_stream(main)
                r.record_stream(side)
                with torch.cuda.stream(side):
                    outs.append(fuse(s, r, Hc, Wc))
            else:
                outs.append(fuse(s, r, Hc, Wc))
            grids.append((Hc, Wc))
            x = rn.view(G, B * Hc * Wc, C)
        if side is not None:
            main.wait_stream(side)
            for o in outs:
                o.record_stream(main)
        return outs, grids


class mit_b0(RGBXTransformer):
    def __init__(self, fuse_cfg=None, frm="FRM", ffm="FFM", **kwargs):
        super().__init__(**MIT_SPECS["mit_b0"], drop_path_rate=0.1, frm=frm, ffm=ffm)


class mit_b1(RGBXTransformer):
    def __init__(self, fuse_cfg=None, frm="FRM", ffm="FFM", **kwargs):
        super().__init__(**MIT_SPECS["mit_b1"], drop_path_rate=0.1, frm=frm, ffm=ffm)


class mit_b2(RGBXTransformer):
    def __init__(self, fuse_cfg=None, frm="FRM", ffm="FFM", **kwargs):
        super().__init__(**MIT_SPECS["mit_b2"], drop_path_rate=0.1, frm=frm, ffm=ffm)


class mit_b3(RGBXTransformer):
    def __init__(self, fuse_cfg=None, frm="FRM", ffm="FFM", **kwargs):
        super().__init__(**MIT_SPECS["mit_b3"], drop_path_rate=0.1, frm=frm, ffm=ffm)


class mit_b4(RGBXTransformer):
    def __init__(self, fuse_cfg=None, frm="FRM", ffm="FFM", **kwargs):
        super().__init__(**MIT_SPECS["mit_b4"], drop_path_rate=0.1, frm=frm, ffm=ffm)


class mit_b5(RGBXTransformer):
    def __init__(self, fuse_cfg=None, frm="FRM", ffm="FFM", **kwargs):
        super().__init__(**MIT_SPECS["mit_b5"], drop_path_rate=0.1, frm=frm, ffm=ffm)


BACKBONES = {"mit_b0": mit_b0, "mit_b1": mit_b1, "mit_b2": mit_b2, "mit_b3": mit_b3, "mit_b4": mit_b4,
             "mit_b5": mit_b5}


def _with_ef_aspp(name):
    spec = MIT_SPECS[name]

    class Net(RGBXTransformer):
        def __init__(self, fuse_cfg=None, frm="FRM", ffm="FFM", **kwargs):
            super().__init__(**spec, drop_path_rate=0.1, frm=frm, ffm=ffm, aspp=True)

    Net.__name__ = Net.__qualname__ = f"{name}_w_ef_aspp"
    return Net


for _name in list(MIT_SPECS):
    MIT_SPECS[f"{_name}_w_ef_aspp"] = MIT_SPECS[_name]
    BACKBONES[f"{_name}_w_ef_aspp"] = _with_ef_aspp(_name)


def load_dualpath_model(model: nn.Module, model_file):
    raw = torch.load(model_file, map_location="cpu", weights_only=True) if isinstance(model_file, str) \
        else model_file
    if "model" in raw:
        raw = raw["model"]
    sd = {}
    for k, v in raw.items():
        if "patch_embed" in k:
            sd[k] = v
            sd[k.replace("patch_embed", "extra_patch_embed")] = v
        elif "block" in k:
            sd[k] = v
            sd[k.replace("block", "extra_block")] = v
        elif "norm" in k:
            sd[k] = v
            sd[k.replace("norm", "extra_norm")] = v
    return model.load_state_dict(sd, strict=False)
```

### rgbx_semantic_segmentation_amd/roofline.py

```python
from __future__ import annotations

import glob
import json
import os

import torch

from . import deferred, _lib
from .floor import step_work

PEAK_BF16_TFLOPS = 2516.6
PEAK_HBM_GBS = 8000.0
_ROOT = os.path.dirname(os.path.dirname(os.path.abspath(__file__)))


RIDGE_FLOP_PER_BYTE = PEAK_BF16_TFLOPS * 1e12 / (PEAK_HBM_GBS * 1e9)


def _pmc_traffic(kernel: str, workload: str, blocks: int):
    for path in sorted(glob.glob(os.path.join(_ROOT, "profiles", "*pmc*.json")), reverse=True):
        try:
            d = json.load(open(path))
        except (OSError, ValueError):
            continue
        if d.get("workload") != workload:
            continue
        k = d.get("kernels", {}).get(kernel)
        if k and k.get("hbm_bytes_per_launch") and k.get("blocks") in (None, blocks):
            return k["hbm_bytes_per_launch"], os.path.relpath(path, _ROOT)
    return None, None


GEMM_FAMILY = ("cmx_gemm", "cmx_gemm_ln", "cmx_gemm_multi", "cmx_conv_implicit_fwd", "cmx_decoder_fuse_fwd",
               "cmx_conv_patch_dgrad", "cmx_gemm_ln_bwd", "cmx_conv_patch_dgrad_ln_bwd")


def _family_traffic(kernels, workload: str):
    for path in sorted(glob.glob(os.path.join(_ROOT, "profiles", "*pmc*.json")), reverse=True):
        try:
            d = json.load(open(path))
        except (OSError, ValueError):
            continue
        if d.get("workload") != workload:
            continue
        ks = [d.get("kernels", {}).get(k) for k in kernels]
        ks = [k for k in ks if k and k.get("hbm_bytes_per_launch") and k.get("launches")]
        if ks:
            n = sum(k["launches"] for k in ks)
            return sum(k["hbm_bytes_per_launch"] * k["launches"] for k in ks) / n, os.path.relpath(path, _ROOT)
    return None, None


FAMILY_RE = (
    ("easpp", r"easpp_"),
    ("wgrad", r"gemm_grouped_kernel|reduce_grouped_kernel"),
    ("gemm", r"gemm_bf16_kernel|gemm_stream|gemm_multi|gemm_generic|splitk_reduce"),
    ("sra", r"sra_"),
    ("dwconv", r"dw2_|dw_"),
    ("layernorm", r"ln_fwd|ln_bwd|rowln"),
    ("adamw", r"adamw"),
    ("batchnorm", r"bn_"),
    ("frm", r"pool_|linear_fwd|linear_bwd|combine_|frm_|reduce_partials"),
    ("ffm", r"ffm_"),
    ("ce", r"ce_|upsample|loss_cells|loss_finalize"),
    ("bilinear", r"bilinear|adj3_|up3_"),
    ("im2col", r"im2col|col2im"),
    ("pe1", r"pe1_"),
)


def family_of(kernel: str) -> str:
    import re
    for fam, rx in FAMILY_RE:
        if re.search(rx, kernel):
            return fam
    return "other"


def trace_kernels(run_step, steps: int):
    from torch.profiler import profile, ProfilerActivity
    torch.cuda.synchronize()
    with profile(activities=[ProfilerActivity.CUDA]) as prof:
        for _ in range(steps):
            run_step()
        torch.cuda.synchronize()
    out = []
    for e in prof.profiler.kineto_results.events():
        if e.device_type() != torch.autograd.DeviceType.CUDA:
            continue
        name = e.name()
        if "Memcpy" in name or "Memset" in name:
            continue
        out.append((name, e.start_ns() / 1e3, e.duration_ns() / 1e3))
    out.sort(key=lambda r: r[1])
    return out


STEP_FIRST = "step_masks_kernel"


def split_steps(recs):
    idx = [i for i, r in enumerate(recs) if STEP_FIRST in r[0]]
    if not idx:
        return []
    segs = [recs[a:b] for a, b in zip(idx, idx[1:] + [len(recs)])]
    full = max(len(sg) for sg in segs)
    return [sg for sg in segs if len(sg) == full]


def measure_in_step(run_step, workload: str, shape: dict, n_params: float, steps: int = 10,
                    step_us: float | None = None):
    recs = trace_kernels(run_step, steps)
    if not recs:
        return None, None
    segs = split_steps(recs)
    if segs:
        recs = [r for sg in segs for r in sg]
        steps = len(segs)
    work = step_work(n_params=n_params, **shape)
    fams = {}
    for name, _, us in recs:
        f = fams.setdefault(family_of(name), [0.0, 0])
        f[0] += us
        f[1] += 1
    busy = sum(v[0] for v in fams.values()) / steps
    scale = (step_us / busy) if step_us else 1.0

    def fam_s(us_total):
        return us_total / steps * scale * 1e-6

    table = {}
    for fam, (us, n) in sorted(fams.items(), key=lambda kv: -kv[1][0]):
        t = fam_s(us)
        fl, by = work[fam] if fam in work else (0.0, 0.0)
        row = {"us_per_step": round(t * 1e6, 1), "profiled_us_per_step": round(us / steps, 1),
               "launches_per_step": round(n / steps, 1), "share_of_busy": round(us / steps / busy, 4)}
        if by:
            row.update({"alg_gb": round(by / 1e9, 4), "tbs": round(by / t / 1e12, 3),
                        "hbm_frac": round(by / t / (PEAK_HBM_GBS * 1e9), 4)})
        if fl:
            row.update({"alg_gflop": round(fl / 1e9, 2), "mfma_frac": round(fl / t / (PEAK_BF16_TFLOPS * 1e12), 4)})
        table[fam] = row
    dom = max((f for f in fams if f in work and work[f][1] > 0), key=lambda f: fams[f][0])
    us, n = fams[dom]
    t = fam_s(us)
    nl = n / steps
    flops, nbytes = work[dom]
    hbm = flops / nbytes < RIDGE_FLOP_PER_BYTE
    gbs, tflops = nbytes / t / 1e9, flops / t / 1e12
    kern = {"gemm": ("gemm_bf16_kernel", "gemm_stream_kernel", "gemm_multi_kernel", "splitk_reduce_kernel"),
            "wgrad": ("gemm_grouped_kernel",)}.get(dom, ())
    traffic, src = _family_traffic(kern, workload) if kern else (None, None)
    roof = {"kernel": f"{dom} family in the replayed step ({nl:.0f} launches per step; kernel trace of {steps} "
                      f"HIP-graph replays)",
            "family": dom, "bound": "hbm" if hbm else "mfma",
            "achieved": round(gbs, 1) if hbm else round(tflops, 2),
            "peak": PEAK_HBM_GBS if hbm else PEAK_BF16_TFLOPS,
            "unit": "GB/s" if hbm else "TFLOP/s",
            "frac": round(gbs / PEAK_HBM_GBS if hbm else tflops / PEAK_BF16_TFLOPS, 4),
            "traffic": traffic,
            "arithmetic_intensity_flop_per_byte": round(flops / nbytes, 1),
            "ridge_flop_per_byte": round(RIDGE_FLOP_PER_BYTE, 1),
            "achieved_tflops": round(tflops, 2), "mfma_frac": round(tflops / PEAK_BF16_TFLOPS, 4),
            "achieved_hbm_gbs": round(gbs, 1), "hbm_frac": round(gbs / PEAK_HBM_GBS, 4),
            "launches": round(nl, 1), "avg_launch_us": round(t / nl * 1e6, 2), "total_us": round(t * 1e6, 1),
            "algorithmic_flop_per_launch": flops / nl, "algorithmic_bytes_per_launch": nbytes / nl,
            "algorithmic_bytes_per_step": nbytes, "workload": workload,
            "timing": f"in-step: kernel durations of {steps} complete replayed steps (torch.profiler / roctracer "
                      f"activity records, steps cut at {STEP_FIRST}), summed per family and divided by {steps}"
                      + (f"; the family's share of that kernel time x the timed step ({step_us:.0f} us)"
                         if step_us else "")}
    if src:
        roof["traffic_source"] = src
        roof["traffic_over_algorithmic"] = round(traffic / (nbytes / nl), 3)
    walls = [sg[-1][1] + sg[-1][2] - sg[0][1] for sg in segs] if segs else []
    if step_us:
        roof["profiled_us"] = round(us / steps, 1)
    return roof, {"busy_us_per_step": round(busy, 1), "launches_per_step": round(len(recs) / steps, 1),
                  "complete_steps_traced": steps if segs else None,
                  "wall_us_per_step_median": round(sorted(walls)[len(walls) // 2], 1) if walls else None,
                  "families": table}


def measure_gemm_family(model, batch, workload: str, shape: dict, warm: int = 4, iters: int = 16):
    import torch as _t
    rgb, x, lab = batch
    timings = []

    def obs(name, fn, args):
        if name not in GEMM_FAMILY:
            return
        for _ in range(warm):
            fn(*args)
        e0, e1 = _t.cuda.Event(enable_timing=True), _t.cuda.Event(enable_timing=True)
        e0.record()
        for _ in range(iters):
            fn(*args)
        e1.record()
        timings.append((name, e0, e1))

    _lib.observer = obs
    try:
        loss = model(rgb, x, lab)
        loss.backward()
    finally:
        _lib.observer = None
    _t.cuda.synchronize()
    if not timings:
        return None
    per = [e0.elapsed_time(e1) / iters * 1e-3 for _, e0, e1 in timings]
    t = sum(per)
    flops, nbytes = step_work(**shape)["gemm"]
    n = len(per)
    traffic, src = _family_traffic(("gemm_bf16_kernel", "gemm_stream_kernel", "gemm_multi_kernel", "splitk_reduce_kernel"),
                                  workload)
    gbs, tflops = nbytes / t / 1e9, flops / t / 1e12
    hbm = flops / nbytes < RIDGE_FLOP_PER_BYTE
    out = {"kernel": f"tile-GEMM family: gemm_bf16_kernel / gemm_multi_kernel / splitk_reduce_kernel ({n} forward and "
                     f"input-gradient launches per step: every Linear, 1x1 / implicit conv, decoder fuse product)",
           "bound": "hbm" if hbm else "mfma",
           "achieved": round(gbs, 1) if hbm else round(tflops, 2),
           "peak": PEAK_HBM_GBS if hbm else PEAK_BF16_TFLOPS,
           "unit": "GB/s" if hbm else "TFLOP/s",
           "frac": round(gbs / PEAK_HBM_GBS if hbm else tflops / PEAK_BF16_TFLOPS, 4),
           "traffic": traffic,
           "arithmetic_intensity_flop_per_byte": round(flops / nbytes, 1),
           "ridge_flop_per_byte": round(RIDGE_FLOP_PER_BYTE, 1),
           "achieved_tflops": round(tflops, 2), "mfma_frac": round(tflops / PEAK_BF16_TFLOPS, 4),
           "achieved_hbm_gbs": round(gbs, 1), "hbm_frac": round(gbs / PEAK_HBM_GBS, 4),
           "launches": n, "avg_launch_us": round(t / n * 1e6, 2), "total_us": round(t * 1e6, 1),
           "by_entry_point_us": {k: round(sum(p for (nm, _, _), p in zip(timings, per) if nm == k) * 1e6, 1)
                                 for k in GEMM_FAMILY if any(nm == k for nm, _, _ in timings)},
           "algorithmic_flop_per_launch": flops / n, "algorithmic_bytes_per_launch": nbytes / n,
           "algorithmic_bytes_per_step": nbytes, "workload": workload,
           "timing": f"each launch re-issued in place {warm} + {iters} times; HIP events around the {iters}"}
    if src:
        out["traffic_source"] = src
    return out


def measure_dominant(model, batch, workload: str, iters: int = 20):
    rgb, x, lab = batch
    seen = []

    def obs(dev, nrec, blk, work, keep, dcode=1):
        seen.append((dev, nrec, blk, list(work), list(keep), dcode))

    deferred.observer = obs
    try:
        loss = model(rgb, x, lab)
        loss.backward()
    finally:
        deferred.observer = None
    torch.cuda.synchronize()
    if not seen:
        return None
    flops = nbytes = t = 0.0
    blk = nrec = 0
    for dev, nr, bl, work, keep, dcode in seen:
        for (G, M, Nr, K) in work:
            flops += 2.0 * G * M * Nr * K
            nbytes += 2.0 * G * (M + Nr) * K + 4.0 * G * M * Nr
        launch = lambda: _lib.call("cmx_gemm_grouped", dev, nr, bl, dcode)
        for _ in range(3):
            launch()
        s, e = torch.cuda.Event(enable_timing=True), torch.cuda.Event(enable_timing=True)
        torch.cuda.synchronize()
        s.record()
        for _ in range(iters):
            launch()
        e.record()
        torch.cuda.synchronize()
        t += s.elapsed_time(e) / iters * 1e-3
        blk += bl
        nrec += nr
    n = len(seen)
    traffic, src = _pmc_traffic("gemm_grouped_kernel", workload, blk // n)
    tflops, gbs = flops / t / 1e12, nbytes / t / 1e9
    ai = flops / nbytes
    hbm = ai < RIDGE_FLOP_PER_BYTE
    out = {"kernel": f"gemm_grouped_kernel (all {nrec} weight-gradient GEMM problems of the backward in {n} grouped "
                     f"launches, {blk} workgroups)",
           "bound": "hbm" if hbm else "mfma",
           "achieved": round(gbs, 1) if hbm else round(tflops, 2),
           "peak": PEAK_HBM_GBS if hbm else PEAK_BF16_TFLOPS,
           "unit": "GB/s" if hbm else "TFLOP/s",
           "frac": round(gbs / PEAK_HBM_GBS if hbm else tflops / PEAK_BF16_TFLOPS, 4),
           "traffic": traffic,
           "arithmetic_intensity_flop_per_byte": round(ai, 1), "ridge_flop_per_byte": round(RIDGE_FLOP_PER_BYTE, 1),
           "achieved_tflops": round(tflops, 2), "mfma_frac": round(tflops / PEAK_BF16_TFLOPS, 4),
           "achieved_hbm_gbs": round(gbs, 1), "hbm_frac": round(gbs / PEAK_HBM_GBS, 4),
           "launches": n, "avg_launch_us": round(t / n * 1e6, 2), "total_us": round(t * 1e6, 1),
           "algorithmic_flop_per_launch": flops / n, "algorithmic_bytes_per_launch": nbytes / n, "workload": workload}
    if src:
        out["traffic_source"] = src
    del seen
    return out
```

Measured before the change: 292.3.

## Fuse MLP fc1 GEMM into dwconv forward and fc2 dgrad into dwconv backward

Result: faster. 297.2 (median of 6 runs) (+1.7%).

```diff
diff --git a/include/cmx_mlp.h b/include/cmx_mlp.h
--- /dev/null
+++ b/include/cmx_mlp.h
@@ -0,0 +1,14 @@
+#ifndef CMX_MLP_H
+#define CMX_MLP_H
+#include "cmx_hip.h"
+#ifdef __cplusplus
+extern "C" {
+#endif
+
+int cmx_mlp_fc1_dwconv_fwd(const void* x, const void* W1, const float* b1, const float* w, const float* b, void* f0, void* out, void* gprime, int NI, int imgs_per_group, int H, int W, int C, int hidden, int act, int dtype, hipStream_t stream);
+int cmx_mlp_fc2_dwconv_bwd(const void* dz, const void* W2, const void* h, const void* gprime, const float* w, void* dh, float* dw, float* db, float* workspace, int NI, int imgs_per_group, int H, int W, int C, int hidden, int accumulate, int dtype, hipStream_t stream);
+
+#ifdef __cplusplus
+}
+#endif
+#endif
diff --git a/rgbx_semantic_segmentation_amd/_lib.py b/rgbx_semantic_segmentation_amd/_lib.py
--- a/rgbx_semantic_segmentation_amd/_lib.py
+++ b/rgbx_semantic_segmentation_amd/_lib.py
@@ -14,6 +14,7 @@
 EASPP_HEADER_PATHS = [os.path.join(_HERE, "..", "include", "cmx_easpp.h"), os.path.join(_HERE, "cmx_easpp.h")]
 FCN_HEADER_PATHS = [os.path.join(_HERE, "..", "include", "cmx_fcn.h"), os.path.join(_HERE, "cmx_fcn.h")]
 DEEPLAB_HEADER_PATHS = [os.path.join(_HERE, "..", "include", "cmx_deeplab.h"), os.path.join(_HERE, "cmx_deeplab.h")]
+MLP_HEADER_PATHS = [os.path.join(_HERE, "..", "include", "cmx_mlp.h"), os.path.join(_HERE, "cmx_mlp.h")]
 
 
 class CMXError(RuntimeError):
@@ -87,16 +88,17 @@
     easpp = parse_header(next(p for p in EASPP_HEADER_PATHS if os.path.exists(p)))
     fcn = parse_header(next(p for p in FCN_HEADER_PATHS if os.path.exists(p)))
     deeplab = parse_header(next(p for p in DEEPLAB_HEADER_PATHS if os.path.exists(p)))
-    for table in (sigs, ohem, easpp, fcn, deeplab):
+    mlp = parse_header(next(p for p in MLP_HEADER_PATHS if os.path.exists(p)))
+    for table in (sigs, ohem, easpp, fcn, deeplab, mlp):
         for name, (rt, argt) in table.items():
             fn = getattr(lib, name)
             fn.argtypes = argt
             fn.restype = rt
             assert STREAM not in table[name].kinds[:-1], f"{name}: hipStream_t must be the last parameter"
-    return lib, sigs, ohem, easpp, fcn, deeplab
+    return lib, sigs, ohem, easpp, fcn, deeplab, mlp
 
 
-LIB, SIGNATURES, OHEM_SIGNATURES, EASPP_SIGNATURES, FCN_SIGNATURES, DEEPLAB_SIGNATURES = _load()
+LIB, SIGNATURES, OHEM_SIGNATURES, EASPP_SIGNATURES, FCN_SIGNATURES, DEEPLAB_SIGNATURES, MLP_SIGNATURES = _load()
 
 
 def last_error() -> str:
@@ -124,7 +126,7 @@
 _BOUND = {name: (getattr(LIB, name), tuple(_pointer_arg if k == POINTER else _scalar_arg for k in sig.kinds),
                  sig.kinds[-1:] == (STREAM,))
           for name, sig in {**SIGNATURES, **OHEM_SIGNATURES, **EASPP_SIGNATURES, **FCN_SIGNATURES,
-                            **DEEPLAB_SIGNATURES}.items()}
+                            **DEEPLAB_SIGNATURES, **MLP_SIGNATURES}.items()}
 
 
 def marshal(name: str, args: tuple) -> tuple:
diff --git a/rgbx_semantic_segmentation_amd/csrc/dwconv.hip b/rgbx_semantic_segmentation_amd/csrc/dwconv.hip
--- a/rgbx_semantic_segmentation_amd/csrc/dwconv.hip
+++ b/rgbx_semantic_segmentation_amd/csrc/dwconv.hip
@@ -1,4 +1,6 @@
 #include "cmx_common.h"
+#include "cmx_mfma.h"
+#include "../../include/cmx_mlp.h"
 
 namespace {
 constexpr int RXF = 4;
@@ -344,7 +346,7 @@
   if constexpr (sizeof(T) == 2) *reinterpret_cast<uint2*>(p) = make_uint2(pack2<T>(o[0].x, o[0].y), pack2<T>(o[1].x, o[1].y));
   else *reinterpret_cast<float4*>(p) = make_float4(o[0].x, o[0].y, o[1].x, o[1].y);
 }
-template <typename T, int CB, int RY_, int RX_>
+template <typename T, int CB, int RY_, int RX_, int PITCH = CB>
 __device__ __forceinline__ void stage_region_pm(const T* __restrict__ base, T* img, int y0, int x0, int H, int W, int C) {
   constexpr int NCG = CB / 8, NPX = RY_ * RX_;
   constexpr int ITER = (NCG * NPX + 255) / 256;
@@ -360,7 +362,50 @@
 #pragma unroll
   for (int k = 0; k < ITER; ++k) {
     const int it = threadIdx.x + k * 256;
-    if (it < NCG * NPX) v8_store<T>(img + it * 8, v[k]);
+    if (it < NCG * NPX) v8_store<T>(img + (it / NCG) * PITCH + (it % NCG) * 8, v[k]);
+  }
+}
+
+template <typename T, int ACT, bool FLIP, int PITCH, bool COPY_IN>
+__device__ __forceinline__ void dw2_fwd_column(const T* hp, const cmx_f2 (&wr)[2][9], const cmx_f2 (&bias)[2],
+                                               T* __restrict__ out, T* __restrict__ gprime, T* __restrict__ hin,
+                                               long o, long ostep, int nr) {
+  cmx_f2 win[3][3][2];
+#pragma unroll
+  for (int j = 0; j < 3; ++j) {
+    v4_unpack<T>(v4_load<T>(hp + j * PITCH), win[0][j]);
+    v4_unpack<T>(v4_load<T>(hp + (EX + j) * PITCH), win[1][j]);
+  }
+#pragma unroll
+  for (int r = 0; r < TY2; ++r) {
+    if (r < nr) {
+#pragma unroll
+      for (int j = 0; j < 3; ++j) {
+        v4_unpack<T>(v4_load<T>(hp + ((r + 2) * EX + j) * PITCH), win[(r + 2) % 3][j]);
+      }
+      if constexpr (COPY_IN) {
+        *reinterpret_cast<V4<T>*>(hin + o) = v4_load<T>(hp + ((r + 1) * EX + 1) * PITCH);
+      }
+      cmx_f2 acc[2] = {bias[0], bias[1]};
+#pragma unroll
+      for (int i = 0; i < 3; ++i)
+#pragma unroll
+        for (int j = 0; j < 3; ++j) {
+          const int tap = FLIP ? 8 - (i * 3 + j) : i * 3 + j;
+#pragma unroll
+          for (int u = 0; u < 2; ++u) acc[u] = pk_fma(wr[u][tap], win[(r + i) % 3][j][u], acc[u]);
+        }
+      if (gprime) {
+        cmx_f2 gd[2];
+#pragma unroll
+        for (int u = 0; u < 2; ++u) gd[u] = act2_grad<ACT>(acc[u]);
+        v4_store<T>(gprime + o, gd);
+      }
+#pragma unroll
+      for (int u = 0; u < 2; ++u) acc[u] = act2_fwd<ACT>(acc[u]);
+      v4_store<T>(out + o, acc);
+      o += ostep;
+    }
   }
 }
 
@@ -390,43 +435,8 @@
     const int x = t.tx0 + pl;
     const int nr = H - t.ty0;
     if (x >= W) return;
-    const T* hp = hc + pl * CB;
-    cmx_f2 win[3][3][2];
-#pragma unroll
-    for (int j = 0; j < 3; ++j) {
-      v4_unpack<T>(v4_load<T>(hp + j * CB), win[0][j]);
-      v4_unpack<T>(v4_load<T>(hp + (EX + j) * CB), win[1][j]);
-    }
-    long o = ibase + ((long)t.ty0 * W + x) * C + cq * 4;
-    const long ostep = (long)W * C;
-#pragma unroll
-    for (int r = 0; r < TY2; ++r) {
-      if (r < nr) {
-#pragma unroll
-        for (int j = 0; j < 3; ++j) {
-          v4_unpack<T>(v4_load<T>(hp + ((r + 2) * EX + j) * CB), win[(r + 2) % 3][j]);
-        }
-        cmx_f2 acc[2] = {bias[0], bias[1]};
-#pragma unroll
-        for (int i = 0; i < 3; ++i)
-#pragma unroll
-          for (int j = 0; j < 3; ++j) {
-            const int tap = FLIP ? 8 - (i * 3 + j) : i * 3 + j;
-#pragma unroll
-            for (int u = 0; u < 2; ++u) acc[u] = pk_fma(wr[u][tap], win[(r + i) % 3][j][u], acc[u]);
-          }
-        if (gprime) {
-          cmx_f2 gd[2];
-#pragma unroll
-          for (int u = 0; u < 2; ++u) gd[u] = act2_grad<ACT>(acc[u]);
-          v4_store<T>(gprime + o, gd);
-        }
-#pragma unroll
-        for (int u = 0; u < 2; ++u) acc[u] = act2_fwd<ACT>(acc[u]);
-        v4_store<T>(out + o, acc);
-        o += ostep;
-      }
-    }
+    dw2_fwd_column<T, ACT, FLIP, CB, false>(hc + pl * CB, wr, bias, out, gprime, nullptr,
+                                            ibase + ((long)t.ty0 * W + x) * C + cq * 4, (long)W * C, nr);
   } else {
     for (int it = pl; it < TY2 * TX2; it += PPI) {
       const int r = it / TX2, c = it % TX2;
@@ -455,6 +465,102 @@
       v4_store<T>(out + o, acc);
     }
   }
+}
+
+constexpr int MLP_CB = 64, MLP_PM = MLP_CB + 8;
+
+template <typename T, int KC, int NCW, int D, typename Epi>
+__device__ __forceinline__ void mlp_chunk_stream(const typename MF<T>::frag (&fw)[KC / 16], const T* __restrict__ a,
+                                                 const int (&off)[NCW], Epi epi) {
+  constexpr int KS = KC / 16, NS = NCW * KS;
+  static_assert(D <= NS, "ring deeper than the stream");
+  typename MF<T>::frag ring[D];
+#pragma unroll
+  for (int i = 0; i < D; ++i) ring[i] = MF<T>::load(a + off[i / KS] + 16 * (i % KS));
+  f32x16 acc = zero16();
+#pragma unroll
+  for (int i = 0; i < NS; ++i) {
+    const typename MF<T>::frag f = ring[i % D];
+    if (i + D < NS) ring[i % D] = MF<T>::load(a + off[(i + D) / KS] + 16 * ((i + D) % KS));
+    acc = MF<T>::mma(fw[i % KS], f, acc);
+    if (i % KS == KS - 1) {
+      epi(i / KS, acc);
+      acc = zero16();
+    }
+  }
+}
+
+template <int EX_, int NPX>
+__device__ __forceinline__ int mlp_pixel(int p, int y0, int x0, int H, int W) {
+  const int py = p / EX_, px = p - py * EX_;
+  const int y = y0 + py, x = x0 + px;
+  return (p < NPX && y >= 0 && y < H && x >= 0 && x < W) ? y * W + x : -1;
+}
+
+template <typename T, int KC, int ACT>
+__global__ __launch_bounds__(256, 5) void dw2_mlp_fwd_kernel(const T* __restrict__ x, const T* __restrict__ W1,
+                                                             const float* __restrict__ b1, const float* __restrict__ w,
+                                                             const float* __restrict__ b, T* __restrict__ f0,
+                                                             T* __restrict__ out, T* __restrict__ gprime, int ipg,
+                                                             int H, int W, int C, int tiles_x, int tiles_y, int ncb) {
+  constexpr int CB = MLP_CB, PM = MLP_PM, NCQ = CB / 4, NPX = EY * EX, NCH = (NPX + 31) / 32;
+  static_assert(256 / NCQ == TX2, "one tile column per thread");
+  __shared__ __attribute__((aligned(16))) T hs[NPX * PM];
+  const Tile2 t = tile2_of(CB, ipg, tiles_x, tiles_y, ncb);
+  const long pix0 = ((long)t.g * ipg + t.img) * H * W;
+  {
+    const int lane = threadIdx.x & 63, wv = threadIdx.x >> 6, r = lane & 31, hf = lane >> 5, nh = wv & 1;
+    const int ch0 = t.cb0 + nh * 32;
+    typename MF<T>::frag fw[KC / 16];
+    const T* wrow = W1 + ((long)t.g * C + ch0 + r) * KC + 8 * hf;
+#pragma unroll
+    for (int s = 0; s < KC / 16; ++s) fw[s] = MF<T>::load(wrow + 16 * s);
+    constexpr bool BIAS_REGS = KC == 64;
+    const float* bp = b1 + (long)t.g * C + ch0 + 4 * hf;
+    float4 bv[4];
+    if constexpr (BIAS_REGS) {
+#pragma unroll
+      for (int q = 0; q < 4; ++q) bv[q] = *reinterpret_cast<const float4*>(bp + 8 * q);
+    }
+    static_assert(NCH == 6, "three chunks per wave");
+    int pix[3], off[3];
+#pragma unroll
+    for (int j = 0; j < 3; ++j) {
+      pix[j] = mlp_pixel<EX, NPX>(((wv >> 1) + 2 * j) * 32 + r, t.ty0 - 1, t.tx0 - 1, H, W);
+      off[j] = (pix[j] < 0 ? 0 : pix[j]) * KC;
+    }
+    mlp_chunk_stream<T, KC, 3, (KC == 64 ? 8 : 4)>(fw, x + pix0 * KC + 8 * hf, off, [&](int j, const f32x16& acc) {
+      const int p = ((wv >> 1) + 2 * j) * 32 + r;
+      if (p < NPX) {
+        T* d = hs + p * PM + nh * 32 + 4 * hf;
+#pragma unroll
+        for (int q = 0; q < 4; ++q) {
+          uint2 v = make_uint2(0, 0);
+          if (pix[j] >= 0) {
+            const float4 bq = BIAS_REGS ? bv[q] : *reinterpret_cast<const float4*>(bp + 8 * q);
+            v = make_uint2(pack2<T>(acc[4 * q] + bq.x, acc[4 * q + 1] + bq.y),
+                           pack2<T>(acc[4 * q + 2] + bq.z, acc[4 * q + 3] + bq.w));
+          }
+          *reinterpret_cast<uint2*>(d + 8 * q) = v;
+        }
+      }
+    });
+  }
+  const int cq = threadIdx.x % NCQ, pl = threadIdx.x / NCQ;
+  const int c0 = t.cb0 + cq * 4;
+  __syncthreads();
+  cmx_f2 wr[2][9], bias[2];
+  load_w36(w + ((long)t.g * C + c0) * 9, wr);
+  if (b) {
+    const float4 b0 = *reinterpret_cast<const float4*>(b + (long)t.g * C + c0);
+    bias[0] = (cmx_f2){b0.x, b0.y}; bias[1] = (cmx_f2){b0.z, b0.w};
+  } else {
+    bias[0] = bias[1] = pk_splat(0.f);
+  }
+  const int xo = t.tx0 + pl;
+  if (xo >= W) return;
+  dw2_fwd_column<T, ACT, false, PM, true>(hs + pl * PM + cq * 4, wr, bias, out, gprime, f0,
+                                          (pix0 + (long)t.ty0 * W + xo) * C + c0, (long)W * C, H - t.ty0);
 }
 
 template <int N>
@@ -500,32 +606,34 @@
   }
 }
 
+template <int CB> constexpr int BWDG_NIT = TYB * TXB / (256 / (CB / 4));
+
 template <typename T, int CB>
-__global__ __launch_bounds__(256, 3) void dw2_bwdg_kernel(const T* __restrict__ da, const T* __restrict__ h,
-                                                       const T* __restrict__ gprime, const float* __restrict__ w,
-                                                       T* __restrict__ dh, float* __restrict__ part, int ipg, int H,
-                                                       int W, int C, int tiles_x, int tiles_y, int ncb, int nsp) {
+__device__ __forceinline__ void bwdg_load_h(const T* __restrict__ h, long ibase, const Tile2& t, int H, int W, int C,
+                                            V4<T> (&hreg)[BWDG_NIT<CB>]) {
   constexpr int NCQ = CB / 4, PPI = 256 / NCQ;
-  constexpr int NE = EYB * EXB, NIN = TYB * TXB;
-  constexpr int LPQ = 64 / NCQ;
-  constexpr int NV = LPQ == 4 ? 10 : 5;
-  constexpr int NIT = NIN / PPI;
-  __shared__ __attribute__((aligned(16))) T dzs[NE * CB];
-  static_assert(sizeof(dzs) >= 4 * 64 * NV * sizeof(float), "cross-wave reduce buffer");
-  static_assert(NIN % PPI == 0, "pixel rounds");
-  const Tile2 t = tile2_of<TYB, TXB>(CB, ipg, tiles_x, tiles_y, ncb);
-  const long ibase = ((long)t.g * ipg + t.img) * H * W * C + t.cb0;
-  stage_dz<T, CB>(da + ibase, gprime + ibase, dzs, t.ty0, t.tx0, H, W, C);
+  static_assert(TYB * TXB % PPI == 0, "pixel rounds");
   const int cq = threadIdx.x % NCQ, pl = threadIdx.x / NCQ;
-  const int c0 = t.cb0 + cq * 4;
-  V4<T> hreg[NIT];
-#pragma unroll
-  for (int k = 0; k < NIT; ++k) {
+#pragma unroll
+  for (int k = 0; k < BWDG_NIT<CB>; ++k) {
     const int it = pl + k * PPI;
     const int y = t.ty0 + it / TXB, x = t.tx0 + it % TXB;
     hreg[k].a = {};
     if (y < H && x < W) hreg[k] = v4_load<T>(h + ibase + ((long)y * W + x) * C + cq * 4);
   }
+}
+
+template <typename T, int CB, int PITCH, int NBYTES>
+__device__ __forceinline__ void bwdg_from_dz(T* dzs, const V4<T> (&hreg)[BWDG_NIT<CB>], const float* __restrict__ w,
+                                             T* __restrict__ dh, float* __restrict__ part, const Tile2& t, long ibase,
+                                             int H, int W, int C, int nsp) {
+  constexpr int NCQ = CB / 4, PPI = 256 / NCQ;
+  constexpr int LPQ = 64 / NCQ;
+  constexpr int NV = LPQ == 4 ? 10 : 5;
+  constexpr int NIT = BWDG_NIT<CB>;
+  static_assert(NBYTES >= 4 * 64 * NV * (int)sizeof(float), "cross-wave reduce buffer");
+  const int cq = threadIdx.x % NCQ, pl = threadIdx.x / NCQ;
+  const int c0 = t.cb0 + cq * 4;
   __syncthreads();
   cmx_f2 wr[2][9];
   load_w36(w + ((long)t.g * C + c0) * 9, wr);
@@ -539,12 +647,12 @@
     const int x = t.tx0 + pl;
     const int nr = H - t.ty0;
     if (x < W) {
-      const T* dzp = dzc + pl * CB;
+      const T* dzp = dzc + pl * PITCH;
       cmx_f2 win[3][3][2];
 #pragma unroll
       for (int j = 0; j < 3; ++j) {
-        v4_unpack<T>(v4_load<T>(dzp + j * CB), win[0][j]);
-        v4_unpack<T>(v4_load<T>(dzp + (EXB + j) * CB), win[1][j]);
+        v4_unpack<T>(v4_load<T>(dzp + j * PITCH), win[0][j]);
+        v4_unpack<T>(v4_load<T>(dzp + (EXB + j) * PITCH), win[1][j]);
       }
       long o = ibase + ((long)t.ty0 * W + x) * C + cq * 4;
       const long ostep = (long)W * C;
@@ -552,7 +660,7 @@
       for (int k = 0; k < NIT; ++k) {
         if (k < nr) {
 #pragma unroll
-          for (int j = 0; j < 3; ++j) v4_unpack<T>(v4_load<T>(dzp + ((k + 2) * EXB + j) * CB), win[(k + 2) % 3][j]);
+          for (int j = 0; j < 3; ++j) v4_unpack<T>(v4_load<T>(dzp + ((k + 2) * EXB + j) * PITCH), win[(k + 2) % 3][j]);
           cmx_f2 hv[2];
           v4_unpack<T>(hreg[k], hv);
           cmx_f2 g[2] = {pk_splat(0.f), pk_splat(0.f)};
@@ -591,7 +699,7 @@
 #pragma unroll
         for (int j = 0; j < 3; ++j) {
           cmx_f2 dv[2];
-          v4_unpack<T>(v4_load<T>(dzc + ((r + 2 - i) * EXB + c + 2 - j) * CB), dv);
+          v4_unpack<T>(v4_load<T>(dzc + ((r + 2 - i) * EXB + c + 2 - j) * PITCH), dv);
 #pragma unroll
           for (int u = 0; u < 2; ++u) {
             g[u] = pk_fma(wr[u][i * 3 + j], dv[u], g[u]);
@@ -639,6 +747,69 @@
     for (int bit = 0; bit < (NV == 5 ? 3 : 2); ++bit) sgi = sgi * 2 + ((sg >> bit) & 1);
     o[q * 40 + sgi * NV + k] = v;
   }
+}
+
+template <typename T, int CB>
+__global__ __launch_bounds__(256, 3) void dw2_bwdg_kernel(const T* __restrict__ da, const T* __restrict__ h,
+                                                       const T* __restrict__ gprime, const float* __restrict__ w,
+                                                       T* __restrict__ dh, float* __restrict__ part, int ipg, int H,
+                                                       int W, int C, int tiles_x, int tiles_y, int ncb, int nsp) {
+  __shared__ __attribute__((aligned(16))) T dzs[EYB * EXB * CB];
+  const Tile2 t = tile2_of<TYB, TXB>(CB, ipg, tiles_x, tiles_y, ncb);
+  const long ibase = ((long)t.g * ipg + t.img) * H * W * C + t.cb0;
+  stage_dz<T, CB>(da + ibase, gprime + ibase, dzs, t.ty0, t.tx0, H, W, C);
+  V4<T> hreg[BWDG_NIT<CB>];
+  bwdg_load_h<T, CB>(h, ibase, t, H, W, C, hreg);
+  bwdg_from_dz<T, CB, CB, (int)sizeof(dzs)>(dzs, hreg, w, dh, part, t, ibase, H, W, C, nsp);
+}
+
+template <typename T, int KC>
+__global__ __launch_bounds__(256, 3) void dw2_mlp_bwdg_kernel(const T* __restrict__ dz2, const T* __restrict__ W2,
+                                                              const T* __restrict__ h, const T* __restrict__ gprime,
+                                                              const float* __restrict__ w, T* __restrict__ dh,
+                                                              float* __restrict__ part, int ipg, int H, int W, int C,
+                                                              int tiles_x, int tiles_y, int ncb, int nsp) {
+  constexpr int CB = MLP_CB, PM = MLP_PM, NE = EYB * EXB, NCH = (NE + 31) / 32;
+  __shared__ __attribute__((aligned(16))) T dzs[NE * PM];
+  const Tile2 t = tile2_of<TYB, TXB>(CB, ipg, tiles_x, tiles_y, ncb);
+  const long pix0 = ((long)t.g * ipg + t.img) * H * W;
+  const long ibase = pix0 * C + t.cb0;
+  stage_region_pm<T, CB, EYB, EXB, PM>(gprime + ibase, dzs, t.ty0 - 1, t.tx0 - 1, H, W, C);
+  V4<T> hreg[BWDG_NIT<CB>];
+  bwdg_load_h<T, CB>(h, ibase, t, H, W, C, hreg);
+  {
+    const int lane = threadIdx.x & 63, wv = threadIdx.x >> 6, r = lane & 31, hf = lane >> 5, nh = wv & 1;
+    typename MF<T>::frag fw[KC / 16];
+    const T* wcol = W2 + (long)t.g * KC * C + t.cb0 + nh * 32 + r;
+#pragma unroll
+    for (int s = 0; s < KC / 16; ++s) {
+      T e[8];
+#pragma unroll
+      for (int k = 0; k < 8; ++k) e[k] = wcol[(long)(16 * s + 8 * hf + k) * C];
+      fw[s] = frag_bits<T>(pack_raw<T>(e));
+    }
+    constexpr int NCW = (NCH + 1) / 2;
+    int pix[NCW], off[NCW];
+#pragma unroll
+    for (int j = 0; j < NCW; ++j) {
+      pix[j] = mlp_pixel<EXB, NE>(((wv >> 1) + 2 * j) * 32 + r, t.ty0 - 1, t.tx0 - 1, H, W);
+      off[j] = (pix[j] < 0 ? 0 : pix[j]) * KC;
+    }
+    mlp_chunk_stream<T, KC, NCW, 8>(fw, dz2 + pix0 * KC + 8 * hf, off, [&](int j, const f32x16& acc) {
+      if (j == 0) __syncthreads();
+      if (pix[j] >= 0) {
+        T* d = dzs + (((wv >> 1) + 2 * j) * 32 + r) * PM + nh * 32 + 4 * hf;
+#pragma unroll
+        for (int q = 0; q < 4; ++q) {
+          const uint2 g = *reinterpret_cast<const uint2*>(d + 8 * q);
+          const cmx_f2 d0 = unpack2<T>(pack2<T>(acc[4 * q], acc[4 * q + 1])) * unpack2<T>(g.x);
+          const cmx_f2 d1 = unpack2<T>(pack2<T>(acc[4 * q + 2], acc[4 * q + 3])) * unpack2<T>(g.y);
+          *reinterpret_cast<uint2*>(d + 8 * q) = make_uint2(pack2<T>(d0.x, d0.y), pack2<T>(d1.x, d1.y));
+        }
+      }
+    });
+  }
+  bwdg_from_dz<T, CB, PM, (int)sizeof(dzs)>(dzs, hreg, w, dh, part, t, ibase, H, W, C, nsp);
 }
 
 
@@ -772,6 +943,22 @@
 
 static int tile_cb(int C, int dtype) { return (C % 64 == 0 && (dtype == 1 || dtype == 2)) ? 64 : C % 32 == 0 ? 32 : 0; }
 
+static bool mlp_fusable(int C, int hidden, int dtype) {
+  return (dtype == 1 || dtype == 2) && (C == 64 || C == 128) && hidden > 0 && hidden % MLP_CB == 0;
+}
+
+static int fold_partials(float* workspace, float* dw, float* db, int G, int P, int C, int accumulate, const char* what,
+                         hipStream_t s) {
+  if (!dw && !db) return cmx_check_launch(what);
+  float* tmp = workspace + (size_t)G * P * C * 10;
+  int st = cmx_reduce_partials(workspace, tmp, G, P, C * 10, 0, 1.f, s);
+  if (st) return st;
+  const long tot = (long)G * C * 10;
+  hipLaunchKernelGGL(dw_scatter_kernel, dim3(cdiv(tot, 256) < 4096 ? cdiv(tot, 256) : 4096), dim3(256), 0, s, tmp, dw,
+                     db, G, C, accumulate);
+  return cmx_check_launch(what);
+}
+
 extern "C" {
 
 int cmx_dwconv3x3_fwd(const void* h, const float* w, const float* b, void* out, int NI, int imgs_per_group, int H,
@@ -832,14 +1019,63 @@
                          (const T*)gprime, w, (T*)dh, workspace, imgs_per_group, H, W, C, tx, ty, ncb, P);
     }
   });
-  if (!dw && !db) return cmx_check_launch("dwconv_bwd_saved");
-  float* tmp = workspace + (size_t)G * P * C * 10;
-  int st = cmx_reduce_partials(workspace, tmp, G, P, C * 10, 0, 1.f, s);
-  if (st) return st;
-  const long tot = (long)G * C * 10;
-  hipLaunchKernelGGL(dw_scatter_kernel, dim3(cdiv(tot, 256) < 4096 ? cdiv(tot, 256) : 4096), dim3(256), 0, s, tmp, dw,
-                     db, G, C, accumulate);
-  return cmx_check_launch("dwconv_bwd_saved");
+  return fold_partials(workspace, dw, db, G, P, C, accumulate, "dwconv_bwd_saved", s);
+}
+
+int cmx_mlp_fc1_dwconv_fwd(const void* x, const void* W1, const float* b1, const float* w, const float* b, void* f0,
+                           void* out, void* gprime, int NI, int imgs_per_group, int H, int W, int C, int hidden,
+                           int act, int dtype, hipStream_t s) {
+  CMX_REQUIRE(mlp_fusable(C, hidden, dtype) && act == ACT_GELU, CMX_ERR_SHAPE,
+              "mlp_fc1_dwconv_fwd: C=%d hidden=%d dtype=%d act=%d (16-bit, C 64 / 128, hidden %% 64 == 0, GELU)", C,
+              hidden, dtype, act);
+  CMX_REQUIRE(NI > 0 && imgs_per_group > 0 && NI % imgs_per_group == 0 && H > 0 && W > 0, CMX_ERR_SHAPE,
+              "mlp_fc1_dwconv_fwd: NI=%d imgs_per_group=%d H=%d W=%d", NI, imgs_per_group, H, W);
+  CMX_REQUIRE(x && W1 && b1 && w && f0 && out && gprime, CMX_ERR_ARG, "mlp_fc1_dwconv_fwd: null operand");
+  CMX_REQUIRE((long)NI * H * W * hidden < (1L << 31), CMX_ERR_SHAPE, "mlp_fc1_dwconv_fwd: tensor too large");
+  const int G = NI / imgs_per_group;
+  const int tx = cdiv(W, TX2), ty = cdiv(H, TY2), ncb = hidden / MLP_CB;
+  const dim3 grid((unsigned)imgs_per_group * ty * tx * ncb, G);
+  CMX_DISPATCH(dtype, T, {
+    if constexpr (sizeof(T) == 2) {
+      if (C == 64) {
+        hipLaunchKernelGGL((dw2_mlp_fwd_kernel<T, 64, ACT_GELU>), grid, dim3(256), 0, s, (const T*)x, (const T*)W1, b1,
+                           w, b, (T*)f0, (T*)out, (T*)gprime, imgs_per_group, H, W, hidden, tx, ty, ncb);
+      } else {
+        hipLaunchKernelGGL((dw2_mlp_fwd_kernel<T, 128, ACT_GELU>), grid, dim3(256), 0, s, (const T*)x, (const T*)W1,
+                           b1, w, b, (T*)f0, (T*)out, (T*)gprime, imgs_per_group, H, W, hidden, tx, ty, ncb);
+      }
+    }
+  });
+  return cmx_check_launch("mlp_fc1_dwconv_fwd");
+}
+
+int cmx_mlp_fc2_dwconv_bwd(const void* dz, const void* W2, const void* h, const void* gprime, const float* w, void* dh,
+                           float* dw, float* db, float* workspace, int NI, int imgs_per_group, int H, int W, int C,
+                           int hidden, int accumulate, int dtype, hipStream_t s) {
+  CMX_REQUIRE(mlp_fusable(C, hidden, dtype), CMX_ERR_SHAPE,
+              "mlp_fc2_dwconv_bwd: C=%d hidden=%d dtype=%d (16-bit, C 64 / 128, hidden %% 64 == 0)", C, hidden, dtype);
+  CMX_REQUIRE(NI > 0 && imgs_per_group > 0 && NI % imgs_per_group == 0 && H > 0 && W > 0, CMX_ERR_SHAPE,
+              "mlp_fc2_dwconv_bwd: NI=%d imgs_per_group=%d H=%d W=%d", NI, imgs_per_group, H, W);
+  CMX_REQUIRE(dz && W2 && h && gprime && w && workspace, CMX_ERR_ARG, "mlp_fc2_dwconv_bwd: null operand");
+  CMX_REQUIRE((long)NI * H * W * hidden < (1L << 31), CMX_ERR_SHAPE, "mlp_fc2_dwconv_bwd: tensor too large");
+  const int G = NI / imgs_per_group;
+  const int tx = cdiv(W, TXB), ty = cdiv(H, TYB), ncb = hidden / MLP_CB;
+  const int P = imgs_per_group * ty * tx;
+  const dim3 grid((unsigned)P * ncb, G);
+  CMX_DISPATCH(dtype, T, {
+    if constexpr (sizeof(T) == 2) {
+      if (C == 64) {
+        hipLaunchKernelGGL((dw2_mlp_bwdg_kernel<T, 64>), grid, dim3(256), 0, s, (const T*)dz, (const T*)W2,
+                           (const T*)h, (const T*)gprime, w, (T*)dh, workspace, imgs_per_group, H, W, hidden, tx, ty,
+                           ncb, P);
+      } else {
+        hipLaunchKernelGGL((dw2_mlp_bwdg_kernel<T, 128>), grid, dim3(256), 0, s, (const T*)dz, (const T*)W2,
+                           (const T*)h, (const T*)gprime, w, (T*)dh, workspace, imgs_per_group, H, W, hidden, tx, ty,
+                           ncb, P);
+      }
+    }
+  });
+  return fold_partials(workspace, dw, db, G, P, hidden, accumulate, "mlp_fc2_dwconv_bwd", s);
 }
 
 int cmx_dwconv3x3_bwd_saved_tiles(int imgs_per_group, int H, int W) {
@@ -899,14 +1135,7 @@
       }
     });
   }
-  if (!dw && !db) return cmx_check_launch("dwconv_bwd");
-  float* tmp = workspace + (size_t)G * P * C * 10;
-  int st = cmx_reduce_partials(workspace, tmp, G, P, C * 10, 0, 1.f, s);
-  if (st) return st;
-  const long tot = (long)G * C * 10;
-  hipLaunchKernelGGL(dw_scatter_kernel, dim3(cdiv(tot, 256) < 4096 ? cdiv(tot, 256) : 4096), dim3(256), 0, s, tmp, dw,
-                     db, G, C, accumulate);
-  return cmx_check_launch("dwconv_bwd");
-}
-
-}
+  return fold_partials(workspace, dw, db, G, P, C, accumulate, "dwconv_bwd", s);
+}
+
+}
diff --git a/rgbx_semantic_segmentation_amd/floor.py b/rgbx_semantic_segmentation_amd/floor.py
--- a/rgbx_semantic_segmentation_amd/floor.py
+++ b/rgbx_semantic_segmentation_amd/floor.py
@@ -21,8 +21,9 @@
         fam[f][0] += flops
         fam[f][1] += byts
 
-    def gemm(M, N, Kd, G=1, res=False, wgrad=True, dgrad=True, bias_grad=True):
-        add("gemm", 2 * G * M * N * Kd, G * A * (M * Kd + N * Kd + M * N + (M * N if res else 0)))
+    def gemm(M, N, Kd, G=1, res=False, wgrad=True, dgrad=True, bias_grad=True, fwd=True):
+        if fwd:
+            add("gemm", 2 * G * M * N * Kd, G * A * (M * Kd + N * Kd + M * N + (M * N if res else 0)))
         if dgrad:
             add("gemm", 2 * G * M * N * Kd, G * A * (M * N + N * Kd + M * Kd))
         if wgrad:
@@ -32,7 +33,12 @@
         add("layernorm", 0, G * A * rows * C * 2 + G * F32 * 2 * rows)
         add("layernorm", 0, G * A * rows * C * (3 + (1 if two else 0) + (1 if tap else 0)) + G * F32 * 2 * rows)
 
-    def dw(M_pix, C, G=1):
+    def dw(M_pix, C, G=1, fc=0):
+        if fc:
+            lin = 2 * G * M_pix * C * fc, G * A * (M_pix * fc + C * fc)
+            add("dwconv", 2 * 9 * G * M_pix * C * 3 + lin[0], G * A * M_pix * C * 3 + lin[1])
+            add("dwconv", lin[0], G * A * M_pix * C * 3 + lin[1])
+            return
         add("dwconv", 2 * 9 * G * M_pix * C * 3, G * A * M_pix * C * 3)
         add("dwconv", 0, G * A * M_pix * C * 4)
 
@@ -76,9 +82,10 @@
             add("sra", 2.5 * fwd_f, G * A * (3 * M * C + Mk * 2 * C + M * C + Mk * 2 * C) + G * F32 * B * NUM_HEADS[s] * N * 2)
             gemm(M, C, C, G, res=True)
             ln(M, C, G, tap=True)
-            gemm(M, 4 * C, C, G)
-            dw(M, 4 * C, G)
-            gemm(M, C, 4 * C, G, res=True)
+            fused = C in (64, 128)
+            gemm(M, 4 * C, C, G, fwd=not fused)
+            dw(M, 4 * C, G, fc=C if fused else 0)
+            gemm(M, C, 4 * C, G, res=True, dgrad=not fused)
         ln(M, C, G, tap=True)
         add("frm", 0, G * A * M * C)
         add("frm", 2 * 2 * B * (16 * C * C + 8 * C * C), F32 * 3 * (16 * C * C + 8 * C * C))
diff --git a/rgbx_semantic_segmentation_amd/functions.py b/rgbx_semantic_segmentation_amd/functions.py
--- a/rgbx_semantic_segmentation_amd/functions.py
+++ b/rgbx_semantic_segmentation_amd/functions.py
@@ -558,6 +558,117 @@
     return DWConvF.apply(h, w, b, wg, bg, NI, ipg, H, W, act, conv.weight)
 
 
+MLP_FUSE = int(os.environ.get("CMX_MLP_FUSE", "3"))
+
+
+class MlpF(Function):
+
+    @staticmethod
+    def forward(ctx, x, res, W1, Wg1, b1, bg1, dw_w, dw_b, dw_wg, dw_bg, W2, Wg2, b2, bg2, a1, a2, a3, geom, rscale,
+                rps, tap, ln, dgrad_tap, fuse):
+        NI, ipg, H, Wd = geom
+        G, M, C = x.shape
+        hidden = W1.shape[1]
+        dt = K.dtype_code(x)
+        f0 = torch.empty(G, M, hidden, dtype=x.dtype, device=x.device)
+        f = torch.empty_like(f0)
+        gprime = torch.empty_like(f0)
+        if fuse & 1:
+            K.call("cmx_mlp_fc1_dwconv_fwd", x, W1, b1, dw_w, dw_b, f0, f, gprime, NI, ipg, H, Wd, C, hidden,
+                   K.ACT["gelu"], dt)
+        else:
+            _fwd_gemm(x, W1, b1, f0)
+            K.call("cmx_dwconv3x3_fwd_save", f0, dw_w, dw_b, f, gprime, NI, ipg, H, Wd, hidden, K.ACT["gelu"], dt)
+        y = torch.empty(G, M, W2.shape[1], dtype=x.dtype, device=x.device)
+        pre = None
+        if ln is not None:
+            gamma, beta, eps, sink = ln
+            pre = K.gemm_ln(f, W2, y, gamma, beta, eps, bias=b2, residual=res, rscale=rscale, rows_per_sample=rps)
+            sink.pre = pre
+        if pre is None:
+            _fwd_gemm(f, W2, b2, y, res=res, rscale=rscale, rps=rps)
+        ctx.save_for_backward(x, W1, f0, gprime, dw_w, f, W2)
+        ctx.meta = (Wg1, bg1, dw_wg, dw_bg, Wg2, bg2, geom, res is not None, rscale, rps, tap, dgrad_tap, fuse)
+        return y
+
+    @staticmethod
+    def backward(ctx, dy):
+        x, W1, f0, gprime, dw_w, f, W2 = ctx.saved_tensors
+        Wg1, bg1, dw_wg, dw_bg, Wg2, bg2, geom, has_res, rscale, rps, tap, dgrad_tap, fuse = ctx.meta
+        NI, ipg, H, Wd = geom
+        dy = _c(dy)
+        G, M, C = dy.shape
+        hidden = f0.shape[-1]
+        dt = K.dtype_code(x)
+        dres = dy if has_res else None
+        dz = dy
+        if rscale is not None:
+            dz = tap.take(dy) if tap is not None else None
+            if dz is None:
+                dz = K.scale_samples(dy, rscale, rps * C)
+        dz = _c(dz)
+        nbytes = K.query("cmx_dwconv3x3_bwd_workspace", NI, ipg, H, Wd, hidden)
+        defer = deferred.ENABLED
+        dw, db = (None, None) if defer else (dw_wg, dw_bg)
+        dh = torch.empty_like(f0)
+        if fuse & 2:
+            _wgrad_into(dz, f, Wg2, bg2)
+            ws = K._ws(nbytes, x.device)
+            K.call("cmx_mlp_fc2_dwconv_bwd", dz, W2, f0, gprime, dw_w, dh, dw, db, ws, NI, ipg, H, Wd, C, hidden, 0, dt)
+        else:
+            da = _dgrad(dz, W2, torch.empty_like(f))
+            _wgrad_into(dz, f, Wg2, bg2)
+            ws = K._ws(nbytes, x.device)
+            K.call("cmx_dwconv3x3_bwd_saved", da, f0, gprime, dw_w, dh, dw, db, ws, NI, ipg, H, Wd, hidden, 0, dt)
+        if defer:
+            P = K.query("cmx_dwconv3x3_bwd_saved_tiles", ipg, H, Wd)
+            deferred.reduce(ws, dw_wg, dw_bg, G, P, P * hidden * 10, hidden * 10, hidden, 10, 9, dw_wg.stride(0), 9,
+                            dw_bg.stride(0), 1)
+        dx = None
+        if dgrad_tap is not None and ctx.needs_input_grad[0]:
+            dgrad_tap.put((dh, W1))
+        elif ctx.needs_input_grad[0]:
+            dx = _dgrad(dh, W1, torch.empty_like(x))
+        _wgrad_into(dh, x, Wg1, bg1)
+        return (dx, dres) + (None,) * 22
+
+
+def mlp_fusable(x, W1, b1, W2) -> bool:
+    C, hidden = x.shape[-1], W1.shape[1]
+    return (MLP_FUSE & 3 != 0 and x.dtype in (torch.bfloat16, torch.float16) and C in (64, 128) and hidden % 64 == 0
+            and b1 is not None and x.is_contiguous() and W1.is_contiguous() and b1.is_contiguous()
+            and W2.is_contiguous() and tuple(W2.shape[1:]) == (C, hidden))
+
+
+def mlp(store, m, x, NI, ipg, H, W, res=None, rscale=None, rps=1, tap=None, ln_tail=None, dgrad_tap=None):
+    G = x.shape[0]
+
+    def lin(layer):
+        W, Wg = store.w(layer.weight), store.g(layer.weight)
+        return (W.view(G, W.shape[1], -1), Wg.view(G, Wg.shape[1], -1), store.w(layer.bias, compute=False).view(G, -1),
+                store.g(layer.bias).view(G, -1))
+
+    W1, Wg1, b1, bg1 = lin(m.fc1)
+    W2, Wg2, b2, bg2 = lin(m.fc2)
+    if not mlp_fusable(x, W1, b1, W2):
+        f = glinear(store, m.fc1.weight, m.fc1.bias, x, dgrad_tap=dgrad_tap)
+        f = dwconv(store, m.dwconv.dwconv, f, NI, ipg, H, W, "gelu")
+        return glinear(store, m.fc2.weight, m.fc2.bias, f, res=res, rscale=rscale, rps=rps, tap=tap, ln_tail=ln_tail)
+    conv = m.dwconv.dwconv
+    dw_w = store.w(conv.weight, compute=False).view(G, -1, 9)
+    dw_b = store.w(conv.bias, compute=False).view(G, -1)
+    dw_wg = store.g(conv.weight).view(G, -1, 9)
+    dw_bg = store.g(conv.bias).view(G, -1)
+    ln = None
+    N = W2.shape[1]
+    if ln_tail is not None and LN_ROW and N <= 128 and N % 8 == 0:
+        nm = ln_tail.mod
+        ln = (store.w(nm.weight, compute=False).view(G, -1), store.w(nm.bias, compute=False).view(G, -1), nm.eps,
+              ln_tail)
+    return MlpF.apply(x, res, W1, Wg1, b1, bg1, dw_w, dw_b, dw_wg, dw_bg, W2, Wg2, b2, bg2, m.fc1.weight,
+                      conv.weight, m.fc2.weight, (NI, ipg, H, W), rscale, rps, tap, ln, dgrad_tap, MLP_FUSE)
+
+
 class DgradTap:
     __slots__ = ("t",)
 
diff --git a/rgbx_semantic_segmentation_amd/models/encoders/dual_segformer.py b/rgbx_semantic_segmentation_amd/models/encoders/dual_segformer.py
--- a/rgbx_semantic_segmentation_amd/models/encoders/dual_segformer.py
+++ b/rgbx_semantic_segmentation_amd/models/encoders/dual_segformer.py
@@ -206,12 +206,10 @@
         x = F.glinear(store, a.proj.weight, a.proj.bias, o, res=xr, rscale=s_attn, rps=N, tap=tap_a, ln_tail=t2)
         ltap = F.DgradTap() if F.ln_bwd_fusable(x) else None
         h, _, xr = F.layernorm_res(store, blk.norm2, x, G, scale=s_attn, rps=N, tap=tap_a, tail=t2, dtap=ltap)
-        f = F.glinear(store, blk.mlp.fc1.weight, blk.mlp.fc1.bias, h, dgrad_tap=ltap)
-        f = F.dwconv(store, blk.mlp.dwconv.dwconv, f, G * B, B, H, W, "gelu")
         tap_m = F.GradTap() if s_mlp is not None else None
         tn = F.LNTail(next_norm) if next_norm is not None else None
-        x = F.glinear(store, blk.mlp.fc2.weight, blk.mlp.fc2.bias, f, res=xr, rscale=s_mlp, rps=N, tap=tap_m,
-                      ln_tail=tn)
+        x = F.mlp(store, blk.mlp, h, G * B, B, H, W, res=xr, rscale=s_mlp, rps=N, tap=tap_m, ln_tail=tn,
+                  dgrad_tap=ltap)
         return x, (s_mlp, tap_m), tn
 
     def run(self, store, images, B, H, W, training, dp_scales: Optional[torch.Tensor], bn_group=None, aspp_mask=None):
diff --git a/rgbx_semantic_segmentation_amd/roofline.py b/rgbx_semantic_segmentation_amd/roofline.py
--- a/rgbx_semantic_segmentation_amd/roofline.py
+++ b/rgbx_semantic_segmentation_amd/roofline.py
@@ -56,7 +56,7 @@
     ("wgrad", r"gemm_grouped_kernel|reduce_grouped_kernel"),
     ("gemm", r"gemm_bf16_kernel|gemm_stream|gemm_multi|gemm_generic|splitk_reduce"),
     ("sra", r"sra_"),
-    ("dwconv", r"dw2_|dw_"),
+    ("dwconv", r"dw2_mlp_|dw2_|dw_"),
     ("layernorm", r"ln_fwd|ln_bwd|rowln"),
     ("adamw", r"adamw"),
     ("batchnorm", r"bn_"),
```
